# Drjay806/PRO-B-GAN

Measured on NVIDIA B200. Metric: generator+discriminator samples/sec (score_triplets pass, bf16 tensor-core mode), higher is better.
Workload: dtype bf16

## Files before the change

include/pbg.h:

```cpp
#ifndef PBG_H_
#define PBG_H_

#include <stddef.h>
#include <stdint.h>

#ifdef __cplusplus
extern "C" {
#endif

#define PBG_ABI_VERSION 1

typedef struct pbg_ctx pbg_ctx;

typedef enum pbg_status {
  PBG_OK = 0,
  PBG_ERR_INVALID = 1,
  PBG_ERR_CUDA = 2,
  PBG_ERR_NOT_LOADED = 3,
  PBG_ERR_INDEX = 4,
  PBG_ERR_UNSUPPORTED = 5,
  PBG_ERR_NOMEM = 6
} pbg_status;

typedef enum pbg_precision {
  PBG_PREC_F32 = 0,
  PBG_PREC_BF16 = 1
} pbg_precision;

typedef enum pbg_dtype { PBG_DT_F32 = 0, PBG_DT_BF16 = 1 } pbg_dtype;

typedef struct pbg_dims {
  int32_t embed_dim;
  int32_t noise_dim;
  int32_t g_hidden;
  int32_t d_hidden;
  int32_t device;
  float leaky_slope;
} pbg_dims;

int pbg_abi_version(void);

int pbg_create(pbg_ctx** out, const pbg_dims* dims);
void pbg_destroy(pbg_ctx* ctx);

const char* pbg_last_error(const pbg_ctx* ctx);

int pbg_load_generator(pbg_ctx* ctx, const float* packed_host, size_t n_floats);

int pbg_load_discriminator(pbg_ctx* ctx, const float* packed_host, size_t n_floats);

int pbg_generator_forward(pbg_ctx* ctx, const float* h, const float* r, const float* z, void* out,
                          int64_t B, int precision, int out_dtype, void* stream);

int pbg_generator_forward_gather(pbg_ctx* ctx, const float* node_emb, int64_t N, const float* rel_emb,
                                 int64_t R, const int64_t* heads, int64_t head_stride,
                                 const int64_t* rels, int64_t rel_stride, const float* z, void* out,
                                 int64_t B, int precision, int out_dtype, void* stream);

int pbg_discriminator_forward(pbg_ctx* ctx, const float* h, const float* r, const float* t,
                              float* logits, float* probs, int64_t B, int precision, void* stream);

int pbg_discriminator_score_triplets(pbg_ctx* ctx, const float* node_emb, int64_t N,
                                     const float* rel_emb, int64_t R, const int64_t* triplets,
                                     float* logits, float* probs, int64_t B, int precision,
                                     void* stream);

int pbg_score_triplets(pbg_ctx* ctx, const float* node_emb, int64_t N, const float* rel_emb, int64_t R,
                       const int64_t* triplets, const float* z, void* gen_out, int out_dtype,
                       float* gen_scores, float* logits, float* probs, int64_t B, int precision,
                       void* stream);

int pbg_score_triplets_host(pbg_ctx* ctx, const float* node_emb, int64_t N, const float* rel_emb,
                            int64_t R, const int64_t* triplets_host, const float* z_host,
                            float* gen_out_host, float* gen_scores_host, float* logits_host,
                            float* probs_host, int64_t B, int precision);

int pbg_score_triplets_host_packed(pbg_ctx* ctx, const float* node_emb, int64_t N, const float* rel_emb,
                                   int64_t R, const void* in_block_host, float* out_block_host, int64_t B,
                                   int precision);

int pbg_draw_latents(pbg_ctx* ctx, uint64_t seed, uint64_t offset, int64_t total_rows, int64_t row_begin,
                     int64_t rows, float* z_out, uint64_t* offset_after, void* stream);

int pbg_set_latent_stream(pbg_ctx* ctx, int enable, uint64_t seed, uint64_t offset);
int pbg_get_latent_stream(pbg_ctx* ctx, uint64_t* seed, uint64_t* offset, void* stream);

int pbg_score_triplets_host_ids(pbg_ctx* ctx, const float* node_emb, int64_t N, const float* rel_emb, int64_t R,
                                const int64_t* triplets_host, float* out_block_host, int64_t B, int precision);

int pbg_reserve(pbg_ctx* ctx, int64_t rows, int precision, int stage_slots);
int pbg_stage_triplets(pbg_ctx* ctx, int slot, const float* node_emb, int64_t N, const float* rel_emb, int64_t R,
                       const int64_t* triplets, const float* z, int64_t B, int want_gen, int want_disc, void* stream);
int pbg_score_staged(pbg_ctx* ctx, int slot, void* gen_out, int out_dtype, float* gen_scores, float* logits,
                     float* probs, void* stream);
int pbg_score_staged_stage_next(pbg_ctx* ctx, int slot, void* gen_out, int out_dtype, float* gen_scores, float* logits,
                                float* probs, const float* node_emb, int64_t N, const float* rel_emb, int64_t R,
                                const int64_t* next_triplets, const float* next_z, int64_t next_B, void* stream);

int pbg_check_indices(pbg_ctx* ctx, void* stream);

int pbg_linear_bf16(pbg_ctx* ctx, int model, int layer, const void* a_bf16, void* out, int64_t M,
                    void* stream);

enum {
  PBG_K_GATHER = 0,
  PBG_K_G_L0 = 1,
  PBG_K_G_L1 = 2,
  PBG_K_G_L2 = 3,
  PBG_K_D_L0 = 4,
  PBG_K_D_L1 = 5,
  PBG_K_OTHER = 6,
  PBG_K_PASS = 7,
  PBG_K_TOPK = 8,
  PBG_NUM_KERNEL_KINDS = 9
};
int pbg_profile_enable(pbg_ctx* ctx, int enable);
int pbg_profile_read(pbg_ctx* ctx, double* ms, int64_t* count);

int pbg_debug_trace(pbg_ctx* ctx, int enable, int64_t* host_out, int64_t n_slots);

int pbg_set_launch_width(pbg_ctx* ctx, int n_ctas);

int pbg_last_pass_sm_clock(pbg_ctx* ctx, void* stream, double* mhz_out);

int pbg_set_workspace_discard(pbg_ctx* ctx, int on);

int pbg_set_result_mirrors(pbg_ctx* ctx, int n, void* const* gen_out, float* const* gen_scores,
                           float* const* logits, float* const* probs);

int pbg_set_result_multicast(pbg_ctx* ctx, void* gen_out_mc, float* gen_scores_mc, float* logits_mc, float* probs_mc);

int pbg_topk_prepare(pbg_ctx* ctx, const float* table, int64_t N, void* stream);
int pbg_topk(pbg_ctx* ctx, const float* queries, int64_t B, int k, int64_t* out_idx, float* out_scores, void* stream);
int64_t pbg_topk_last_flagged(pbg_ctx* ctx, void* stream);

int64_t pbg_parse_index_rows(const char* text, size_t len, int cols, int64_t* out, size_t cap_rows);

int64_t pbg_format_f32_json(const float* v, size_t rows, int cols, int indent, int depth, char* out, size_t cap);
int64_t pbg_format_i64_json(const int64_t* v, size_t rows, int cols, int indent, int depth, char* out, size_t cap);

int64_t pbg_launch_count(const pbg_ctx* ctx);

#ifdef __cplusplus
}
#endif
#endif
```

pro-b-gan_b200/csrc/gather.cuh:

```cuda
#pragma once
#include <cuda_bf16.h>
#include <stdint.h>

namespace pbg {

struct GatherParams {
  const float* node_emb;
  const float* rel_emb;
  long long N, R;
  int E, Z;
  const long long* heads; long long head_stride;
  const long long* rels;  long long rel_stride;
  const long long* tails; long long tail_stride;
  const float* h; const float* r; const float* t;
  const float* z;
  void* xg; int ldg;
  void* xd; int ldd;
  long long B;
  int* err_flag;
};

template <typename T>
__device__ __forceinline__ void store4(T* dst, float4 v);
template <>
__device__ __forceinline__ void store4<float>(float* dst, float4 v) {
  *reinterpret_cast<float4*>(dst) = v;
}
template <>
__device__ __forceinline__ void store4<__nv_bfloat16>(__nv_bfloat16* dst, float4 v) {
  __nv_bfloat162 lo = __floats2bfloat162_rn(v.x, v.y), hi = __floats2bfloat162_rn(v.z, v.w);
  uint2 w;
  w.x = *reinterpret_cast<uint32_t*>(&lo);
  w.y = *reinterpret_cast<uint32_t*>(&hi);
  *reinterpret_cast<uint2*>(dst) = w;
}

__device__ __forceinline__ float4 ld_stream4(const float* p) {
  float4 v;
  asm volatile("ld.global.nc.L1::no_allocate.v4.f32 {%0, %1, %2, %3}, [%4];"
               : "=f"(v.x), "=f"(v.y), "=f"(v.z), "=f"(v.w) : "l"(p));
  return v;
}

template <typename T>
__global__ void __launch_bounds__(256) gather_concat_kernel(const GatherParams p) {
  const int lane = threadIdx.x & 31;
  const long long warp_global = (static_cast<long long>(blockIdx.x) * blockDim.x + threadIdx.x) >> 5;
  const long long num_warps = (static_cast<long long>(gridDim.x) * blockDim.x) >> 5;
  const int E4 = p.E >> 2, Z4 = p.Z >> 2;
  T* xg = static_cast<T*>(p.xg);
  T* xd = static_cast<T*>(p.xd);

  for (long long b = warp_global; b < p.B; b += num_warps) {
    const float *hrow, *rrow, *trow = nullptr;
    bool bad = false;
    if (p.heads != nullptr) {
      long long i = p.heads[b * p.head_stride];
      if (i < 0) i += p.N;
      if (i < 0 || i >= p.N) { bad = true; i = 0; }
      hrow = p.node_emb + i * p.E;
    } else {
      hrow = p.h + b * p.E;
    }
    if (p.rels != nullptr) {
      long long i = p.rels[b * p.rel_stride];
      if (i < 0 || i >= p.R) { bad = true; i = 0; }
      rrow = p.rel_emb + i * p.E;
    } else {
      rrow = p.r + b * p.E;
    }
    if (p.tails != nullptr) {
      long long i = p.tails[b * p.tail_stride];
      if (i < 0) i += p.N;
      if (i < 0 || i >= p.N) { bad = true; i = 0; }
      trow = p.node_emb + i * p.E;
    } else if (xd != nullptr) {
      trow = p.t + b * p.E;
    }
    if (bad && lane == 0) atomicOr(p.err_flag, 1);

    T* g = xg ? xg + b * p.ldg : nullptr;
    T* d = xd ? xd + b * p.ldd : nullptr;
    for (int v = lane; v < E4; v += 32) {
      const float4 hv = ld_stream4(hrow + 4 * v);
      const float4 rv = ld_stream4(rrow + 4 * v);
      if (g) { store4<T>(g + 4 * v, hv); store4<T>(g + p.E + 4 * v, rv); }
      if (d) {
        store4<T>(d + 4 * v, hv);
        store4<T>(d + p.E + 4 * v, rv);
        store4<T>(d + 2 * p.E + 4 * v, ld_stream4(trow + 4 * v));
      }
    }
    if (g) {
      const float* zrow = p.z + b * p.Z;
      for (int v = lane; v < Z4; v += 32) store4<T>(g + 2 * p.E + 4 * v, ld_stream4(zrow + 4 * v));
      for (int v = (2 * p.E + p.Z) / 4 + lane; v < p.ldg / 4; v += 32)
        store4<T>(g + 4 * v, make_float4(0.f, 0.f, 0.f, 0.f));
    }
    if (d) {
      for (int v = (3 * p.E) / 4 + lane; v < p.ldd / 4; v += 32)
        store4<T>(d + 4 * v, make_float4(0.f, 0.f, 0.f, 0.f));
    }
  }
}

struct StageParams {
  GatherParams g;
  float* xt;
};
__global__ void __launch_bounds__(128, 12) stage_rows_kernel(const __grid_constant__ StageParams sp) {
  const int lane = threadIdx.x & 31;
  const long long warp_global = (static_cast<long long>(blockIdx.x) * blockDim.x + threadIdx.x) >> 5;
  const long long num_warps = (static_cast<long long>(gridDim.x) * blockDim.x) >> 5;
  const int E = sp.g.E, Z = sp.g.Z, E4 = E >> 2, Z4 = Z >> 2;
  const long long N = sp.g.N;
  __nv_bfloat16* const xg = static_cast<__nv_bfloat16*>(sp.g.xg);
  __nv_bfloat16* const xd = static_cast<__nv_bfloat16*>(sp.g.xd);
  for (long long b = warp_global; b < sp.g.B; b += num_warps) {
    bool bad = false;
    long long hi = sp.g.heads[b * 3], ri = sp.g.rels[b * 3], ti = sp.g.tails[b * 3];
    if (hi < 0) hi += N;
    if (ti < 0) ti += N;
    if (hi < 0 || hi >= N) { bad = true; hi = 0; }
    if (ri < 0 || ri >= sp.g.R) { bad = true; ri = 0; }
    if (ti < 0 || ti >= N) { bad = true; ti = 0; }
    if (bad && lane == 0) atomicOr(sp.g.err_flag, 1);
    const float* hrow = sp.g.node_emb + hi * E;
    const float* rrow = sp.g.rel_emb + ri * E;
    const float* trow = sp.g.node_emb + ti * E;
    __nv_bfloat16* g = xg ? xg + b * sp.g.ldg : nullptr;
    __nv_bfloat16* d = xd ? xd + b * sp.g.ldd : nullptr;
    for (int v = lane; v < E4; v += 32) {
      const float4 hv = ld_stream4(hrow + 4 * v);
      const float4 rv = ld_stream4(rrow + 4 * v);
      const float4 tv = ld_stream4(trow + 4 * v);
      if (g) {
        store4<__nv_bfloat16>(g + 4 * v, hv);
        store4<__nv_bfloat16>(g + E + 4 * v, rv);
      }
      if (d) {
        store4<__nv_bfloat16>(d + 4 * v, hv);
        store4<__nv_bfloat16>(d + E + 4 * v, rv);
        store4<__nv_bfloat16>(d + 2 * E + 4 * v, tv);
      }
      if (sp.xt) store4<float>(sp.xt + b * E + 4 * v, tv);
    }
    if (g) {
      for (int v = lane; v < Z4; v += 32) store4<__nv_bfloat16>(g + 2 * E + 4 * v, ld_stream4(sp.g.z + b * Z + 4 * v));
      for (int v = (2 * E + Z) / 4 + lane; v < sp.g.ldg / 4; v += 32)
        store4<__nv_bfloat16>(g + 4 * v, make_float4(0.f, 0.f, 0.f, 0.f));
    }
    if (d)
      for (int v = (3 * E) / 4 + lane; v < sp.g.ldd / 4; v += 32)
        store4<__nv_bfloat16>(d + 4 * v, make_float4(0.f, 0.f, 0.f, 0.f));
  }
}

__global__ void pack_bf16_kernel(const float* __restrict__ src, __nv_bfloat16* __restrict__ dst, int rows, int cols,
                                 int rows_p, int cols_p) {
  const long long total = static_cast<long long>(rows_p) * cols_p;
  for (long long i = static_cast<long long>(blockIdx.x) * blockDim.x + threadIdx.x; i < total;
       i += static_cast<long long>(gridDim.x) * blockDim.x) {
    const int r = static_cast<int>(i / cols_p), c = static_cast<int>(i % cols_p);
    dst[i] = __float2bfloat16_rn((r < rows && c < cols) ? src[static_cast<long long>(r) * cols + c] : 0.f);
  }
}

__global__ void pad_f32_kernel(const float* __restrict__ src, float* __restrict__ dst, int n, int n_p) {
  for (int i = blockIdx.x * blockDim.x + threadIdx.x; i < n_p; i += gridDim.x * blockDim.x)
    dst[i] = i < n ? src[i] : 0.f;
}

}
```

pro-b-gan_b200/csrc/pass2_kernel.cuh:

```cuda
#pragma once
#include <cuda.h>
#include "ptx.cuh"
#include "gather.cuh"
#include "tc_common.cuh"
#include "pass_common.cuh"

namespace pbg {

#ifndef PBG_STAGES
#define PBG_STAGES 5
#endif
#ifndef PBG_EPI_WARPS
#define PBG_EPI_WARPS 8
#endif
constexpr int kP2Stages = PBG_STAGES;
constexpr int kP2Epi = PBG_EPI_WARPS;
constexpr int kP2Slots = kP2Epi / 4;
constexpr int kP2Threads = 64 + 32 * kP2Epi;
static_assert(kP2Epi == 8 || kP2Epi == 16, "epilogue warps");
#ifndef PBG_ROLES_FIRST
#define PBG_ROLES_FIRST 0
#endif
constexpr int kProdWarp = PBG_ROLES_FIRST ? 0 : kP2Epi;
constexpr int kMmaWarp = PBG_ROLES_FIRST ? 1 : kP2Epi + 1;
// ... 50 lines not shown
  int phase0_groups;
  int n_total;
  int n_seg;
  P2Segment seg[16];
  int nrb;
  int rb_cap;
  int M;
  float slope;
  PassSched* sched;
  int* ready;
  int* fin;
  void* gen_out; int out_f32; int n_valid; int ld_gen;
  float* cosine; const float* tail_tab; const long long* tail_idx; long long tail_stride; long long n_ent;
  float* part_g;
  int slots_g;
  const float* w3; float b3; float* logits; float* probs;
  int w3_off;
  float* part_d;
  int slots_d;
  int n_mirror;
  void* mir_gen[kMaxMirrors]; float* mir_cos[kMaxMirrors]; float* mir_logits[kMaxMirrors]; float* mir_probs[kMaxMirrors];
  void* mc_gen; float* mc_cos; float* mc_logits; float* mc_probs;
  long long* trace;
};
static_assert(sizeof(Pass2Params) <= 4096, "kernel parameter space");

struct P2Smem {
  static constexpr int kA = 128 * kBlockK * 2;
  static constexpr int kW = 128 * kBlockK * 2;
  static constexpr int kStage = kA + kW;
  static constexpr int kStagingOff = kP2Stages * kStage;
  static constexpr int kStagingPerWarp = 4096;
  static constexpr int kBiasOff = kStagingOff + kP2Epi * kStagingPerWarp;
  static constexpr int kBiasFloats = 6144;
  static constexpr int kBarOff = kBiasOff + kBiasFloats * 4;
  static constexpr int kXchgOff = kBarOff + 256;
  static constexpr int kXchgBytes = 4 * 32 * 3 * 4;
  static constexpr int kTotal = kXchgOff + kXchgBytes + 256 + 1024 ;
};
static_assert(P2Smem::kTotal <= 232448, "pass2: shared memory budget");

__device__ __forceinline__ void st_cluster_u32x2(uint32_t cluster_addr, uint2 v) {
  asm volatile("st.shared::cluster.v2.u32 [%0], {%1, %2};" ::"r"(cluster_addr), "r"(v.x), "r"(v.y) : "memory");
}
__device__ __forceinline__ void multimem_st_v4(void* mc_addr, uint4 v) {
  asm volatile("multimem.st.relaxed.sys.global.v4.f32 [%0], {%1, %2, %3, %4};" ::"l"(mc_addr), "f"(__uint_as_float(v.x)),
               "f"(__uint_as_float(v.y)), "f"(__uint_as_float(v.z)), "f"(__uint_as_float(v.w)) : "memory");
}
__device__ __forceinline__ void multimem_st_f32(float* mc_addr, float v) {
  asm volatile("multimem.st.relaxed.sys.global.f32 [%0], %1;" ::"l"(mc_addr), "f"(v) : "memory");
}
__device__ __forceinline__ float2 add2(float2 a, float2 b) {
  float2 d;
  asm("{\n\t.reg .b64 ra, rb, rd;\n\tmov.b64 ra, {%2, %3};\n\tmov.b64 rb, {%4, %5};\n\tadd.rn.f32x2 rd, ra, rb;\n\t"
      "mov.b64 {%0, %1}, rd;\n\t}\n"
      : "=f"(d.x), "=f"(d.y) : "f"(a.x), "f"(a.y), "f"(b.x), "f"(b.y));
  return d;
}
__device__ __forceinline__ float2 mul2(float2 a, float2 b) {
  float2 d;
  asm("{\n\t.reg .b64 ra, rb, rd;\n\tmov.b64 ra, {%2, %3};\n\tmov.b64 rb, {%4, %5};\n\tmul.rn.f32x2 rd, ra, rb;\n\t"
      "mov.b64 {%0, %1}, rd;\n\t}\n"
      : "=f"(d.x), "=f"(d.y) : "f"(a.x), "f"(a.y), "f"(b.x), "f"(b.y));
  return d;
}
__device__ __forceinline__ uint32_t bias_leaky_pack(uint32_t a0, uint32_t a1, float b0, float b1, float slope) {
  const float2 y = add2(make_float2(__uint_as_float(a0), __uint_as_float(a1)), make_float2(b0, b1));
  const float2 s = mul2(y, make_float2(slope, slope));
  return pack_bf16x2(fmaxf(y.x, s.x), fmaxf(y.y, s.y));
}

__device__ __forceinline__ int p2_dep_target(const Pass2Params& p, int dep_kind) {
  if (p.no_deps) return 0;
  if (dep_kind == DEP_X) return p.gather_external ? 0 : kP2GroupsPerBlock;
  const int producer = dep_kind == DEP_G0 ? IT_G_L0 : (dep_kind == DEP_D0 ? IT_D_L0 : IT_G_L1);
  return p.layer[producer].n_tiles * kP2WarpsPerPair;
}
__device__ __forceinline__ void p2_arrive(const Pass2Params& p, int dep_kind, int rb, int lane, bool async_stores,
                                          long long* t_wait = nullptr) {
  __syncwarp();
  if (lane == 0) {
    int* ctr = p.ready + dep_kind * p.rb_cap + rb;
    if (async_stores) {
      const long long t0 = t_wait ? clock64() : 0;
      tma_store_wait<0>();
      if (t_wait) *t_wait += clock64() - t0;
      red_relaxed_gpu_add(ctr, 1);
    } else {
      red_release_gpu_add(ctr, 1);
    }
  }
}
__device__ __forceinline__ void p2_arrive_done(const Pass2Params& p, int dep_kind, int rb, int lane) {
  if (lane == 0) red_relaxed_gpu_add(p.ready + dep_kind * p.rb_cap + rb, 1);
}
__device__ __forceinline__ void p2_poll_dep(const Pass2Params& p, int dep_kind, int rb) {
  const int target = p2_dep_target(p, dep_kind);
  const int* ctr = p.ready + dep_kind * p.rb_cap + rb;
  uint32_t spins = 0;
  while (ld_relaxed_gpu(ctr) < target) {
    __nanosleep(p.poll_ns);
#if PBG_HANG_GUARD
    if (++spins > 4000000u) pbg_wait_timed_out("dependency (kind, row block)", dep_kind, rb);
#endif
  }
  fence_proxy_async_all();
}

__device__ __forceinline__ void p2_discard(const void* base, size_t bytes, int part, int nparts, int lane) {
  const char* b = static_cast<const char*>(base);
  for (size_t off = static_cast<size_t>(part) * 4096 + static_cast<size_t>(lane) * 128; off < bytes; off += static_cast<size_t>(nparts) * 4096)
    asm volatile("discard.global.L2 [%0], 128;" ::"l"(b + off) : "memory");
}

__device__ __forceinline__ void p2_tail_load(float4 (&tv)[8], unsigned long long trow_bits, int col0, int n_valid, int lane) {
#pragma unroll
  for (int i = 0; i < 8; ++i) {
    const int r = i * 4 + (lane >> 3), t = lane & 7;
    const float* tp2 = reinterpret_cast<const float*>(__shfl_sync(0xffffffffu, trow_bits, r));
    tv[i] = make_float4(0.f, 0.f, 0.f, 0.f);
    if (tp2 != nullptr && col0 + t * 4 < n_valid) tv[i] = ld_stream4(tp2 + col0 + t * 4);
  }
}
__device__ __forceinline__ void p2_tail_stage(uint8_t* st, const float4 (&tv)[8], int lane) {
#pragma unroll
  for (int i = 0; i < 8; ++i) {
    const int r = i * 4 + (lane >> 3), t = lane & 7;
    *reinterpret_cast<float4*>(st + r * 128 + ((t ^ (r & 7)) << 4)) = tv[i];
  }
  __syncwarp();
}
__device__ __forceinline__ void p2_tail_dot(const uint8_t* st, const float* f, int col0, int n_valid, int lane, float& d, float& pp,
                                            float& tt) {
#pragma unroll
  for (int t = 0; t < 8; ++t) {
    const float4 x = *reinterpret_cast<const float4*>(st + lane * 128 + ((t ^ (lane & 7)) << 4));
    if (col0 + t * 4 < n_valid) {
      d += f[4 * t] * x.x + f[4 * t + 1] * x.y + f[4 * t + 2] * x.z + f[4 * t + 3] * x.w;
      pp += f[4 * t] * f[4 * t] + f[4 * t + 1] * f[4 * t + 1] + f[4 * t + 2] * f[4 * t + 2] + f[4 * t + 3] * f[4 * t + 3];
      tt += x.x * x.x + x.y * x.y + x.z * x.z + x.w * x.w;
    }
  }
  __syncwarp();
}

template <class F>
__device__ __forceinline__ void p2_gather_group_bulk(const GatherParams& g, long long group, int lane, uint8_t* st,
                                                     F&& before_staging, bool keep) {
  const long long r0 = group * 4;
  __nv_bfloat16* xg = static_cast<__nv_bfloat16*>(g.xg);
  __nv_bfloat16* xd = static_cast<__nv_bfloat16*>(g.xd);
  const float* src = nullptr;
  bool bad = false;
  if (lane < 12) {
    const long long row = r0 + lane / 3;
    const int which = lane % 3;
    if (row < g.B) {
      if (which == 0) {
        if (g.heads) { long long i = g.heads[row * g.head_stride]; if (i < 0) i += g.N; if (i < 0 || i >= g.N) { bad = true; i = 0; } src = g.node_emb + i * g.E; }
        else src = g.h + row * g.E;
      } else if (which == 1) {
        if (g.rels) { long long i = g.rels[row * g.rel_stride]; if (i < 0 || i >= g.R) { bad = true; i = 0; } src = g.rel_emb + i * g.E; }
        else src = g.r + row * g.E;
      } else if (g.tails) {
        long long i = g.tails[row * g.tail_stride]; if (i < 0) i += g.N; if (i < 0 || i >= g.N) { bad = true; i = 0; } src = g.node_emb + i * g.E;
      } else if (xd != nullptr) {
        src = g.t + row * g.E;
      }
    }
  }
  if (bad) atomicOr(g.err_flag, 1);
  const unsigned long long sp = reinterpret_cast<unsigned long long>(src);
  const int Z4 = g.Z >> 2;
  const int wg = 2 * g.E + g.Z, wd = 3 * g.E;
  float4 hv[4], rv[4], tv[4], zv[4];
#pragma unroll
  for (int j = 0; j < 4; ++j) {
    const float* ph = reinterpret_cast<const float*>(__shfl_sync(0xffffffffu, sp, j * 3 + 0));
    const float* pr = reinterpret_cast<const float*>(__shfl_sync(0xffffffffu, sp, j * 3 + 1));
    const float* pt = reinterpret_cast<const float*>(__shfl_sync(0xffffffffu, sp, j * 3 + 2));
    const long long row = r0 + j;
    hv[j] = rv[j] = tv[j] = zv[j] = make_float4(0.f, 0.f, 0.f, 0.f);
    if (row < g.B) {
      hv[j] = ld_stream4(ph + 4 * lane);
      rv[j] = ld_stream4(pr + 4 * lane);
      if (xd != nullptr) tv[j] = ld_stream4(pt + 4 * lane);
      if (xg != nullptr && lane < Z4) zv[j] = ld_stream4(g.z + row * g.Z + 4 * lane);
    }
  }
  before_staging();
  const long long nrow = min(4ll, g.B - r0);
  if (xg != nullptr) {
#pragma unroll
    for (int j = 0; j < 4; ++j) {
      __nv_bfloat16* o = reinterpret_cast<__nv_bfloat16*>(st) + j * wg;
      store4<__nv_bfloat16>(o + 4 * lane, hv[j]);
      store4<__nv_bfloat16>(o + g.E + 4 * lane, rv[j]);
      if (lane < Z4) store4<__nv_bfloat16>(o + 2 * g.E + 4 * lane, zv[j]);
    }
    fence_proxy_async_smem();
    __syncwarp();
    if (lane == 0 && nrow > 0) {
      if (keep) bulk_store_1d_hint(xg + r0 * wg, st, static_cast<uint32_t>(nrow * wg * 2), kEvictLast);
      else bulk_store_1d(xg + r0 * wg, st, static_cast<uint32_t>(nrow * wg * 2));
      tma_store_commit();
      if (xd != nullptr) tma_store_wait_read<0>();
    }
    __syncwarp();
  }
  if (xd != nullptr) {
#pragma unroll
    for (int j = 0; j < 4; ++j) {
      __nv_bfloat16* o = reinterpret_cast<__nv_bfloat16*>(st) + j * wd;
      store4<__nv_bfloat16>(o + 4 * lane, hv[j]);
      store4<__nv_bfloat16>(o + g.E + 4 * lane, rv[j]);
      store4<__nv_bfloat16>(o + 2 * g.E + 4 * lane, tv[j]);
    }
    fence_proxy_async_smem();
    __syncwarp();
    if (lane == 0 && nrow > 0) {
      if (keep) bulk_store_1d_hint(xd + r0 * wd, st, static_cast<uint32_t>(nrow * wd * 2), kEvictLast);
      else bulk_store_1d(xd + r0 * wd, st, static_cast<uint32_t>(nrow * wd * 2));
      tma_store_commit();
    }
  }
}

__device__ __forceinline__ uint32_t ring_dep(uint2 it) { return (it.x >> 24) << 3; }

template <bool TR, bool FASTG, bool BIASS>
__global__ void __cluster_dims__(2, 1, 1) __launch_bounds__(kP2Threads, 1)
pbg_pass2_kernel(const __grid_constant__ Pass2Params p) {
  using L = P2Smem;
  extern __shared__ uint8_t smem_raw[];
  uint8_t* smem = smem_raw + ((1024u - (smem_u32(smem_raw) & 1023u)) & 1023u);
  uint64_t* full_bar = reinterpret_cast<uint64_t*>(smem + L::kBarOff);
  uint64_t* empty_bar = full_bar + kP2Stages;
  uint64_t* tmem_full = empty_bar + kP2Stages;
  uint64_t* tmem_empty = tmem_full + 2;
  uint64_t* sched_full = tmem_empty + 2;
  uint64_t* sched_empty = sched_full + kP2Ring;
  uint64_t* bias_bar = sched_empty + kP2Ring;
  uint2* ring = reinterpret_cast<uint2*>(bias_bar + 1);
  uint32_t* tmem_slot = reinterpret_cast<uint32_t*>(ring + kP2Ring);
  int* last_flag = reinterpret_cast<int*>(tmem_slot + 1);
  volatile long long* t_issue = reinterpret_cast<volatile long long*>(smem + L::kXchgOff + L::kXchgBytes);
  float* xchg = reinterpret_cast<float*>(smem + L::kXchgOff);
  float* sbias = reinterpret_cast<float*>(smem + L::kBiasOff);

  const int warp = threadIdx.x >> 5;
  const int lane = threadIdx.x & 31;
  const uint32_t rank = cluster_ctarank();
  const bool leader = rank == 0;
  const long long t_entry = (TR && p.trace && threadIdx.x == 0) ? static_cast<long long>(globaltimer_ns()) : 0;
  asm volatile("griddepcontrol.launch_dependents;" ::: "memory");
  constexpr int kRingConsumers = 2 * (1 + kP2Epi) + 1;

  if (threadIdx.x == 0) {
    for (int i = 0; i < 5; ++i) {
      if (p.layer_mask & (1u << i)) {
        prefetch_tmap(&p.tm_a[i]);
        prefetch_tmap(&p.tm_w[i]);
        if (p.layer[i].epi == PEPI_STORE) prefetch_tmap(&p.tm_o[i]);
      }
    }
    for (int s = 0; s < kP2Stages; ++s) {
      mbar_init(&full_bar[s], 1);
      mbar_init(&empty_bar[s], 1);
    }
    for (int s = 0; s < 2; ++s) {
      mbar_init(&tmem_full[s], 1);
      mbar_init(&tmem_empty[s], kP2WarpsPerPair);
    }
    for (int s = 0; s < kP2Ring; ++s) {
      mbar_init(&sched_full[s], 1);
      mbar_init(&sched_empty[s], kRingConsumers);
    }
    mbar_init(bias_bar, 1);
    fence_mbar_init();
    if (BIASS) {
    uint32_t bytes = 0;
    for (int k = 0; k < 5; ++k)
      if (p.layer_mask & (1u << k)) bytes += static_cast<uint32_t>(p.layer[k].n_tiles * p.layer[k].block_n) * 4u;
    if (p.layer_mask & (1u << IT_D_L1)) bytes += static_cast<uint32_t>(p.layer[IT_D_L1].n_tiles * p.layer[IT_D_L1].block_n) * 4u;
    mbar_arrive_expect_tx(bias_bar, bytes);
    for (int k = 0; k < 5; ++k)
      if (p.layer_mask & (1u << k))
        bulk_load_1d(sbias + p.layer[k].bias_off, p.layer[k].bias, static_cast<uint32_t>(p.layer[k].n_tiles * p.layer[k].block_n) * 4u, bias_bar);
    if (p.layer_mask & (1u << IT_D_L1))
      bulk_load_1d(sbias + p.w3_off, p.w3, static_cast<uint32_t>(p.layer[IT_D_L1].n_tiles * p.layer[IT_D_L1].block_n) * 4u, bias_bar);
    }
  }
  if (warp == kMmaWarp) tmem_alloc_pair<512>(tmem_slot);
  tc_fence_before();
  __syncthreads();
  cluster_sync_all();
  tc_fence_after();
  asm volatile("griddepcontrol.wait;" ::: "memory");
  const uint32_t tmem_base = *tmem_slot;
  long long* const clk0 = reinterpret_cast<long long*>(smem + L::kXchgOff + L::kXchgBytes) + 8;
  if (blockIdx.x == 0 && threadIdx.x == 0) { clk0[0] = clock64(); clk0[1] = static_cast<long long>(globaltimer_ns()); }
  long long* const tr = (TR && p.trace) ? p.trace + kTraceSlots * blockIdx.x : nullptr;
  if (tr && threadIdx.x == 0) { tr[0] = clock64(); tr[14] = static_cast<long long>(globaltimer_ns()); tr[254] = t_entry; }

  const uint32_t lead_tmem_empty = mapa_u32(smem_u32(tmem_empty), 0);
  const uint32_t sched_empty_addr = mapa_u32(smem_u32(sched_empty), 1);
  const uint32_t ring_addr = mapa_u32(smem_u32(ring), 1);
  if (warp == kMmaWarp && !leader) {
    if (lane == 0) {
      uint32_t slot = 0, sphase = 0;
      const uint32_t lead_sched_full = mapa_u32(smem_u32(sched_full), 0);
      for (;;) {
        const int ticket = atomicAdd(&p.sched->q_head, 1);
        uint2 it = make_uint2(IT_END, 0u);
        if (ticket < p.n_total) {
          int sg = 0;
          while (sg + 1 < p.n_seg && ticket >= p.seg[sg + 1].start) ++sg;
          const int i = ticket - p.seg[sg].start;
          const int nt1 = p.seg[sg].n_tiles, nt = nt1 + p.seg[sg].n_tiles2;
          const int j = i % nt;
          it = make_uint2(static_cast<uint32_t>(j < nt1 ? p.seg[sg].kind : p.seg[sg].kind2) | (static_cast<uint32_t>(j < nt1 ? j : j - nt1) << 8),
                          static_cast<uint32_t>(p.seg[sg].rb0 + i / nt));
        }
        if ((it.x & 0xff) != IT_END) p2_poll_dep(p, p.layer[it.x & 0xff].dep_kind, static_cast<int>(it.y));
        mbar_wait_role(&sched_empty[slot], sphase ^ 1);
        ring[slot] = it;
        mbar_arrive(&sched_full[slot]);
        mbar_arrive_cluster(lead_sched_full + slot * 8);
        if (++slot == kP2Ring) { slot = 0; sphase ^= 1; }
        if ((it.x & 0xff) == IT_END) break;
      }
    }
    __syncwarp();
  } else if (warp == kProdWarp) {
    if (lane == 0) {
      uint32_t stage = 0, phase = 0, slot = 0, sphase = 0;
      long long w_dep = 0, w_empty = 0, n_items = 0;
      const uint32_t lead_full = mapa_u32(smem_u32(full_bar), 0);
      for (;;) {
        mbar_wait_role(&sched_full[slot], sphase);
        const uint2 it = ld_cluster_u32x2(ring_addr + slot * 8);
        mbar_arrive_remote(sched_empty_addr + slot * 8 + ring_dep(it));
        if (++slot == kP2Ring) { slot = 0; sphase ^= 1; }
        const int kind = it.x & 0xff;
        if (kind == IT_END) break;
        long long* ti = (tr && n_items < kTraceItems) ? tr + 16 + 4 * n_items : nullptr;
        if (ti) { ti[0] = (clock64() << 20) | (static_cast<long long>(it.y & 0xfff) << 8) | kind; }
        ++n_items;
        const int n_blk = (it.x >> 8) & 0xff;
        const int rb = static_cast<int>(it.y);
        const P2Layer& ly = p.layer[kind];
        const int w_rows = ly.block_n >> 1;
        const uint32_t bytes_pair = 2u * (L::kA + static_cast<uint32_t>(w_rows) * kBlockK * 2);
        const int a_row = rb * kP2Rows + static_cast<int>(rank) * 128;
        const int w_row = n_blk * ly.block_n + static_cast<int>(rank) * w_rows;
        for (int kb = 0; kb < ly.num_kb; ++kb) {
          if (tr) { const long long t = clock64(); mbar_wait_role(&empty_bar[stage], phase ^ 1); w_empty += clock64() - t; }
          else mbar_wait_role(&empty_bar[stage], phase ^ 1);
          uint8_t* sa = smem + stage * L::kStage;
          if (leader) mbar_arrive_expect_tx(&full_bar[stage], bytes_pair);
          if (tr) t_issue[stage] = clock64();
          tma_load_2d_pair(sa + L::kA, &p.tm_w[kind], lead_full + stage * 8, kb * kBlockK, w_row);
          tma_load_2d_pair(sa, &p.tm_a[kind], lead_full + stage * 8, kb * kBlockK, a_row);
          if (++stage == kP2Stages) { stage = 0; phase ^= 1; }
        }
      }
      if (tr) { tr[1] = w_empty; tr[2] = clock64(); tr[12] = n_items; if (leader) tr[11] = w_dep; }
    }
    __syncwarp();
// ... 589 lines not shown
```

pro-b-gan_b200/csrc/pass_common.cuh:

```cuda
#pragma once
#include <cuda.h>
#include "ptx.cuh"
#include "gather.cuh"
#include "tc_common.cuh"

namespace pbg {

enum : int { IT_G_L0 = 0, IT_D_L0 = 1, IT_G_L1 = 2, IT_D_L1 = 3, IT_G_L2 = 4, IT_GATHER = 5, IT_END = 255 };
enum : int { DEP_X = 0, DEP_G0 = 1, DEP_D0 = 2, DEP_G1 = 3, DEP_KINDS = 4 };
enum : int { FIN_G = 0, FIN_D = 1, FIN_KINDS = 2 };
enum : int { PEPI_STORE = 0, PEPI_TANH = 1, PEPI_ROWDOT = 2 };

constexpr int kEpiWarps = 8;
constexpr int kPassThreads = 64 + 32 * kEpiWarps;
constexpr int kTraceSlots = 256;
constexpr int kTraceItems = 54;


struct PassSched {
  int q_head;
  int q_tail;
  int p0_next;
  int init;
  int done;
  int pad_;
  long long clk_ticks, clk_ns;
};



__device__ __forceinline__ int ld_relaxed_gpu(const int* p) {
  int v;
  asm volatile("ld.relaxed.gpu.global.s32 %0, [%1];" : "=r"(v) : "l"(p) : "memory");
  return v;
}
__device__ __forceinline__ void fence_acq_rel_gpu() { asm volatile("fence.acq_rel.gpu;" ::: "memory"); }
__device__ __forceinline__ void red_release_gpu_add(int* p, int v) {
  asm volatile("red.release.gpu.global.add.s32 [%0], %1;" ::"l"(p), "r"(v) : "memory");
}
__device__ __forceinline__ void red_relaxed_gpu_add(int* p, int v) {
  asm volatile("red.relaxed.gpu.global.add.s32 [%0], %1;" ::"l"(p), "r"(v) : "memory");
}
__device__ __forceinline__ int atom_relaxed_gpu_add(int* p, int v) {
  int old;
  asm volatile("atom.relaxed.gpu.global.add.s32 %0, [%1], %2;" : "=r"(old) : "l"(p), "r"(v) : "memory");
  return old;
}
__device__ __forceinline__ int atom_release_gpu_add(int* p, int v) {
  int old;
  asm volatile("atom.release.gpu.global.add.s32 %0, [%1], %2;" : "=r"(old) : "l"(p), "r"(v) : "memory");
  return old;
}
__device__ __forceinline__ unsigned long long globaltimer_ns() {
  unsigned long long t;
  asm volatile("mov.u64 %0, %%globaltimer;" : "=l"(t));
  return t;
}
__device__ __forceinline__ void fence_proxy_async_all() { asm volatile("fence.proxy.async;" ::: "memory"); }

__device__ __forceinline__ void tmem_ld_32x32_ptr(uint32_t taddr, uint32_t* v) {
  asm volatile(
      "tcgen05.ld.sync.aligned.32x32b.x32.b32 "
      "{%0, %1, %2, %3, %4, %5, %6, %7, %8, %9, %10, %11, %12, %13, %14, %15, "
      "%16, %17, %18, %19, %20, %21, %22, %23, %24, %25, %26, %27, %28, %29, %30, %31}, [%32];"
      : "=r"(v[0]), "=r"(v[1]), "=r"(v[2]), "=r"(v[3]), "=r"(v[4]), "=r"(v[5]), "=r"(v[6]), "=r"(v[7]),
        "=r"(v[8]), "=r"(v[9]), "=r"(v[10]), "=r"(v[11]), "=r"(v[12]), "=r"(v[13]), "=r"(v[14]), "=r"(v[15]),
        "=r"(v[16]), "=r"(v[17]), "=r"(v[18]), "=r"(v[19]), "=r"(v[20]), "=r"(v[21]), "=r"(v[22]), "=r"(v[23]),
        "=r"(v[24]), "=r"(v[25]), "=r"(v[26]), "=r"(v[27]), "=r"(v[28]), "=r"(v[29]), "=r"(v[30]), "=r"(v[31])
      : "r"(taddr)
      : "memory");
}

__device__ __forceinline__ float leaky_max(float x, float slope) { return fmaxf(x, x * slope); }

template <int MODE = 0>
__device__ __forceinline__ void pass_gather_group(const GatherParams& g, long long group, int lane) {
  const long long r0 = group * 4;
  __nv_bfloat16* xg = static_cast<__nv_bfloat16*>(g.xg);
  __nv_bfloat16* xd = static_cast<__nv_bfloat16*>(g.xd);
  const float* src = nullptr;
  bool bad = false;
  if (lane < 12) {
    const long long row = r0 + lane / 3;
    const int which = lane % 3;
    if (row < g.B) {
      if (which == 0) {
        if (g.heads) { long long i = g.heads[row * g.head_stride]; if (i < 0) i += g.N; if (i < 0 || i >= g.N) { bad = true; i = 0; } src = g.node_emb + i * g.E; }
        else src = g.h + row * g.E;
      } else if (which == 1) {
        if (g.rels) { long long i = g.rels[row * g.rel_stride]; if (i < 0 || i >= g.R) { bad = true; i = 0; } src = g.rel_emb + i * g.E; }
        else src = g.r + row * g.E;
      } else if (g.tails) {
        long long i = g.tails[row * g.tail_stride]; if (i < 0) i += g.N; if (i < 0 || i >= g.N) { bad = true; i = 0; } src = g.node_emb + i * g.E;
      } else if (xd != nullptr) {
        src = g.t + row * g.E;
      }
    }
  }
  if (bad) atomicOr(g.err_flag, 1);
  const unsigned long long sp = reinterpret_cast<unsigned long long>(src);
  const int E4 = g.E >> 2, Z4 = g.Z >> 2;
  if (MODE == 1 || (MODE == 0 && E4 == 32 && Z4 <= 32)) {
    float4 hv[4], rv[4], tv[4], zv[4];
#pragma unroll
    for (int j = 0; j < 4; ++j) {
      const float* ph = reinterpret_cast<const float*>(__shfl_sync(0xffffffffu, sp, j * 3 + 0));
      const float* pr = reinterpret_cast<const float*>(__shfl_sync(0xffffffffu, sp, j * 3 + 1));
      const float* pt = reinterpret_cast<const float*>(__shfl_sync(0xffffffffu, sp, j * 3 + 2));
      const long long row = r0 + j;
      hv[j] = rv[j] = tv[j] = zv[j] = make_float4(0.f, 0.f, 0.f, 0.f);
      if (row < g.B) {
        hv[j] = ld_stream4(ph + 4 * lane);
        rv[j] = ld_stream4(pr + 4 * lane);
        if (xd != nullptr) tv[j] = ld_stream4(pt + 4 * lane);
        if (xg != nullptr && lane < Z4) zv[j] = ld_stream4(g.z + row * g.Z + 4 * lane);
      }
    }
#pragma unroll
    for (int j = 0; j < 4; ++j) {
      const long long row = r0 + j;
      if (row >= g.B) continue;
      if (xg != nullptr) {
        __nv_bfloat16* o = xg + row * g.ldg;
        store4<__nv_bfloat16>(o + 4 * lane, hv[j]);
        store4<__nv_bfloat16>(o + g.E + 4 * lane, rv[j]);
        if (lane < Z4) store4<__nv_bfloat16>(o + 2 * g.E + 4 * lane, zv[j]);
        for (int v = (2 * g.E + g.Z) / 4 + lane; v < g.ldg / 4; v += 32)
          store4<__nv_bfloat16>(o + 4 * v, make_float4(0.f, 0.f, 0.f, 0.f));
      }
      if (xd != nullptr) {
        __nv_bfloat16* o = xd + row * g.ldd;
        store4<__nv_bfloat16>(o + 4 * lane, hv[j]);
        store4<__nv_bfloat16>(o + g.E + 4 * lane, rv[j]);
        store4<__nv_bfloat16>(o + 2 * g.E + 4 * lane, tv[j]);
        for (int v = (3 * g.E) / 4 + lane; v < g.ldd / 4; v += 32)
          store4<__nv_bfloat16>(o + 4 * v, make_float4(0.f, 0.f, 0.f, 0.f));
      }
    }
  } else {
    for (int j = 0; j < 4; ++j) {
      const float* ph = reinterpret_cast<const float*>(__shfl_sync(0xffffffffu, sp, j * 3 + 0));
      const float* pr = reinterpret_cast<const float*>(__shfl_sync(0xffffffffu, sp, j * 3 + 1));
      const float* pt = reinterpret_cast<const float*>(__shfl_sync(0xffffffffu, sp, j * 3 + 2));
      const long long row = r0 + j;
      if (row >= g.B) continue;
      __nv_bfloat16* og = xg ? xg + row * g.ldg : nullptr;
      __nv_bfloat16* od = xd ? xd + row * g.ldd : nullptr;
      for (int v = lane; v < E4; v += 32) {
        const float4 h4 = ld_stream4(ph + 4 * v), r4 = ld_stream4(pr + 4 * v);
        if (og) { store4<__nv_bfloat16>(og + 4 * v, h4); store4<__nv_bfloat16>(og + g.E + 4 * v, r4); }
        if (od) {
          store4<__nv_bfloat16>(od + 4 * v, h4);
          store4<__nv_bfloat16>(od + g.E + 4 * v, r4);
          store4<__nv_bfloat16>(od + 2 * g.E + 4 * v, ld_stream4(pt + 4 * v));
        }
      }
      if (og) {
        for (int v = lane; v < Z4; v += 32) store4<__nv_bfloat16>(og + 2 * g.E + 4 * v, ld_stream4(g.z + row * g.Z + 4 * v));
        for (int v = (2 * g.E + g.Z) / 4 + lane; v < g.ldg / 4; v += 32)
          store4<__nv_bfloat16>(og + 4 * v, make_float4(0.f, 0.f, 0.f, 0.f));
      }
      if (od)
        for (int v = (3 * g.E) / 4 + lane; v < g.ldd / 4; v += 32)
          store4<__nv_bfloat16>(od + 4 * v, make_float4(0.f, 0.f, 0.f, 0.f));
    }
  }
}

__device__ __forceinline__ void warp_publish(int* counter, int lane) {
  __syncwarp();
  if (lane == 0) red_release_gpu_add(counter, 1);
}
__device__ __forceinline__ int warp_publish_fetch(int* counter, int lane) {
  __syncwarp();
  int old = 0;
  if (lane == 0) old = atom_release_gpu_add(counter, 1);
  return __shfl_sync(0xffffffffu, old, 0);
}


}
```

pro-b-gan_b200/csrc/pbg.cu:

```cuda
#include <cuda.h>
#include <cuda_runtime.h>
#include <cuda_bf16.h>

#include <algorithm>
#include <cstdarg>
#include <cstdio>
#include <cstring>
#include <cstdlib>
#include <map>
#include <tuple>
#include <new>
#include <string>
#include <vector>

#include "../../include/pbg.h"
#include "gather.cuh"
#include "gemm_f32.cuh"
#include "tc_common.cuh"
#include "pass_common.cuh"
#include "pass2_kernel.cuh"
#include "topk_kernel.cuh"
#include "index_rows.cuh"
#include "json_out.cuh"
#include "latent.cuh"

using namespace pbg;

namespace {

constexpr long long kMaxChunk = 65536;
constexpr int kPartSlotsG = 16;
constexpr int kPartSlotsD = 64;

inline int round_up(int v, int m) { return (v + m - 1) / m * m; }

struct Linear {
  int n = 0, k = 0;
  int np = 0, kp = 0;
  float* w_f32 = nullptr;
  float* b_f32 = nullptr;
  __nv_bfloat16* w_bf16 = nullptr;
  float* b_pad = nullptr;
  CUtensorMap tmap_w128;
  CUtensorMap tmap_w64;
};

struct Workspace {
  long long rows = 0;
  void *xg0 = nullptr, *xd0 = nullptr, *bufA = nullptr, *bufB = nullptr, *bufD = nullptr;
  CUtensorMap tm_xg0, tm_xd0, tm_bufA_g, tm_bufA_d, tm_bufB_g, tm_bufD_d;
  CUtensorMap tmo_bufA, tmo_bufB, tmo_bufD;
  int mb_cap = 0;
  int* ready = nullptr;
  int* fin = nullptr;
  PassSched* sched = nullptr;
  float* part_g = nullptr;
  float* part_d = nullptr;
};

struct TopkState {
  const float* table = nullptr; long long N = 0, n_pad = 0;
  __nv_bfloat16* tn = nullptr; float* inv_t = nullptr; CUtensorMap tm_t;
  long long q_cap = 0; __nv_bfloat16* qn = nullptr; float* inv_q = nullptr; CUtensorMap tm_q;
  size_t cand_cap = 0; unsigned* cand_grp = nullptr; unsigned* cand_mask = nullptr; int* cand_cnt = nullptr;
  size_t samp_cap = 0; int* samp_keys = nullptr;
  float* tau = nullptr; int* flag = nullptr;
  long long last_rows = 0; bool last_filtered = false;
  size_t score_cap = 0; float* score_buf = nullptr;
};

struct StageSlot {
  long long cap = 0;
  void *xg0 = nullptr, *xd0 = nullptr;
  float* xt = nullptr;
  float* z = nullptr;
  CUtensorMap tm_xg0, tm_xd0;
  long long B = -1;
  bool has_g = false, has_d = false;
  bool has_xt = false;
  const float* node_emb = nullptr; long long N = 0; const long long* tails = nullptr;
};

thread_local std::string g_create_error;

typedef CUresult (*EncodeTiledFn)(CUtensorMap*, CUtensorMapDataType, cuuint32_t, void*, const cuuint64_t*,
                                  const cuuint64_t*, const cuuint32_t*, const cuuint32_t*, CUtensorMapInterleave,
                                  CUtensorMapSwizzle, CUtensorMapL2promotion, CUtensorMapFloatOOBfill);

}

struct pbg_ctx {
  pbg_dims dims{};
  int num_sms = 0;
  int max_threads_sm = 0;
  bool g_loaded = false, d_loaded = false;
  int kg0 = 0, kg0p = 0, kd0 = 0, kd0p = 0, hgp = 0, hdp = 0, hd2 = 0, hmax = 0;
  Linear g[3], d[2];
  float* d_w3 = nullptr;
  float* d_w3_pad = nullptr;
  float d_b3 = 0.f;
  Workspace ws_bf16, ws_f32;
  StageSlot stage[2];
  int* err_flag = nullptr;
  int* err_flag_host = nullptr;
  cudaStream_t own_stream = nullptr;
  long long host_cap = 0;
  char* st_block = nullptr;
  EncodeTiledFn encode = nullptr;
  TopkState tk;
  bool lat_on = false;
  unsigned long long lat_seed = 0;
  LatentStream* lat_st = nullptr;
  long long lat_cap = 0;
  float* lat_z = nullptr;
  long long launches = 0;
  int launch_ctas = 0;
  int discard = 1;
  bool host_block = false;
  cudaEvent_t host_evt = nullptr;
  int n_mirror = 0;
  void* mir_gen[kMaxMirrors] = {}; float* mir_cos[kMaxMirrors] = {}; float* mir_logits[kMaxMirrors] = {}; float* mir_probs[kMaxMirrors] = {};
  void* mc_gen = nullptr; float *mc_cos = nullptr, *mc_logits = nullptr, *mc_probs = nullptr;
  bool profiling = false;
  long long* trace = nullptr;
  struct ProfRec { cudaEvent_t a, b; int kind; };
  std::vector<ProfRec> prof;
  std::string err;
};

namespace {

int fail(pbg_ctx* c, int code, const char* fmt, ...) {
  char buf[512];
  va_list ap;
  va_start(ap, fmt);
  vsnprintf(buf, sizeof buf, fmt, ap);
  va_end(ap);
  if (c) c->err = buf; else g_create_error = buf;
  return code;
}

struct LaunchScope {
  pbg_ctx* c; cudaStream_t s; cudaEvent_t b = nullptr;
  LaunchScope(pbg_ctx* c_, int kind, cudaStream_t s_) : c(c_), s(s_) {
    c->launches += 1;
    if (c->profiling) {
      cudaEvent_t a;
      cudaEventCreate(&a); cudaEventCreate(&b);
      cudaEventRecord(a, s);
      c->prof.push_back({a, b, kind});
    }
  }
  ~LaunchScope() { if (b) cudaEventRecord(b, s); }
};

#define PBG_CUDA(c, expr)                                                                               \
  do {                                                                                                  \
    cudaError_t e_ = (expr);                                                                            \
    if (e_ != cudaSuccess) return fail((c), PBG_ERR_CUDA, "%s failed: %s", #expr, cudaGetErrorString(e_)); \
  } while (0)

#define PBG_TRY(expr)            \
  do {                           \
    int s_ = (expr);             \
    if (s_ != PBG_OK) return s_; \
  } while (0)

int make_tmap(pbg_ctx* c, CUtensorMap* tm, const void* base, long long rows, int cols, int box_rows) {
  cuuint64_t dims[2] = {static_cast<cuuint64_t>(cols), static_cast<cuuint64_t>(rows)};
  cuuint64_t strides[1] = {static_cast<cuuint64_t>(cols) * 2};
  cuuint32_t box[2] = {static_cast<cuuint32_t>(kBlockK), static_cast<cuuint32_t>(box_rows)};
  cuuint32_t estr[2] = {1, 1};
  CUresult r = c->encode(tm, CU_TENSOR_MAP_DATA_TYPE_BFLOAT16, 2, const_cast<void*>(base), dims, strides, box, estr,
                         CU_TENSOR_MAP_INTERLEAVE_NONE, CU_TENSOR_MAP_SWIZZLE_128B, CU_TENSOR_MAP_L2_PROMOTION_L2_256B,
                         CU_TENSOR_MAP_FLOAT_OOB_FILL_NONE);
  if (r != CUDA_SUCCESS) return fail(c, PBG_ERR_CUDA, "cuTensorMapEncodeTiled failed (%d) rows=%lld cols=%d", (int)r, rows, cols);
  return PBG_OK;
}

void free_linear(Linear& l) {
  cudaFree(l.w_f32); cudaFree(l.b_f32); cudaFree(l.w_bf16); cudaFree(l.b_pad);
  l = Linear{};
}

void free_ws(Workspace& w) {
  cudaFree(w.xg0); cudaFree(w.xd0); cudaFree(w.bufA); cudaFree(w.bufB); cudaFree(w.bufD);
  cudaFree(w.ready); cudaFree(w.fin); cudaFree(w.sched); cudaFree(w.part_g); cudaFree(w.part_d);
  w = Workspace{};
}

int upload_linear(pbg_ctx* c, Linear& l, int n, int k, int kp, const float* w_host, const float* b_host) {
  free_linear(l);
  l.n = n; l.k = k; l.kp = kp;
  l.np = round_up(n, 128);
  PBG_CUDA(c, cudaMalloc(&l.w_f32, sizeof(float) * n * k));
  PBG_CUDA(c, cudaMalloc(&l.b_f32, sizeof(float) * n));
  PBG_CUDA(c, cudaMalloc(&l.w_bf16, sizeof(__nv_bfloat16) * (size_t)l.np * l.kp));
  PBG_CUDA(c, cudaMalloc(&l.b_pad, sizeof(float) * l.np));
  PBG_CUDA(c, cudaMemcpyAsync(l.w_f32, w_host, sizeof(float) * n * k, cudaMemcpyHostToDevice, c->own_stream));
  PBG_CUDA(c, cudaMemcpyAsync(l.b_f32, b_host, sizeof(float) * n, cudaMemcpyHostToDevice, c->own_stream));
  { LaunchScope ls(c, PBG_K_OTHER, c->own_stream);
    pack_bf16_kernel<<<c->num_sms * 4, 256, 0, c->own_stream>>>(l.w_f32, l.w_bf16, n, k, l.np, l.kp); }
  { LaunchScope ls(c, PBG_K_OTHER, c->own_stream);
    pad_f32_kernel<<<8, 256, 0, c->own_stream>>>(l.b_f32, l.b_pad, n, l.np); }
  PBG_CUDA(c, cudaGetLastError());
  PBG_CUDA(c, cudaStreamSynchronize(c->own_stream));
  PBG_TRY(make_tmap(c, &l.tmap_w128, l.w_bf16, l.np, l.kp, 128));
  return make_tmap(c, &l.tmap_w64, l.w_bf16, l.np, l.kp, 64);
}

int begin_growth(pbg_ctx* c, cudaStream_t s, const char* what) {
  cudaStreamCaptureStatus st = cudaStreamCaptureStatusNone;
  if (cudaStreamIsCapturing(s, &st) == cudaSuccess && st != cudaStreamCaptureStatusNone)
    return fail(c, PBG_ERR_INVALID, "%s must grow while the stream is being captured: call pbg_reserve() first", what);
  PBG_CUDA(c, cudaDeviceSynchronize());
  return PBG_OK;
}

long long pow2_cap(long long rows) {
  long long cap = 1024;
  while (cap < rows) cap *= 2;
  return std::min(cap, kMaxChunk);
}

template <class T>
int realloc_dev(pbg_ctx* c, T*& p, size_t bytes) {
  cudaFree(p); p = nullptr;
  PBG_CUDA(c, cudaMalloc(&p, bytes));
  return PBG_OK;
}

void free_stage(StageSlot& st) {
  cudaFree(st.xg0); cudaFree(st.xd0); cudaFree(st.xt); cudaFree(st.z);
  st = StageSlot{};
}

int ensure_ws(pbg_ctx* c, int prec, long long rows, cudaStream_t stream) {
  Workspace& w = prec == PBG_PREC_BF16 ? c->ws_bf16 : c->ws_f32;
  if (w.rows >= rows) return PBG_OK;
  PBG_TRY(begin_growth(c, stream, "the workspace"));
  const long long cap = pow2_cap(rows);
  free_ws(w);
  if (prec == PBG_PREC_BF16) {
    const size_t es = sizeof(__nv_bfloat16);
    PBG_CUDA(c, cudaMalloc(&w.xg0, es * cap * c->kg0p));
    PBG_CUDA(c, cudaMalloc(&w.xd0, es * cap * c->kd0p));
    PBG_CUDA(c, cudaMalloc(&w.bufA, es * cap * c->hmax));
    PBG_CUDA(c, cudaMalloc(&w.bufB, es * cap * c->hmax));
    PBG_CUDA(c, cudaMalloc(&w.bufD, es * cap * c->hdp));
    PBG_TRY(make_tmap(c, &w.tm_bufD_d, w.bufD, cap, c->hdp, kBlockM));
    PBG_TRY(make_tmap(c, &w.tmo_bufA, w.bufA, cap, c->hgp, 32));
    PBG_TRY(make_tmap(c, &w.tmo_bufB, w.bufB, cap, c->hgp, 32));
    PBG_TRY(make_tmap(c, &w.tmo_bufD, w.bufD, cap, c->hdp, 32));
    w.mb_cap = static_cast<int>(cap / kBlockM);
    PBG_CUDA(c, cudaMalloc(&w.ready, sizeof(int) * DEP_KINDS * w.mb_cap));
    PBG_CUDA(c, cudaMalloc(&w.fin, sizeof(int) * FIN_KINDS * w.mb_cap));
    PBG_CUDA(c, cudaMalloc(&w.sched, sizeof(PassSched)));
    PBG_CUDA(c, cudaMalloc(&w.part_g, sizeof(float) * w.mb_cap * kPartSlotsG * 3 * kBlockM));
    PBG_CUDA(c, cudaMalloc(&w.part_d, sizeof(float) * w.mb_cap * kPartSlotsD * kBlockM));
    PBG_CUDA(c, cudaMemset(w.ready, 0, sizeof(int) * DEP_KINDS * w.mb_cap));
    PBG_CUDA(c, cudaMemset(w.fin, 0, sizeof(int) * FIN_KINDS * w.mb_cap));
    PBG_CUDA(c, cudaMemset(w.sched, 0, sizeof(PassSched)));
    PBG_TRY(make_tmap(c, &w.tm_xg0, w.xg0, cap, c->kg0p, kBlockM));
    PBG_TRY(make_tmap(c, &w.tm_xd0, w.xd0, cap, c->kd0p, kBlockM));
    PBG_TRY(make_tmap(c, &w.tm_bufA_g, w.bufA, cap, c->hgp, kBlockM));
    PBG_TRY(make_tmap(c, &w.tm_bufA_d, w.bufA, cap, c->hdp, kBlockM));
    PBG_TRY(make_tmap(c, &w.tm_bufB_g, w.bufB, cap, c->hgp, kBlockM));
  } else {
    const size_t es = sizeof(float);
    const int hm = std::max(std::max(c->dims.g_hidden, c->dims.d_hidden), c->dims.embed_dim);
    PBG_CUDA(c, cudaMalloc(&w.xg0, es * cap * c->kg0));
    PBG_CUDA(c, cudaMalloc(&w.xd0, es * cap * c->kd0));
    PBG_CUDA(c, cudaMalloc(&w.bufA, es * cap * hm));
    PBG_CUDA(c, cudaMalloc(&w.bufB, es * cap * hm));
  }
  w.rows = cap;
  return PBG_OK;
}

int ensure_stage(pbg_ctx* c, StageSlot& st, long long rows, cudaStream_t stream) {
  if (st.cap >= rows) return PBG_OK;
  PBG_TRY(begin_growth(c, stream, "a staging slot"));
  const long long cap = pow2_cap(rows);
  free_stage(st);
  const size_t es = sizeof(__nv_bfloat16);
  PBG_CUDA(c, cudaMalloc(&st.xg0, es * cap * c->kg0p));
  PBG_CUDA(c, cudaMalloc(&st.xd0, es * cap * c->kd0p));
  PBG_CUDA(c, cudaMalloc(&st.xt, sizeof(float) * cap * c->dims.embed_dim));
  PBG_CUDA(c, cudaMalloc(&st.z, sizeof(float) * cap * c->dims.noise_dim));
  PBG_TRY(make_tmap(c, &st.tm_xg0, st.xg0, cap, c->kg0p, kBlockM));
  PBG_TRY(make_tmap(c, &st.tm_xd0, st.xd0, cap, c->kd0p, kBlockM));
  st.cap = cap;
  return PBG_OK;
}

int ensure_latents(pbg_ctx* c, long long rows, cudaStream_t stream) {
  if (c->lat_cap >= rows) return PBG_OK;
  PBG_TRY(begin_growth(c, stream, "the latent workspace"));
  const long long cap = pow2_cap(rows);
  c->lat_cap = 0;
  PBG_TRY(realloc_dev(c, c->lat_z, sizeof(float) * cap * c->dims.noise_dim));
  c->lat_cap = cap;
  return PBG_OK;
}

int check_draw_size(pbg_ctx* c, long long total_rows) {
  if (total_rows < 1) return fail(c, PBG_ERR_INVALID, "latent draw: total_rows must be positive");
  if (total_rows > 0x7fffffffll / c->dims.noise_dim)
    return fail(c, PBG_ERR_UNSUPPORTED, "latent draw: %lld x %d elements is above the 2^31 - 1 of one torch launch",
                total_rows, c->dims.noise_dim);
  return PBG_OK;
}

int launch_draw(pbg_ctx* c, unsigned long long seed, unsigned long long offset, LatentStream* st, bool advance,
                long long total_rows, long long row_begin, long long rows, float* out, cudaStream_t s) {
  if (rows <= 0) return PBG_OK;
  const long long Z = c->dims.noise_dim;
  const LatentGeometry g = latent_geometry(total_rows * Z, c->num_sms, c->max_threads_sm);
  LatentParams p{};
  p.seed = seed; p.offset = offset; p.st = st; p.advance = advance ? 1 : 0; p.inc = g.inc; p.T = g.T;
  p.e_begin = row_begin * Z; p.e_end = (row_begin + rows) * Z; p.out = out;
  const long long r_lo = p.e_begin / (4 * g.T), r_hi = (p.e_end - 1) / (4 * g.T);
  p.slot_begin = r_lo * g.T;
  const long long blocks = (r_hi - r_lo + 1) * g.T / kLatentThreads;
  { LaunchScope ls(c, PBG_K_OTHER, s);
    latent_draw_kernel<<<static_cast<unsigned>(blocks), kLatentThreads, 0, s>>>(p); }
  PBG_CUDA(c, cudaGetLastError());
  return PBG_OK;
}

int draw_stream(pbg_ctx* c, long long B, float* out, cudaStream_t s) {
  PBG_TRY(check_draw_size(c, B));
  return launch_draw(c, c->lat_seed, 0, c->lat_st, true, B, 0, B, out, s);
}

template <int ACT>
int launch_f32(pbg_ctx* c, int kind, const Linear& l, const float* A, long long lda, float* out, long long ldo, long long M,
               cudaStream_t s) {
  F32GemmParams p{A, lda, l.w_f32, l.k, l.b_f32, out, ldo, (int)M, l.n, l.k, c->dims.leaky_slope};
  dim3 grid((l.n + 63) / 64, (unsigned)((M + 63) / 64));
  { LaunchScope ls(c, kind, s);
    gemm_f32_kernel<ACT><<<grid, 256, 0, s>>>(p); }
  PBG_CUDA(c, cudaGetLastError());
  return PBG_OK;
}


int pass_grid(const pbg_ctx* c) {
  static const int env = [] { const char* e = getenv("PBG_GRID"); return e ? atoi(e) : 0; }();
  const int want = c->launch_ctas > 0 ? c->launch_ctas : env;
  return (want > 0 && want < c->num_sms) ? std::max(2, want) : c->num_sms;
}

struct Pass;
int launch_pass2(pbg_ctx* c, Workspace& w, const Pass& a, const GatherParams& gp, long long off, long long rows,
                 void* gen_out, float* scores, bool external_gather, const StageSlot* slot = nullptr, bool gather_ahead = false);

struct Pass {
  const float* node_emb = nullptr; long long N = 0;
  const float* rel_emb = nullptr;  long long R = 0;
  const long long *heads = nullptr, *rels = nullptr, *tails = nullptr;
  long long hs = 1, rs = 1, ts = 1;
  const float *h = nullptr, *r = nullptr, *t = nullptr, *z = nullptr;
  bool draw_z = false;
  void* gen_out = nullptr; int out_dtype = PBG_DT_F32;
  float *gen_scores = nullptr, *logits = nullptr, *probs = nullptr;
  bool run_g = false, run_d = false;
  long long B = 0; int prec = PBG_PREC_BF16; cudaStream_t stream = nullptr;
};

int run_chunk(pbg_ctx* c, const Pass& a, long long off, long long rows) {
  const int E = c->dims.embed_dim, Z = c->dims.noise_dim;
  const bool bf = a.prec == PBG_PREC_BF16;
  Workspace& w = bf ? c->ws_bf16 : c->ws_f32;
  cudaStream_t s = a.stream;

  GatherParams gp{};
  gp.node_emb = a.node_emb; gp.rel_emb = a.rel_emb; gp.N = a.N; gp.R = a.R; gp.E = E; gp.Z = Z;
  gp.heads = a.heads ? a.heads + off * a.hs : nullptr; gp.head_stride = a.hs;
  gp.rels = a.rels ? a.rels + off * a.rs : nullptr;    gp.rel_stride = a.rs;
  gp.tails = a.tails ? a.tails + off * a.ts : nullptr; gp.tail_stride = a.ts;
  gp.h = a.h ? a.h + off * E : nullptr; gp.r = a.r ? a.r + off * E : nullptr; gp.t = a.t ? a.t + off * E : nullptr;
  gp.z = a.z ? a.z + off * Z : nullptr;
  if (a.draw_z) {
    PBG_TRY(launch_draw(c, c->lat_seed, 0, c->lat_st, off + rows == a.B, a.B, off, rows, c->lat_z, s));
    gp.z = c->lat_z;
  }
  gp.xg = a.run_g ? w.xg0 : nullptr; gp.ldg = bf ? c->kg0p : c->kg0;
  gp.xd = a.run_d ? w.xd0 : nullptr; gp.ldd = bf ? c->kd0p : c->kd0;
  gp.B = rows; gp.err_flag = c->err_flag;
  const int gather_blocks = (int)std::min<long long>((rows + 7) / 8, (long long)c->num_sms * 8);
  if (!bf && (c->n_mirror > 0 || c->mc_gen || c->mc_cos || c->mc_logits || c->mc_probs))
    return fail(c, PBG_ERR_UNSUPPORTED, "result mirrors / multicast are a bf16-mode feature");
  static const bool split_env = [] { const char* e = getenv("PBG_SPLIT_GATHER"); return e && atoi(e) != 0; }();
  const bool split = bf && split_env && rows > 0;
  if (!bf) {
    LaunchScope ls(c, PBG_K_GATHER, s);
    gather_concat_kernel<float><<<gather_blocks, 256, 0, s>>>(gp);
  } else if (split) {
    LaunchScope ls(c, PBG_K_GATHER, s);
    gather_concat_kernel<__nv_bfloat16><<<gather_blocks, 256, 0, s>>>(gp);
  }
  PBG_CUDA(c, cudaGetLastError());

  const size_t out_es = a.out_dtype == PBG_DT_BF16 ? 2 : 4;
  void* gen_out = a.gen_out ? static_cast<char*>(a.gen_out) + (size_t)off * E * out_es : nullptr;
  float* scores = a.gen_scores ? a.gen_scores + off : nullptr;

  if (bf) {
    return launch_pass2(c, w, a, gp, off, rows, gen_out, scores, split);
  } else {
    float *xg0 = (float*)w.xg0, *xd0 = (float*)w.xd0, *bufA = (float*)w.bufA, *bufB = (float*)w.bufB;
    const int row_blocks = (int)std::min<long long>((rows + 7) / 8, (long long)c->num_sms * 8);
    if (a.run_g) {
      const int H = c->dims.g_hidden;
      PBG_TRY(launch_f32<ACT_LEAKY>(c, PBG_K_G_L0, c->g[0], xg0, c->kg0, bufA, H, rows, s));
      PBG_TRY(launch_f32<ACT_LEAKY>(c, PBG_K_G_L1, c->g[1], bufA, H, bufB, H, rows, s));
      float* pred = gen_out ? (float*)gen_out : bufA;
      PBG_TRY(launch_f32<ACT_TANH>(c, PBG_K_G_L2, c->g[2], bufB, H, pred, E, rows, s));
      if (scores) {
        { LaunchScope ls(c, PBG_K_OTHER, s);
          cosine_f32_kernel<<<row_blocks, 256, 0, s>>>(pred, E, a.node_emb, a.N, a.tails + off * a.ts, a.ts, E, rows,
                                                       scores); }
        PBG_CUDA(c, cudaGetLastError());
      }
    }
    if (a.run_d) {
      const int H = c->dims.d_hidden, H2 = c->hd2;
      PBG_TRY(launch_f32<ACT_LEAKY>(c, PBG_K_D_L0, c->d[0], xd0, c->kd0, bufA, H, rows, s));
      PBG_TRY(launch_f32<ACT_LEAKY>(c, PBG_K_D_L1, c->d[1], bufA, H, bufB, H2, rows, s));
      { LaunchScope ls(c, PBG_K_OTHER, s);
        rowdot_f32_kernel<<<row_blocks, 256, 0, s>>>(bufB, H2, c->d_w3, c->d_b3, H2, rows, a.logits + off,
                                                     a.probs ? a.probs + off : nullptr); }
      PBG_CUDA(c, cudaGetLastError());
    }
  }
  return PBG_OK;
}


template <class... KArgs, class... Args>
cudaError_t launch_pdl(bool pdl, void (*kern)(KArgs...), unsigned grid, unsigned block, size_t smem, cudaStream_t s, Args&&... args) {
  cudaLaunchConfig_t cfg = {};
  cfg.gridDim = dim3(grid); cfg.blockDim = dim3(block); cfg.dynamicSmemBytes = smem; cfg.stream = s;
  cudaLaunchAttribute at[1];
  at[0].id = cudaLaunchAttributeProgrammaticStreamSerialization;
  at[0].val.programmaticStreamSerializationAllowed = 1;
  cfg.attrs = at; cfg.numAttrs = pdl ? 1 : 0;
  return cudaLaunchKernelEx(&cfg, kern, static_cast<KArgs>(args)...);
}

using Pass2Kernel = void (*)(Pass2Params);
const Pass2Kernel kPass2[8] = {
    pbg_pass2_kernel<false, false, false>, pbg_pass2_kernel<false, false, true>, pbg_pass2_kernel<false, true, false>,
    pbg_pass2_kernel<false, true, true>,   pbg_pass2_kernel<true, false, false>, pbg_pass2_kernel<true, false, true>,
    pbg_pass2_kernel<true, true, false>,   pbg_pass2_kernel<true, true, true>};

const int kEpiOf[5] = {PEPI_STORE, PEPI_STORE, PEPI_STORE, PEPI_ROWDOT, PEPI_TANH};
const int kPredOf[5] = {DEP_X, DEP_X, DEP_G0, DEP_D0, DEP_G1};
const int kOutOf[5] = {DEP_G0, DEP_D0, DEP_G1, -1, -1};

void set_layer(Pass2Params& p, int k, const Linear& l, const CUtensorMap& amap, const CUtensorMap* omap,
               __nv_bfloat16* out, int ldo) {
  const int bn = (l.np % 256 == 0) ? 256 : 128;
  p.tm_a[k] = amap;
  p.tm_w[k] = bn == 256 ? l.tmap_w128 : l.tmap_w64;
  if (omap) p.tm_o[k] = *omap;
  p.layer[k] = P2Layer{l.kp / kBlockK, bn, l.np / bn, kEpiOf[k], kPredOf[k], kOutOf[k], ldo, -1, l.b_pad, out};
  p.layer_mask |= 1u << k;
}

int launch_pass2(pbg_ctx* c, Workspace& w, const Pass& a, const GatherParams& gp, long long off, long long rows,
                 void* gen_out, float* scores, bool external_gather, const StageSlot* slot, bool gather_ahead) {
  const int grid = pass_grid(c) & ~1;
  Pass2Params p;
  memset(&p, 0, sizeof p);
  const Linear* lin[5] = {&c->g[0], &c->d[0], &c->g[1], &c->d[1], &c->g[2]};
  const CUtensorMap* amap[5] = {slot ? &slot->tm_xg0 : &w.tm_xg0, slot ? &slot->tm_xd0 : &w.tm_xd0, &w.tm_bufA_g, &w.tm_bufD_d,
                                &w.tm_bufB_g};
  const CUtensorMap* omap[5] = {&w.tmo_bufA, &w.tmo_bufD, &w.tmo_bufB, nullptr, nullptr};
  const bool on[5] = {a.run_g, a.run_d, a.run_g, a.run_d, a.run_g};
  const int nrb = static_cast<int>((rows + kP2Rows - 1) / kP2Rows);
  __nv_bfloat16* outs[5] = {(__nv_bfloat16*)w.bufA, (__nv_bfloat16*)w.bufD, (__nv_bfloat16*)w.bufB, nullptr, nullptr};
  const int ldos[5] = {c->hgp, c->hdp, c->hgp, 0, 0};
  long long total = 0;
  for (int k = 0; k < 5; ++k) {
    if (!on[k]) continue;
    set_layer(p, k, *lin[k], *amap[k], omap[k], outs[k], ldos[k]);
    if (p.layer[k].n_tiles > 255) return fail(c, PBG_ERR_UNSUPPORTED, "layer too wide for the tile index");
    total += static_cast<long long>(nrb) * p.layer[k].n_tiles;
  }
  bool biass = false;
  {
    int off = 0;
    for (int k = 0; k < 5; ++k) if (on[k]) { p.layer[k].bias_off = off; off += lin[k]->np; }
    p.w3_off = off;
    if (on[IT_D_L1]) off += lin[IT_D_L1]->np;
    biass = off <= P2Smem::kBiasFloats;
  }
  if (on[IT_D_L1] && lin[IT_D_L1]->np / 64 > kPartSlotsD) return fail(c, PBG_ERR_UNSUPPORTED, "d_hidden too wide for the partial buffer");
  if (on[IT_G_L2] && lin[IT_G_L2]->np / 64 > kPartSlotsG / 2) return fail(c, PBG_ERR_UNSUPPORTED, "embed_dim too wide for the partial buffer");
  p.phase0_groups = external_gather ? 0 : nrb * kP2GroupsPerBlock;
  p.gather_external = external_gather ? 1 : 0;
  if (gather_ahead) {
    p.phase0_groups = static_cast<int>((gp.B + 3) / 4);
    p.gather_ahead = 1;
  }
  {
    static const int waves_env = [] { const char* e = getenv("PBG_WAVES"); return e ? atoi(e) : 1; }();
    const int waves = std::max(1, std::min(waves_env, std::min(nrb, 3)));
    static const int mix_env = [] { const char* e = getenv("PBG_MIX"); return e ? atoi(e) : 0; }();
    const bool mix = on[IT_D_L1] && on[IT_G_L2] && mix_env != 0;
    int start = 0;
    auto add_seg = [&](int k, int rb_lo, int rb_hi, int k2 = -1) {
      if (k < 0 || !on[k] || rb_hi == rb_lo) return;
      const int nt2 = (k2 >= 0 && on[k2]) ? p.layer[k2].n_tiles : 0;
      p.seg[p.n_seg++] = P2Segment{k, p.layer[k].n_tiles, start, rb_lo, nt2 ? k2 : k, nt2};
      start += (rb_hi - rb_lo) * (p.layer[k].n_tiles + nt2);
    };
    for (int wv = 0; wv < waves; ++wv) {
      const int rb_lo = static_cast<int>(static_cast<long long>(nrb) * wv / waves);
      const int rb_hi = static_cast<int>(static_cast<long long>(nrb) * (wv + 1) / waves);
      add_seg(IT_G_L0, rb_lo, rb_hi);
      add_seg(IT_D_L0, rb_lo, rb_hi);
    }
    add_seg(IT_G_L1, 0, nrb);
    if (mix) {
      add_seg(IT_D_L1, 0, nrb, IT_G_L2);
    } else {
      add_seg(IT_D_L1, 0, nrb);
      add_seg(IT_G_L2, 0, nrb);
    }
    if (start != total) return fail(c, PBG_ERR_INVALID, "internal: static item list does not cover the pass");
    p.n_total = start;
  }
  p.gather = gp;
  static const int poll_env = [] { const char* e = getenv("PBG_POLL_NS"); return e ? atoi(e) : 40; }();
  p.poll_ns = poll_env;
  static const int defer_env = [] { const char* e = getenv("PBG_GATHER_DEFER"); return e ? atoi(e) : 1; }();
  p.gather_defer = defer_env;
  p.discard = c->discard;
  if (!external_gather) {
    p.dead_xg = gp.xg; p.dead_xd = gp.xd;
  } else if (gather_ahead && slot) {
    p.dead_xg = a.run_g ? slot->xg0 : nullptr; p.dead_xd = a.run_d ? slot->xd0 : nullptr;
  }
  p.dead_ldg = c->kg0p; p.dead_ldd = c->kd0p;
  p.nrb = nrb; p.rb_cap = w.mb_cap; p.M = static_cast<int>(rows); p.slope = c->dims.leaky_slope;
  p.sched = w.sched; p.ready = w.ready; p.fin = w.fin;
  p.gen_out = gen_out; p.out_f32 = a.out_dtype == PBG_DT_F32; p.n_valid = c->dims.embed_dim; p.ld_gen = c->dims.embed_dim;
  if (scores && slot && slot->has_xt) {
    p.cosine = scores; p.tail_tab = slot->xt; p.n_ent = slot->cap; p.tail_idx = nullptr; p.tail_stride = 0;
  } else if (scores && slot) {
    p.cosine = scores; p.tail_tab = slot->node_emb; p.n_ent = slot->N; p.tail_idx = slot->tails; p.tail_stride = 3;
  } else if (scores) {
    p.cosine = scores; p.tail_tab = a.node_emb; p.n_ent = a.N;
    p.tail_idx = a.tails + off * a.ts; p.tail_stride = a.ts;
  }
  p.part_g = w.part_g; p.slots_g = on[IT_G_L2] ? (c->dims.embed_dim + 63) / 64 : 0;
  p.w3 = c->d_w3_pad; p.b3 = c->d_b3;
  p.logits = a.logits ? a.logits + off : nullptr;
  p.probs = a.probs ? a.probs + off : nullptr;
  p.part_d = w.part_d; p.slots_d = on[IT_D_L1] ? lin[IT_D_L1]->np / 64 : 0;
  p.trace = c->trace;
  p.n_mirror = c->n_mirror;
  for (int i = 0; i < c->n_mirror; ++i) {
    if (gen_out && !c->mir_gen[i]) return fail(c, PBG_ERR_INVALID, "result mirror %d has no gen_out buffer", i);
    if (scores && !c->mir_cos[i]) return fail(c, PBG_ERR_INVALID, "result mirror %d has no gen_scores buffer", i);
    if (a.logits && !c->mir_logits[i]) return fail(c, PBG_ERR_INVALID, "result mirror %d has no logits buffer", i);
    const size_t es = a.out_dtype == PBG_DT_BF16 ? 2 : 4;
    p.mir_gen[i] = c->mir_gen[i] ? static_cast<char*>(c->mir_gen[i]) + static_cast<size_t>(off) * c->dims.embed_dim * es : nullptr;
    p.mir_cos[i] = c->mir_cos[i] ? c->mir_cos[i] + off : nullptr;
    p.mir_logits[i] = c->mir_logits[i] ? c->mir_logits[i] + off : nullptr;
    p.mir_probs[i] = (c->mir_probs[i] && a.probs) ? c->mir_probs[i] + off : nullptr;
  }
  {
    const size_t es = a.out_dtype == PBG_DT_BF16 ? 2 : 4;
    p.mc_gen = (c->mc_gen && gen_out) ? static_cast<char*>(c->mc_gen) + static_cast<size_t>(off) * c->dims.embed_dim * es : nullptr;
    p.mc_cos = (c->mc_cos && scores) ? c->mc_cos + off : nullptr;
    p.mc_logits = (c->mc_logits && a.logits) ? c->mc_logits + off : nullptr;
    p.mc_probs = (c->mc_probs && a.probs) ? c->mc_probs + off : nullptr;
  }
  static const bool pdl = [] { const char* e = getenv("PBG_PDL"); return !e || atoi(e) != 0; }();
  const bool fastg = c->dims.embed_dim == 128 && c->dims.noise_dim % 4 == 0 && c->dims.noise_dim <= 128 &&
                     c->kg0p == c->kg0 && c->kd0p == c->kd0;
  const Pass2Kernel kern = kPass2[(p.trace ? 4 : 0) | (fastg ? 2 : 0) | (biass ? 1 : 0)];
  cudaError_t le;
  { LaunchScope ls(c, PBG_K_PASS, a.stream);
    le = launch_pdl(pdl, kern, grid, kP2Threads, P2Smem::kTotal, a.stream, p); }
  if (le == cudaSuccess) le = cudaGetLastError();
  if (le != cudaSuccess) {
    cudaFuncAttributes fa{};
    cudaFuncGetAttributes(&fa, kern);
    return fail(c, PBG_ERR_CUDA, "pass kernel launch failed: %s (grid %d x %d threads, %d regs/thread, %zu B static + %d B dynamic smem, "
                "max threads/block %d, max dynamic smem %d)", cudaGetErrorString(le), grid, kP2Threads, fa.numRegs,
                fa.sharedSizeBytes, P2Smem::kTotal, fa.maxThreadsPerBlock, fa.maxDynamicSharedSizeBytes);
  }
  return PBG_OK;
}

int run_pass(pbg_ctx* c, Pass a) {
  if (!c) return PBG_ERR_INVALID;
  if (a.B < 0) return fail(c, PBG_ERR_INVALID, "negative batch");
  if (a.prec != PBG_PREC_F32 && a.prec != PBG_PREC_BF16) return fail(c, PBG_ERR_INVALID, "unknown precision %d", a.prec);
  if (a.run_g && !c->g_loaded) return fail(c, PBG_ERR_NOT_LOADED, "generator weights not loaded");
  if (a.run_d && !c->d_loaded) return fail(c, PBG_ERR_NOT_LOADED, "discriminator weights not loaded");
  if (a.run_g && a.z == nullptr && !c->lat_on) return fail(c, PBG_ERR_INVALID, "generator needs latents z");
  a.draw_z = a.run_g && a.z == nullptr && a.B > 0;
  if (a.draw_z) PBG_TRY(check_draw_size(c, a.B));
  if (a.run_g && a.gen_out && a.prec == PBG_PREC_F32 && a.out_dtype != PBG_DT_F32)
    return fail(c, PBG_ERR_INVALID, "fp32 mode writes fp32 output");
  if (a.gen_scores && a.tails == nullptr) return fail(c, PBG_ERR_INVALID, "gen_scores needs tail ids");
  if (a.B == 0 || (!a.run_g && !a.run_d)) return PBG_OK;
  PBG_CUDA(c, cudaSetDevice(c->dims.device));
  const long long chunk = std::min(a.B, kMaxChunk);
  PBG_TRY(ensure_ws(c, a.prec, chunk, a.stream));
  if (a.draw_z) PBG_TRY(ensure_latents(c, chunk, a.stream));
  for (long long off = 0; off < a.B; off += chunk) PBG_TRY(run_chunk(c, a, off, std::min(chunk, a.B - off)));
  return PBG_OK;
}

}

extern "C" {

int pbg_abi_version(void) { return PBG_ABI_VERSION; }

const char* pbg_last_error(const pbg_ctx* ctx) { return ctx ? ctx->err.c_str() : g_create_error.c_str(); }

int64_t pbg_launch_count(const pbg_ctx* ctx) { return ctx ? ctx->launches : 0; }

int64_t pbg_format_f32_json(const float* v, size_t rows, int cols, int indent, int depth, char* out, size_t cap) {
  if ((!v && rows) || cols < 0 || depth < 0) return -(int64_t)fail(nullptr, PBG_ERR_INVALID, "format_f32_json: bad arguments");
  return (int64_t)pbg_host::format_rows<float>(v, rows, cols, indent, depth, out, cap, pbg_host::put_py_float);
}

int64_t pbg_format_i64_json(const int64_t* v, size_t rows, int cols, int indent, int depth, char* out, size_t cap) {
  if ((!v && rows) || cols < 0 || depth < 0) return -(int64_t)fail(nullptr, PBG_ERR_INVALID, "format_i64_json: bad arguments");
  return (int64_t)pbg_host::format_rows<int64_t>(v, rows, cols, indent, depth, out, cap, pbg_host::put_i64);
}

int64_t pbg_parse_index_rows(const char* text, size_t len, int cols, int64_t* out, size_t cap_rows) {
  if (!text || cols < 1 || cols > 8) return -(int64_t)fail(nullptr, PBG_ERR_INVALID, "parse_index_rows: null text or cols outside 1..8");
  const char* msg = nullptr;
  size_t off = 0;
  const long long rows = pbg_host::parse_index_rows(text, len, cols, out, cap_rows, &msg, &off);
  if (rows < 0) return -(int64_t)fail(nullptr, PBG_ERR_INVALID, "parse_index_rows: %s at byte %zu", msg, off);
  return rows;
}

int pbg_topk_prepare(pbg_ctx* c, const float* table, int64_t N, void* stream) {
  if (!c) return PBG_ERR_INVALID;
  if (!table || N <= 0) return fail(c, PBG_ERR_INVALID, "topk: null or empty table");
  const int E = c->dims.embed_dim;
  if (E % 4) return fail(c, PBG_ERR_UNSUPPORTED, "topk: embed_dim must be a multiple of 4");
  PBG_CUDA(c, cudaSetDevice(c->dims.device));
  cudaStream_t s = (cudaStream_t)stream;
  TopkState& t = c->tk;
  const long long n_pad = (N + 255) / 256 * 256;
  if (n_pad != t.n_pad) {
    PBG_TRY(begin_growth(c, s, "the top-k table"));
    t.n_pad = 0;
    PBG_TRY(realloc_dev(c, t.tn, sizeof(__nv_bfloat16) * n_pad * E));
    PBG_TRY(realloc_dev(c, t.inv_t, sizeof(float) * n_pad));
    t.n_pad = n_pad;
    if (E == 128) PBG_TRY(make_tmap(c, &t.tm_t, t.tn, n_pad, E, 128));
  }
  t.table = table; t.N = N;
  { LaunchScope ls(c, PBG_K_OTHER, s);
    if (E <= 128) topk_prepare_kernel<8, 1><<<c->num_sms * 8, 256, 0, s>>>(table, N, n_pad, E, t.tn, t.inv_t);
    else topk_prepare_kernel<2, 4><<<c->num_sms * 8, 256, 0, s>>>(table, N, n_pad, E, t.tn, t.inv_t); }
  PBG_CUDA(c, cudaGetLastError());
  return PBG_OK;
}

constexpr int kTkGeneralMaxK = 512;

namespace {
int topk_general(pbg_ctx* c, TopkState& t, const float* q, long long rows, int k, long long* oi, float* os, cudaStream_t s) {
  const int E = c->dims.embed_dim;
  const long long chunk = std::max<long long>(64, std::min<long long>(rows, (512ll << 20) / (4 * t.N)));
  const size_t need = static_cast<size_t>(chunk) * t.N;
  if (t.score_cap < need) {
    PBG_TRY(begin_growth(c, s, "the top-k score buffer"));
    t.score_cap = 0;
    PBG_TRY(realloc_dev(c, t.score_buf, sizeof(float) * need));
    t.score_cap = need;
  }
  const int threads = std::max(32, std::min(256, (200 * 1024 / (k * 8)) / 32 * 32));
  const size_t smem = static_cast<size_t>(E) * 4 + static_cast<size_t>(threads) * k * 8;
  for (long long off = 0; off < rows; off += chunk) {
    const long long r = std::min(chunk, rows - off);
    F32GemmParams gp{q + off * E, E, t.table, E, nullptr, t.score_buf, t.N, (int)r, (int)t.N, E, 0.f};
    dim3 grid((unsigned)((t.N + 63) / 64), (unsigned)((r + 63) / 64));
    { LaunchScope ls(c, PBG_K_OTHER, s);
      gemm_f32_kernel<ACT_NONE><<<grid, 256, 0, s>>>(gp); }
    PBG_CUDA(c, cudaGetLastError());
    { LaunchScope ls(c, PBG_K_OTHER, s);
      topk_select_kernel<<<static_cast<unsigned>(std::min<long long>(r, 6ll * c->num_sms)), kSelThreads, 0, s>>>(
          t.score_buf, t.inv_q + off, t.inv_t, t.N, k, r, oi + off * k, os + off * k, t.flag + off); }
    PBG_CUDA(c, cudaGetLastError());
    { LaunchScope ls(c, PBG_K_OTHER, s);
      topk_exact_kernel<<<static_cast<unsigned>(std::min<long long>(r, 2ll * c->num_sms)), threads, smem, s>>>(
          q + off * E, t.inv_q + off, t.table, t.inv_t, t.N, E, k, t.flag + off, 0, t.score_buf, oi + off * k, os + off * k, r); }
    PBG_CUDA(c, cudaGetLastError());
  }
  return PBG_OK;
}
}

int pbg_topk(pbg_ctx* c, const float* queries, int64_t B, int k, int64_t* out_idx, float* out_scores, void* stream) {
  if (!c) return PBG_ERR_INVALID;
  TopkState& t = c->tk;
  if (B < 0) return fail(c, PBG_ERR_INVALID, "negative batch");
  if (B == 0) return PBG_OK;
  if (!t.table) return fail(c, PBG_ERR_NOT_LOADED, "topk: no table prepared (pbg_topk_prepare)");
  if (!queries || !out_idx || !out_scores) return fail(c, PBG_ERR_INVALID, "null tensor");
  if (k < 1) return fail(c, PBG_ERR_INVALID, "topk: k must be positive");
  if (k > t.N) return fail(c, PBG_ERR_INVALID, "topk: k = %d exceeds the %lld rows of the table", k, t.N);
  if (k > kTkGeneralMaxK) return fail(c, PBG_ERR_UNSUPPORTED, "topk: k = %d is above the %d this library selects on the device", k, kTkGeneralMaxK);
  PBG_CUDA(c, cudaSetDevice(c->dims.device));
  cudaStream_t s = (cudaStream_t)stream;
  const int E = c->dims.embed_dim;
  const long long kChunk = k > 16 ? 4096 : 16384;
  const int stride = tk_sample_stride(k);
  const bool filter = E == 128 && k <= kTkMaxK && t.N >= std::max<long long>(16 * 256, 64ll * stride * k);
  for (long long off = 0; off < B; off += kChunk) {
    const long long rows = std::min(kChunk, B - off);
    const long long rows_pad = (rows + 255) / 256 * 256;
    const float* q = queries + off * E;
    if (t.q_cap < rows_pad) {
      PBG_TRY(begin_growth(c, s, "the top-k query buffers"));
      t.q_cap = 0;
      PBG_TRY(realloc_dev(c, t.qn, sizeof(__nv_bfloat16) * rows_pad * E));
      PBG_TRY(realloc_dev(c, t.inv_q, sizeof(float) * rows_pad));
      PBG_TRY(realloc_dev(c, t.flag, sizeof(int) * rows_pad));
      PBG_TRY(realloc_dev(c, t.tau, sizeof(float) * rows_pad));
      t.q_cap = rows_pad;
      if (E == 128) PBG_TRY(make_tmap(c, &t.tm_q, t.qn, rows_pad, E, 128));
    }
    { LaunchScope ls(c, PBG_K_OTHER, s);
      const unsigned pg = static_cast<unsigned>(std::min<long long>(c->num_sms * 8, (rows_pad + 7) / 8));
      if (E <= 128) topk_prepare_kernel<8, 1><<<pg, 256, 0, s>>>(q, rows, rows_pad, E, t.qn, t.inv_q);
      else topk_prepare_kernel<2, 4><<<pg, 256, 0, s>>>(q, rows, rows_pad, E, t.qn, t.inv_q); }
    PBG_CUDA(c, cudaGetLastError());
    long long* oi = reinterpret_cast<long long*>(out_idx) + off * k;
    float* os = out_scores + off * k;
    t.last_rows = rows; t.last_filtered = filter;
    if (!filter) {
      PBG_TRY(topk_general(c, t, q, rows, k, oi, os, s));
      continue;
    }
    const int grid = pass_grid(c) & ~1;
    const int npairs = grid / 2;
    const int n_rb = static_cast<int>(rows_pad / 256);
    const int n_tiles = static_cast<int>(t.n_pad / 256);
    auto split = [&](int tiles, TopkParams& p, bool align) {
      p.n_rb = n_rb;
      p.n_tiles = tiles;
      p.total = n_rb * tiles;
      p.span = std::max({1, (p.total + npairs - 1) / npairs, (tiles + kTkMaxRanges - 2) / (kTkMaxRanges - 1)});
      if (align && p.span < tiles) { const int pieces = std::max(1, tiles / p.span); p.span = (tiles + pieces - 1) / pieces; }
      p.n_ranges = 1;
      for (int rb = 0; rb < n_rb; ++rb)
        p.n_ranges = std::max(p.n_ranges, ((rb + 1) * tiles - 1) / p.span - (rb * tiles) / p.span + 1);
    };
    TopkParams ps, pm;
    memset(&ps, 0, sizeof ps); memset(&pm, 0, sizeof pm);
    ps.tm_q = pm.tm_q = t.tm_q; ps.tm_t = pm.tm_t = t.tm_t; ps.N = pm.N = t.N;
    ps.tile_stride = stride; pm.tile_stride = 1;
    split((n_tiles + stride - 1) / stride, ps, true);
    split(n_tiles, pm, false);
    const int n_slists = ps.n_ranges * 2, n_lists = pm.n_ranges * 2;
    const size_t need = static_cast<size_t>(rows_pad) * n_lists * kTkCand;
    const size_t sneed = static_cast<size_t>(rows_pad) * n_slists * kTkKeys;
    if (t.cand_cap < need || t.samp_cap < sneed) {
      PBG_TRY(begin_growth(c, s, "the top-k candidate buffers"));
      t.cand_cap = t.samp_cap = 0;
      PBG_TRY(realloc_dev(c, t.cand_grp, sizeof(unsigned) * need));
      PBG_TRY(realloc_dev(c, t.cand_mask, sizeof(unsigned) * need));
      PBG_TRY(realloc_dev(c, t.cand_cnt, sizeof(int) * need / kTkCand));
      PBG_TRY(realloc_dev(c, t.samp_keys, sizeof(int) * sneed));
      t.cand_cap = need; t.samp_cap = sneed;
    }
    ps.samp_keys = t.samp_keys;
    pm.tau = t.tau; pm.cand_grp = t.cand_grp; pm.cand_mask = t.cand_mask; pm.cand_cnt = t.cand_cnt;
    { LaunchScope ls(c, PBG_K_TOPK, s);
      PBG_CUDA(c, launch_pdl(true, pbg_topk_scan_kernel<TK_SAMPLE>, std::min(grid, 2 * ((ps.total + ps.span - 1) / ps.span)), kPassThreads, TkSmem::kTotal, s, ps)); }
    { LaunchScope ls(c, PBG_K_OTHER, s);
      PBG_CUDA(c, launch_pdl(false, topk_tau_kernel, static_cast<unsigned>((rows_pad + 7) / 8), 256, 0, s, t.samp_keys, n_slists, rows, rows_pad, k, t.tau)); }
    { LaunchScope ls(c, PBG_K_TOPK, s);
      PBG_CUDA(c, launch_pdl(true, pbg_topk_scan_kernel<TK_SCAN>, std::min(grid, 2 * ((pm.total + pm.span - 1) / pm.span)), kPassThreads, TkSmem::kTotal, s, pm)); }
    { LaunchScope ls(c, PBG_K_OTHER, s);
      PBG_CUDA(c, launch_pdl(false, topk_rescore_kernel, static_cast<unsigned>((rows + kTkRescoreWarps - 1) / kTkRescoreWarps), 32 * kTkRescoreWarps, 0, s,
                             q, t.inv_q, t.table, t.inv_t, t.cand_grp, t.cand_mask, t.cand_cnt, t.tau, n_lists, rows, t.N, k, oi, os, t.flag)); }
    {
      LaunchScope ls(c, PBG_K_OTHER, s);
      PBG_CUDA(c, launch_pdl(true, topk_exact_kernel, static_cast<unsigned>(std::min<long long>(rows, 2ll * c->num_sms)), 256,
                             static_cast<size_t>(E * 4 + 256 * k * 8), s, q, t.inv_q, t.table, t.inv_t, t.N, E, k, t.flag, 0, nullptr, oi, os, rows)); }
  }
  return PBG_OK;
}

int64_t pbg_topk_last_flagged(pbg_ctx* c, void* stream) {
  if (!c) return -1;
  TopkState& t = c->tk;
  if (!t.last_filtered || t.last_rows <= 0) return 0;
  if (cudaSetDevice(c->dims.device) != cudaSuccess) return -1;
  std::vector<int> h(static_cast<size_t>(t.last_rows));
  if (cudaMemcpyAsync(h.data(), t.flag, sizeof(int) * h.size(), cudaMemcpyDeviceToHost, (cudaStream_t)stream) != cudaSuccess) return -1;
  if (cudaStreamSynchronize((cudaStream_t)stream) != cudaSuccess) return -1;
  int64_t n = 0, why[5] = {0, 0, 0, 0, 0};
  for (int v : h) { n += v != 0; why[(v >= 0 && v <= 4) ? v : 0] += 1; }
  char buf[160];
  snprintf(buf, sizeof buf, "topk: %lld of %lld rows to the exact scan (list overflow %lld, too many candidates %lld, too few %lld, proof failed %lld)",
           (long long)n, t.last_rows, (long long)why[1], (long long)why[2], (long long)why[3], (long long)why[4]);
  c->err = buf;
  return n;
}

int pbg_set_result_mirrors(pbg_ctx* c, int n, void* const* gen_out, float* const* gen_scores, float* const* logits,
                           float* const* probs) {
  if (!c) return PBG_ERR_INVALID;
  if (n < 0 || n > kMaxMirrors) return fail(c, PBG_ERR_INVALID, "at most %d result mirrors", kMaxMirrors);
  c->n_mirror = n;
  for (int i = 0; i < kMaxMirrors; ++i) {
    c->mir_gen[i] = (i < n && gen_out) ? gen_out[i] : nullptr;
    c->mir_cos[i] = (i < n && gen_scores) ? gen_scores[i] : nullptr;
    c->mir_logits[i] = (i < n && logits) ? logits[i] : nullptr;
    c->mir_probs[i] = (i < n && probs) ? probs[i] : nullptr;
  }
  return PBG_OK;
}

int pbg_set_result_multicast(pbg_ctx* c, void* gen_out_mc, float* gen_scores_mc, float* logits_mc, float* probs_mc) {
  if (!c) return PBG_ERR_INVALID;
  c->mc_gen = gen_out_mc; c->mc_cos = gen_scores_mc; c->mc_logits = logits_mc; c->mc_probs = probs_mc;
  return PBG_OK;
}

int pbg_set_launch_width(pbg_ctx* c, int n_ctas) {
  if (!c) return PBG_ERR_INVALID;
  if (n_ctas < 0) return fail(c, PBG_ERR_INVALID, "launch width must be >= 0");
  c->launch_ctas = n_ctas;
  return PBG_OK;
}

int pbg_last_pass_sm_clock(pbg_ctx* c, void* stream, double* mhz_out) {
  if (!c || !mhz_out) return PBG_ERR_INVALID;
  *mhz_out = 0.0;
  Workspace& w = c->ws_bf16;
  if (!w.sched) return fail(c, PBG_ERR_INVALID, "no bf16-mode pass has run on this ctx");
  PBG_CUDA(c, cudaSetDevice(c->dims.device));
  cudaStream_t s = (cudaStream_t)stream;
  PassSched h;
  PBG_CUDA(c, cudaMemcpyAsync(&h, w.sched, sizeof h, cudaMemcpyDeviceToHost, s));
  PBG_CUDA(c, cudaStreamSynchronize(s));
  if (h.clk_ns > 0) *mhz_out = static_cast<double>(h.clk_ticks) / static_cast<double>(h.clk_ns) * 1e3;
  return PBG_OK;
}

int pbg_set_workspace_discard(pbg_ctx* c, int on) {
  if (!c) return PBG_ERR_INVALID;
  c->discard = on ? 1 : 0;
  return PBG_OK;
}

int pbg_create(pbg_ctx** out, const pbg_dims* dims) {
  if (!out || !dims) return fail(nullptr, PBG_ERR_INVALID, "null argument");
  *out = nullptr;
  const int E = dims->embed_dim, Z = dims->noise_dim, HG = dims->g_hidden, HD = dims->d_hidden;
  if (E <= 0 || Z <= 0 || HG <= 0 || HD <= 0) return fail(nullptr, PBG_ERR_INVALID, "dims must be positive");
  if (!(dims->leaky_slope >= 0.f && dims->leaky_slope <= 1.f))
    return fail(nullptr, PBG_ERR_UNSUPPORTED, "leaky_slope must be in [0, 1]");
  if (E % 8 || Z % 8 || HG % 8 || HD % 16)
    return fail(nullptr, PBG_ERR_UNSUPPORTED, "embed_dim, noise_dim, g_hidden must be multiples of 8 and d_hidden of 16");
  int ndev = 0;
  cudaError_t e = cudaGetDeviceCount(&ndev);
  if (e != cudaSuccess || ndev == 0)
    return fail(nullptr, PBG_ERR_UNSUPPORTED, "no CUDA device (%s); this library has no CPU fallback",
                e == cudaSuccess ? "device count 0" : cudaGetErrorString(e));
  if (dims->device < 0 || dims->device >= ndev) return fail(nullptr, PBG_ERR_INVALID, "device %d out of range", dims->device);
  cudaDeviceProp prop;
  if ((e = cudaGetDeviceProperties(&prop, dims->device)) != cudaSuccess)
    return fail(nullptr, PBG_ERR_CUDA, "cudaGetDeviceProperties: %s", cudaGetErrorString(e));
  if (prop.major != 10)
    return fail(nullptr, PBG_ERR_UNSUPPORTED, "device %d is sm_%d%d; the kernels are sm_100a only (no fallback)",
                dims->device, prop.major, prop.minor);
  pbg_ctx* c = new (std::nothrow) pbg_ctx();
  if (!c) return fail(nullptr, PBG_ERR_NOMEM, "out of host memory");
  c->dims = *dims;
  c->num_sms = prop.multiProcessorCount;
  c->max_threads_sm = prop.maxThreadsPerMultiProcessor;
  if (const char* e = getenv("PBG_DISCARD")) c->discard = atoi(e) != 0;
  if (const char* e = getenv("PBG_HOST_SYNC")) c->host_block = strcmp(e, "block") == 0;
  c->kg0 = 2 * E + Z; c->kg0p = round_up(c->kg0, kBlockK);
  c->kd0 = 3 * E;     c->kd0p = round_up(c->kd0, kBlockK);
  c->hgp = round_up(HG, 128); c->hdp = round_up(HD, 128);
  c->hd2 = HD / 2;
  c->hmax = std::max(c->hgp, c->hdp);
  auto bail = [&](int code) { g_create_error = c->err; pbg_destroy(c); return code; };
  if (cudaSetDevice(dims->device) != cudaSuccess) { c->err = "cudaSetDevice failed"; return bail(PBG_ERR_CUDA); }
  e = cudaSuccess;
  for (Pass2Kernel k : kPass2)
    if (e == cudaSuccess) e = cudaFuncSetAttribute(k, cudaFuncAttributeMaxDynamicSharedMemorySize, P2Smem::kTotal);
  if (e == cudaSuccess) e = cudaFuncSetAttribute(pbg_topk_scan_kernel<TK_SAMPLE>, cudaFuncAttributeMaxDynamicSharedMemorySize, TkSmem::kTotal);
  if (e == cudaSuccess) e = cudaFuncSetAttribute(pbg_topk_scan_kernel<TK_SCAN>, cudaFuncAttributeMaxDynamicSharedMemorySize, TkSmem::kTotal);
  if (e == cudaSuccess) e = cudaFuncSetAttribute(topk_exact_kernel, cudaFuncAttributeMaxDynamicSharedMemorySize, 220 * 1024);
  if (e != cudaSuccess) { c->err = std::string("cudaFuncSetAttribute failed: ") + cudaGetErrorString(e); return bail(PBG_ERR_CUDA); }
  void* fn = nullptr;
  cudaDriverEntryPointQueryResult qres;
  if (cudaGetDriverEntryPoint("cuTensorMapEncodeTiled", &fn, cudaEnableDefault, &qres) != cudaSuccess || !fn) {
    c->err = "cuTensorMapEncodeTiled not available from the driver";
    return bail(PBG_ERR_CUDA);
  }
  c->encode = reinterpret_cast<EncodeTiledFn>(fn);
  if (cudaStreamCreateWithFlags(&c->own_stream, cudaStreamNonBlocking) != cudaSuccess ||
      cudaMalloc(&c->err_flag, sizeof(int)) != cudaSuccess ||
      cudaMemset(c->err_flag, 0, sizeof(int)) != cudaSuccess ||
      cudaMallocHost(&c->err_flag_host, sizeof(int)) != cudaSuccess ||
      cudaMalloc(&c->lat_st, sizeof(LatentStream)) != cudaSuccess ||
      cudaMemset(c->lat_st, 0, sizeof(LatentStream)) != cudaSuccess) {
    c->err = std::string("ctx allocation failed: ") + cudaGetErrorString(cudaGetLastError());
    return bail(PBG_ERR_CUDA);
  }
  *c->err_flag_host = 0;
  *out = c;
  return PBG_OK;
}

void pbg_destroy(pbg_ctx* c) {
  if (!c) return;
  cudaSetDevice(c->dims.device);
  cudaDeviceSynchronize();
  for (auto& l : c->g) free_linear(l);
  for (auto& l : c->d) free_linear(l);
  cudaFree(c->d_w3); cudaFree(c->d_w3_pad);
  free_ws(c->ws_bf16); free_ws(c->ws_f32);
  free_stage(c->stage[0]); free_stage(c->stage[1]);
  cudaFree(c->err_flag); cudaFree(c->trace);
  cudaFree(c->lat_st); cudaFree(c->lat_z);
  cudaFree(c->tk.tn); cudaFree(c->tk.inv_t); cudaFree(c->tk.qn); cudaFree(c->tk.inv_q);
  cudaFree(c->tk.cand_grp); cudaFree(c->tk.cand_mask); cudaFree(c->tk.cand_cnt); cudaFree(c->tk.flag);
  cudaFree(c->tk.samp_keys); cudaFree(c->tk.tau); cudaFree(c->tk.score_buf);

  if (c->err_flag_host) cudaFreeHost(c->err_flag_host);
  if (c->host_evt) cudaEventDestroy(c->host_evt);
  cudaFree(c->st_block);
  if (c->own_stream) cudaStreamDestroy(c->own_stream);
  delete c;
}

int pbg_load_generator(pbg_ctx* c, const float* p, size_t n_floats) {
  if (!c || !p) return PBG_ERR_INVALID;
  const size_t E = c->dims.embed_dim, H = c->dims.g_hidden, K0 = c->kg0;
  const size_t want = H * K0 + H + H * H + H + E * H + E;
  if (n_floats != want) return fail(c, PBG_ERR_INVALID, "generator blob has %zu floats, expected %zu", n_floats, want);
  PBG_CUDA(c, cudaSetDevice(c->dims.device));
  c->g_loaded = false;
  const float* w1 = p;            const float* b1 = w1 + H * K0;
  const float* w2 = b1 + H;       const float* b2 = w2 + H * H;
  const float* w3 = b2 + H;       const float* b3 = w3 + E * H;
  PBG_TRY(upload_linear(c, c->g[0], (int)H, (int)K0, c->kg0p, w1, b1));
  PBG_TRY(upload_linear(c, c->g[1], (int)H, (int)H, c->hgp, w2, b2));
  PBG_TRY(upload_linear(c, c->g[2], (int)E, (int)H, c->hgp, w3, b3));
  c->g_loaded = true;
  return PBG_OK;
}

int pbg_load_discriminator(pbg_ctx* c, const float* p, size_t n_floats) {
  if (!c || !p) return PBG_ERR_INVALID;
  const size_t H = c->dims.d_hidden, H2 = c->hd2, K0 = c->kd0;
  const size_t want = H * K0 + H + H2 * H + H2 + H2 + 1;
  if (n_floats != want) return fail(c, PBG_ERR_INVALID, "discriminator blob has %zu floats, expected %zu", n_floats, want);
  PBG_CUDA(c, cudaSetDevice(c->dims.device));
  c->d_loaded = false;
  const float* w1 = p;            const float* b1 = w1 + H * K0;
  const float* w2 = b1 + H;       const float* b2 = w2 + H2 * H;
  const float* w3 = b2 + H2;      const float* b3 = w3 + H2;
  PBG_TRY(upload_linear(c, c->d[0], (int)H, (int)K0, c->kd0p, w1, b1));
  PBG_TRY(upload_linear(c, c->d[1], (int)H2, (int)H, c->hdp, w2, b2));
  cudaFree(c->d_w3); cudaFree(c->d_w3_pad); c->d_w3 = c->d_w3_pad = nullptr;
  const int np = c->d[1].np;
  PBG_CUDA(c, cudaMalloc(&c->d_w3, sizeof(float) * H2));
  PBG_CUDA(c, cudaMalloc(&c->d_w3_pad, sizeof(float) * np));
  PBG_CUDA(c, cudaMemcpyAsync(c->d_w3, w3, sizeof(float) * H2, cudaMemcpyHostToDevice, c->own_stream));
  { LaunchScope ls(c, PBG_K_OTHER, c->own_stream);
    pad_f32_kernel<<<8, 256, 0, c->own_stream>>>(c->d_w3, c->d_w3_pad, (int)H2, np); }
  PBG_CUDA(c, cudaGetLastError());
  PBG_CUDA(c, cudaStreamSynchronize(c->own_stream));
  c->d_b3 = *b3;
  c->d_loaded = true;
  return PBG_OK;
}

int pbg_generator_forward(pbg_ctx* c, const float* h, const float* r, const float* z, void* out, int64_t B,
                          int precision, int out_dtype, void* stream) {
  if (!c) return PBG_ERR_INVALID;
  if (B > 0 && (!h || !r || !out)) return fail(c, PBG_ERR_INVALID, "null tensor");
  Pass a; a.h = h; a.r = r; a.z = z; a.gen_out = out; a.out_dtype = out_dtype; a.run_g = true;
  a.B = B; a.prec = precision; a.stream = (cudaStream_t)stream;
  return run_pass(c, a);
}

int pbg_generator_forward_gather(pbg_ctx* c, const float* node_emb, int64_t N, const float* rel_emb, int64_t R,
                                 const int64_t* heads, int64_t head_stride, const int64_t* rels, int64_t rel_stride,
                                 const float* z, void* out, int64_t B, int precision, int out_dtype, void* stream) {
  if (!c) return PBG_ERR_INVALID;
  if (B > 0 && (!node_emb || !rel_emb || !heads || !rels || !out)) return fail(c, PBG_ERR_INVALID, "null tensor");
  Pass a; a.node_emb = node_emb; a.N = N; a.rel_emb = rel_emb; a.R = R;
  a.heads = (const long long*)heads; a.hs = head_stride; a.rels = (const long long*)rels; a.rs = rel_stride;
  a.z = z; a.gen_out = out; a.out_dtype = out_dtype; a.run_g = true;
  a.B = B; a.prec = precision; a.stream = (cudaStream_t)stream;
  return run_pass(c, a);
}

int pbg_discriminator_forward(pbg_ctx* c, const float* h, const float* r, const float* t, float* logits, float* probs,
                              int64_t B, int precision, void* stream) {
  if (!c) return PBG_ERR_INVALID;
  if (B > 0 && (!h || !r || !t || !logits)) return fail(c, PBG_ERR_INVALID, "null tensor");
  Pass a; a.h = h; a.r = r; a.t = t; a.logits = logits; a.probs = probs; a.run_d = true;
  a.B = B; a.prec = precision; a.stream = (cudaStream_t)stream;
  return run_pass(c, a);
}

int pbg_discriminator_score_triplets(pbg_ctx* c, const float* node_emb, int64_t N, const float* rel_emb, int64_t R,
                                     const int64_t* triplets, float* logits, float* probs, int64_t B, int precision,
                                     void* stream) {
  return pbg_score_triplets(c, node_emb, N, rel_emb, R, triplets, nullptr, nullptr, PBG_DT_F32, nullptr, logits, probs,
                            B, precision, stream);
}

int pbg_score_triplets(pbg_ctx* c, const float* node_emb, int64_t N, const float* rel_emb, int64_t R,
                       const int64_t* triplets, const float* z, void* gen_out, int out_dtype, float* gen_scores,
                       float* logits, float* probs, int64_t B, int precision, void* stream) {
  if (!c) return PBG_ERR_INVALID;
  if (B > 0 && (!node_emb || !rel_emb || !triplets)) return fail(c, PBG_ERR_INVALID, "null tensor");
  Pass a; a.node_emb = node_emb; a.N = N; a.rel_emb = rel_emb; a.R = R;
  const long long* t = (const long long*)triplets;
  a.heads = t; a.rels = t + 1; a.tails = t + 2; a.hs = a.rs = a.ts = 3;
  a.z = z; a.gen_out = gen_out; a.out_dtype = out_dtype; a.gen_scores = gen_scores;
  a.logits = logits; a.probs = probs;
  a.run_g = (gen_out != nullptr || gen_scores != nullptr); a.run_d = (logits != nullptr);
  a.B = B; a.prec = precision; a.stream = (cudaStream_t)stream;
  return run_pass(c, a);
}

int pbg_reserve(pbg_ctx* c, int64_t rows, int precision, int stage_slots) {
  if (!c) return PBG_ERR_INVALID;
  if (rows <= 0) return fail(c, PBG_ERR_INVALID, "reserve: rows must be positive");
  if (precision != PBG_PREC_F32 && precision != PBG_PREC_BF16) return fail(c, PBG_ERR_INVALID, "unknown precision %d", precision);
  if (stage_slots < 0 || stage_slots > 2) return fail(c, PBG_ERR_INVALID, "reserve: stage_slots must be 0, 1 or 2");
  PBG_CUDA(c, cudaSetDevice(c->dims.device));
  const long long chunk = std::min<long long>(rows, kMaxChunk);
  PBG_TRY(ensure_ws(c, precision, chunk, nullptr));
  PBG_TRY(ensure_latents(c, chunk, nullptr));
  for (int i = 0; i < stage_slots; ++i) PBG_TRY(ensure_stage(c, c->stage[i], chunk, nullptr));
  return PBG_OK;
}

int pbg_draw_latents(pbg_ctx* c, uint64_t seed, uint64_t offset, int64_t total_rows, int64_t row_begin, int64_t rows,
                     float* z_out, uint64_t* offset_after, void* stream) {
  if (!c) return PBG_ERR_INVALID;
  PBG_TRY(check_draw_size(c, total_rows));
  if (row_begin < 0 || rows < 0 || row_begin + rows > total_rows)
    return fail(c, PBG_ERR_INVALID, "latent draw: rows [%lld, %lld) outside the %lld of the draw", (long long)row_begin,
                (long long)(row_begin + rows), (long long)total_rows);
  if (rows > 0 && !z_out) return fail(c, PBG_ERR_INVALID, "null tensor");
  if (offset % 4) return fail(c, PBG_ERR_INVALID, "latent draw: the Philox offset must be a multiple of 4, as torch's");
  PBG_CUDA(c, cudaSetDevice(c->dims.device));
  PBG_TRY(launch_draw(c, seed, offset, nullptr, false, total_rows, row_begin, rows, z_out, (cudaStream_t)stream));
  if (offset_after)
    *offset_after = offset + latent_geometry(total_rows * c->dims.noise_dim, c->num_sms, c->max_threads_sm).inc;
  return PBG_OK;
}

int pbg_set_latent_stream(pbg_ctx* c, int enable, uint64_t seed, uint64_t offset) {
  if (!c) return PBG_ERR_INVALID;
  if (offset % 4) return fail(c, PBG_ERR_INVALID, "latent stream: the Philox offset must be a multiple of 4, as torch's");
  PBG_CUDA(c, cudaSetDevice(c->dims.device));
  PBG_CUDA(c, cudaDeviceSynchronize());
  const LatentStream st{offset, 0u};
  PBG_CUDA(c, cudaMemcpy(c->lat_st, &st, sizeof st, cudaMemcpyHostToDevice));
  c->lat_on = enable != 0;
  c->lat_seed = seed;
  return PBG_OK;
}

int pbg_get_latent_stream(pbg_ctx* c, uint64_t* seed, uint64_t* offset, void* stream) {
  if (!c || !seed || !offset) return PBG_ERR_INVALID;
  PBG_CUDA(c, cudaSetDevice(c->dims.device));
  LatentStream st{};
  PBG_CUDA(c, cudaMemcpyAsync(&st, c->lat_st, sizeof st, cudaMemcpyDeviceToHost, (cudaStream_t)stream));
  PBG_CUDA(c, cudaStreamSynchronize((cudaStream_t)stream));
  *seed = c->lat_seed;
  *offset = st.offset;
  return PBG_OK;
}

namespace {
GatherParams slot_gather(const pbg_ctx* c, const StageSlot& st, const float* node_emb, long long N, const float* rel_emb,
                         long long R, const long long* t, const float* z, long long B, bool gen, bool disc) {
  GatherParams gp{};
  gp.node_emb = node_emb; gp.rel_emb = rel_emb; gp.N = N; gp.R = R; gp.E = c->dims.embed_dim; gp.Z = c->dims.noise_dim;
  gp.heads = t; gp.rels = t + 1; gp.tails = t + 2; gp.head_stride = gp.rel_stride = gp.tail_stride = 3;
  gp.z = z;
  gp.xg = gen ? st.xg0 : nullptr; gp.ldg = c->kg0p;
  gp.xd = disc ? st.xd0 : nullptr; gp.ldd = c->kd0p;
  gp.B = B; gp.err_flag = c->err_flag;
  return gp;
}

int staged_pass(pbg_ctx* c, int slot, void* gen_out, int out_dtype, float* gen_scores, float* logits, float* probs,
                void* stream, Pass& a) {
  if (slot < 0 || slot > 1) return fail(c, PBG_ERR_INVALID, "score_staged: slot must be 0 or 1");
  const StageSlot& st = c->stage[slot];
  if (st.B <= 0) return fail(c, PBG_ERR_INVALID, "score_staged: nothing staged in slot %d", slot);
  a.gen_out = gen_out; a.out_dtype = out_dtype; a.gen_scores = gen_scores; a.logits = logits; a.probs = probs;
  a.run_g = (gen_out != nullptr || gen_scores != nullptr); a.run_d = (logits != nullptr);
  if (a.run_g && !st.has_g) return fail(c, PBG_ERR_INVALID, "score_staged: slot %d holds no generator operands", slot);
  if (a.run_d && !st.has_d) return fail(c, PBG_ERR_INVALID, "score_staged: slot %d holds no discriminator operands", slot);
  a.B = st.B; a.prec = PBG_PREC_BF16; a.stream = (cudaStream_t)stream;
  return PBG_OK;
}
}

int pbg_stage_triplets(pbg_ctx* c, int slot, const float* node_emb, int64_t N, const float* rel_emb, int64_t R,
                       const int64_t* triplets, const float* z, int64_t B, int want_gen, int want_disc, void* stream) {
  if (!c) return PBG_ERR_INVALID;
  if (slot < 0 || slot > 1) return fail(c, PBG_ERR_INVALID, "stage: slot must be 0 or 1");
  if (B <= 0 || B > kMaxChunk) return fail(c, PBG_ERR_INVALID, "stage: B must be in [1, %lld]", kMaxChunk);
  if (!node_emb || !rel_emb || !triplets) return fail(c, PBG_ERR_INVALID, "null tensor");
  if (!want_gen && !want_disc) return fail(c, PBG_ERR_INVALID, "stage: nothing to stage");
  if (want_gen && !c->g_loaded) return fail(c, PBG_ERR_NOT_LOADED, "generator weights not loaded");
  if (want_disc && !c->d_loaded) return fail(c, PBG_ERR_NOT_LOADED, "discriminator weights not loaded");
  if (want_gen && !z && !c->lat_on) return fail(c, PBG_ERR_INVALID, "generator needs latents z");
  PBG_CUDA(c, cudaSetDevice(c->dims.device));
  cudaStream_t s = (cudaStream_t)stream;
  StageSlot& st = c->stage[slot];
  PBG_TRY(ensure_stage(c, st, B, s));
  if (want_gen && !z) {
    PBG_TRY(draw_stream(c, B, st.z, s));
    z = st.z;
  }
  const long long* t = (const long long*)triplets;
  StageParams sp{};
  sp.g = slot_gather(c, st, node_emb, N, rel_emb, R, t, z, B, want_gen != 0, want_disc != 0);
  sp.xt = want_gen ? st.xt : nullptr;
  const int blocks = (int)std::min<long long>((B + 3) / 4, (long long)c->num_sms * 16);
  { LaunchScope ls(c, PBG_K_GATHER, s);
    stage_rows_kernel<<<blocks, 128, 0, s>>>(sp); }
  PBG_CUDA(c, cudaGetLastError());
  st.B = B; st.has_g = want_gen != 0; st.has_d = want_disc != 0; st.has_xt = want_gen != 0;
  st.node_emb = node_emb; st.N = N; st.tails = t + 2;
  return PBG_OK;
}

int pbg_score_staged(pbg_ctx* c, int slot, void* gen_out, int out_dtype, float* gen_scores, float* logits, float* probs,
                     void* stream) {
  if (!c) return PBG_ERR_INVALID;
  Pass a;
  PBG_TRY(staged_pass(c, slot, gen_out, out_dtype, gen_scores, logits, probs, stream, a));
  if (!a.run_g && !a.run_d) return PBG_OK;
  PBG_CUDA(c, cudaSetDevice(c->dims.device));
  PBG_TRY(ensure_ws(c, PBG_PREC_BF16, a.B, a.stream));
  GatherParams gp{};
  return launch_pass2(c, c->ws_bf16, a, gp, 0, a.B, gen_out, gen_scores, true, &c->stage[slot]);
}

int pbg_score_staged_stage_next(pbg_ctx* c, int slot, void* gen_out, int out_dtype, float* gen_scores, float* logits, float* probs,
                                const float* node_emb, int64_t N, const float* rel_emb, int64_t R, const int64_t* next_triplets,
                                const float* next_z, int64_t next_B, void* stream) {
  if (!c) return PBG_ERR_INVALID;
  Pass a;
  PBG_TRY(staged_pass(c, slot, gen_out, out_dtype, gen_scores, logits, probs, stream, a));
  StageSlot& st = c->stage[slot];
  StageSlot& nx = c->stage[1 - slot];
  if (next_B <= 0 || next_B > kMaxChunk) return fail(c, PBG_ERR_INVALID, "stage next: B must be in [1, %lld]", kMaxChunk);
  if (!node_emb || !rel_emb || !next_triplets) return fail(c, PBG_ERR_INVALID, "null tensor");
  if (!a.run_g && !a.run_d) return fail(c, PBG_ERR_INVALID, "score_staged_stage_next: no result requested");
  if (a.run_g && !next_z && !c->lat_on) return fail(c, PBG_ERR_INVALID, "generator needs latents z");
  PBG_CUDA(c, cudaSetDevice(c->dims.device));
  PBG_TRY(ensure_ws(c, PBG_PREC_BF16, a.B, a.stream));
  PBG_TRY(ensure_stage(c, nx, next_B, a.stream));
  if (a.run_g && !next_z) {
    PBG_TRY(draw_stream(c, next_B, nx.z, a.stream));
    next_z = nx.z;
  }
  const long long* t = reinterpret_cast<const long long*>(next_triplets);
  const GatherParams gp = slot_gather(c, nx, node_emb, N, rel_emb, R, t, next_z, next_B, a.run_g, a.run_d);
  PBG_TRY(launch_pass2(c, c->ws_bf16, a, gp, 0, a.B, gen_out, gen_scores, true, &st, true));
  st.B = -1;
  nx.B = next_B; nx.has_g = a.run_g; nx.has_d = a.run_d; nx.has_xt = false;
  nx.node_emb = node_emb; nx.N = N; nx.tails = t + 2;
  return PBG_OK;
}

int pbg_linear_bf16(pbg_ctx* c, int model, int layer, const void* a, void* out, int64_t M, void* stream) {
  if (!c || !a || !out || M <= 0) return c ? fail(c, PBG_ERR_INVALID, "bad argument") : PBG_ERR_INVALID;
  if (model == 0 && !c->g_loaded) return fail(c, PBG_ERR_NOT_LOADED, "generator weights not loaded");
  if (model == 1 && !c->d_loaded) return fail(c, PBG_ERR_NOT_LOADED, "discriminator weights not loaded");
  if (model < 0 || model > 1 || layer < 0 || layer > (model == 0 ? 2 : 1)) return fail(c, PBG_ERR_INVALID, "no such layer");
  if (M > kMaxChunk) return fail(c, PBG_ERR_INVALID, "linear_bf16: at most %lld rows", kMaxChunk);
  PBG_CUDA(c, cudaSetDevice(c->dims.device));
  cudaStream_t s = (cudaStream_t)stream;
  PBG_TRY(ensure_ws(c, PBG_PREC_BF16, M, s));
  Workspace& w = c->ws_bf16;
  static const int kind_of[2][3] = {{IT_G_L0, IT_G_L1, IT_G_L2}, {IT_D_L0, IT_D_L1, -1}};
  const int k = kind_of[model][layer];
  const Linear& l = model == 0 ? c->g[layer] : c->d[layer];
  const bool store = kEpiOf[k] == PEPI_STORE;
  CUtensorMap amap, omap;
  PBG_TRY(make_tmap(c, &amap, a, M, l.kp, kBlockM));
  if (store) PBG_TRY(make_tmap(c, &omap, out, M, l.np, 32));
  Pass2Params p;
  memset(&p, 0, sizeof p);
  set_layer(p, k, l, amap, store ? &omap : nullptr, store ? static_cast<__nv_bfloat16*>(out) : nullptr, l.np);
  const int nrb = static_cast<int>((M + kP2Rows - 1) / kP2Rows);
  p.seg[0] = P2Segment{k, p.layer[k].n_tiles, 0, 0, k, 0};
  p.n_seg = 1; p.n_total = nrb * p.layer[k].n_tiles;
  p.no_deps = 1; p.gather_external = 1; p.phase0_groups = 0;
  p.poll_ns = 40; p.gather_defer = 1;
  p.nrb = nrb; p.rb_cap = w.mb_cap; p.M = static_cast<int>(M); p.slope = c->dims.leaky_slope;
  p.sched = w.sched; p.ready = w.ready; p.fin = w.fin;
  p.part_g = w.part_g; p.part_d = w.part_d;
  if (k == IT_G_L2) {
    p.gen_out = out; p.out_f32 = 1; p.n_valid = c->dims.embed_dim; p.ld_gen = c->dims.embed_dim;
    p.slots_g = (c->dims.embed_dim + 63) / 64;
  }
  if (k == IT_D_L1) {
    if (l.np / 64 > kPartSlotsD) return fail(c, PBG_ERR_UNSUPPORTED, "d_hidden too wide for the partial buffer");
    p.w3 = c->d_w3_pad; p.b3 = c->d_b3; p.logits = static_cast<float*>(out); p.slots_d = l.np / 64;
  }
  p.w3_off = -1;
  const int grid = pass_grid(c) & ~1;
  cudaError_t le;
  { LaunchScope ls(c, model == 0 ? PBG_K_G_L0 + layer : PBG_K_D_L0 + layer, s);
    le = launch_pdl(false, kPass2[0], grid, kP2Threads, P2Smem::kTotal, s, p); }
  if (le == cudaSuccess) le = cudaGetLastError();
  if (le != cudaSuccess) return fail(c, PBG_ERR_CUDA, "single-layer pass launch failed: %s", cudaGetErrorString(le));
  return PBG_OK;
}

int pbg_profile_enable(pbg_ctx* c, int enable) {
  if (!c) return PBG_ERR_INVALID;
  c->profiling = enable != 0;
  return PBG_OK;
}

int pbg_profile_read(pbg_ctx* c, double* ms, int64_t* count) {
  if (!c || !ms || !count) return PBG_ERR_INVALID;
  PBG_CUDA(c, cudaSetDevice(c->dims.device));
  PBG_CUDA(c, cudaDeviceSynchronize());
  for (auto& r : c->prof) {
    float t = 0.f;
    if (cudaEventElapsedTime(&t, r.a, r.b) == cudaSuccess && r.kind >= 0 && r.kind < PBG_NUM_KERNEL_KINDS) {
      ms[r.kind] += t; count[r.kind] += 1;
    }
    cudaEventDestroy(r.a); cudaEventDestroy(r.b);
  }
  c->prof.clear();
  return PBG_OK;
}

int pbg_debug_trace(pbg_ctx* c, int enable, int64_t* host_out, int64_t n_slots) {
  if (!c) return PBG_ERR_INVALID;
  PBG_CUDA(c, cudaSetDevice(c->dims.device));
  PBG_CUDA(c, cudaDeviceSynchronize());
  const size_t n = static_cast<size_t>(c->num_sms) * kTraceSlots;
  if (host_out && c->trace) {
    std::vector<long long> tmp(n);
    PBG_CUDA(c, cudaMemcpy(tmp.data(), c->trace, n * sizeof(long long), cudaMemcpyDeviceToHost));
    for (size_t i = 0; i < n && i < static_cast<size_t>(n_slots); ++i) host_out[i] = tmp[i];
  }
  if (enable && !c->trace) {
    PBG_CUDA(c, cudaMalloc(&c->trace, n * sizeof(long long)));
  } else if (!enable && c->trace) {
    cudaFree(c->trace); c->trace = nullptr;
  }
  if (c->trace) PBG_CUDA(c, cudaMemset(c->trace, 0, n * sizeof(long long)));
  return PBG_OK;
}

int pbg_check_indices(pbg_ctx* c, void* stream) {
  if (!c) return PBG_ERR_INVALID;
  cudaStream_t s = (cudaStream_t)stream;
  PBG_CUDA(c, cudaSetDevice(c->dims.device));
  PBG_CUDA(c, cudaMemcpyAsync(c->err_flag_host, c->err_flag, sizeof(int), cudaMemcpyDeviceToHost, s));
  if (c->host_block) {
    if (!c->host_evt) PBG_CUDA(c, cudaEventCreateWithFlags(&c->host_evt, cudaEventBlockingSync | cudaEventDisableTiming));
    PBG_CUDA(c, cudaEventRecord(c->host_evt, s));
    PBG_CUDA(c, cudaEventSynchronize(c->host_evt));
  } else {
    PBG_CUDA(c, cudaStreamSynchronize(s));
  }
  if (*c->err_flag_host != 0) {
    PBG_CUDA(c, cudaMemsetAsync(c->err_flag, 0, sizeof(int), s));
    PBG_CUDA(c, cudaStreamSynchronize(s));
    return fail(c, PBG_ERR_INDEX, "index out of range in embedding gather");
  }
  return PBG_OK;
}

namespace {
int score_host(pbg_ctx* c, const float* node_emb, int64_t N, const float* rel_emb, int64_t R, const int64_t* triplets_host,
               const float* z_host, float* gen_out_host, float* gen_scores_host, float* logits_host, float* probs_host,
               int64_t B, int precision, bool packed) {
  if (!c) return PBG_ERR_INVALID;
  if (B < 0) return fail(c, PBG_ERR_INVALID, "negative batch");
  if (B == 0) return PBG_OK;
  if (!triplets_host) return fail(c, PBG_ERR_INVALID, "null triplets");
  const bool run_g = gen_out_host || gen_scores_host;
  if (run_g && !z_host && !c->lat_on) return fail(c, PBG_ERR_INVALID, "generator needs latents z");
  PBG_CUDA(c, cudaSetDevice(c->dims.device));
  const int E = c->dims.embed_dim, Z = c->dims.noise_dim;
  cudaStream_t s = c->own_stream;
  if (c->host_cap < B) {
    PBG_TRY(begin_growth(c, s, "the host staging block"));
    c->host_cap = 0;
    const size_t per_row = sizeof(long long) * 3 + sizeof(float) * (Z + 3 + E);
    PBG_TRY(realloc_dev(c, c->st_block, per_row * B + 64));
    c->host_cap = B;
  }
  auto up16 = [](size_t v) { return (v + 15) & ~static_cast<size_t>(15); };
  char* b0 = c->st_block;
  size_t off = 0;
  long long* trip = reinterpret_cast<long long*>(b0 + off);  off = up16(off + sizeof(long long) * 3 * B);
  float* z = reinterpret_cast<float*>(b0 + off);             off += sizeof(float) * Z * B;
  float* scores = reinterpret_cast<float*>(b0 + off);        off += sizeof(float) * B;
  float* logits = reinterpret_cast<float*>(b0 + off);        off += sizeof(float) * B;
  float* probs = reinterpret_cast<float*>(b0 + off);         off = up16(off + sizeof(float) * B);
  float* gen = reinterpret_cast<float*>(b0 + off);
  const bool one_h2d = packed && z_host && reinterpret_cast<char*>(z) == reinterpret_cast<char*>(trip) + sizeof(long long) * 3 * B;
  if (one_h2d) {
    PBG_CUDA(c, cudaMemcpyAsync(trip, triplets_host, sizeof(long long) * 3 * B + sizeof(float) * Z * B, cudaMemcpyHostToDevice, s));
  } else {
    PBG_CUDA(c, cudaMemcpyAsync(trip, triplets_host, sizeof(long long) * 3 * B, cudaMemcpyHostToDevice, s));
    if (run_g && z_host) PBG_CUDA(c, cudaMemcpyAsync(z, z_host, sizeof(float) * Z * B, cudaMemcpyHostToDevice, s));
  }
  PBG_TRY(pbg_score_triplets(c, node_emb, N, rel_emb, R, (const int64_t*)trip, run_g && z_host ? z : nullptr,
                             gen_out_host ? gen : nullptr, PBG_DT_F32, gen_scores_host ? scores : nullptr,
                             logits_host ? logits : nullptr, probs_host ? probs : nullptr, B, precision, s));
  if (packed) {
    PBG_CUDA(c, cudaMemcpyAsync(gen_scores_host, scores, sizeof(float) * 3 * B, cudaMemcpyDeviceToHost, s));
  } else {
    if (gen_scores_host) PBG_CUDA(c, cudaMemcpyAsync(gen_scores_host, scores, sizeof(float) * B, cudaMemcpyDeviceToHost, s));
// ... 36 lines not shown
```

pro-b-gan_b200/pbg/cabi.py:

```python
from __future__ import annotations

import ctypes as C
from pathlib import Path

from . import build as _build

PBG_OK, PBG_ERR_INVALID, PBG_ERR_CUDA, PBG_ERR_NOT_LOADED, PBG_ERR_INDEX, PBG_ERR_UNSUPPORTED, PBG_ERR_NOMEM = range(7)
PREC_F32, PREC_BF16 = 0, 1
DT_F32, DT_BF16 = 0, 1
KERNEL_KINDS = ("gather", "g_l0", "g_l1", "g_l2", "d_l0", "d_l1", "other", "pass", "topk")

SYMBOLS = (
    "pbg_abi_version", "pbg_create", "pbg_destroy", "pbg_last_error", "pbg_load_generator",
    "pbg_load_discriminator", "pbg_generator_forward", "pbg_generator_forward_gather",
    "pbg_discriminator_forward", "pbg_discriminator_score_triplets", "pbg_score_triplets",
    "pbg_score_triplets_host", "pbg_linear_bf16", "pbg_profile_enable", "pbg_profile_read", "pbg_debug_trace", "pbg_check_indices", "pbg_launch_count",
    "pbg_set_launch_width", "pbg_set_result_mirrors", "pbg_topk_prepare", "pbg_topk", "pbg_parse_index_rows", "pbg_format_f32_json", "pbg_format_i64_json",
    "pbg_reserve", "pbg_stage_triplets", "pbg_score_staged", "pbg_set_result_multicast", "pbg_topk_last_flagged", "pbg_score_triplets_host_packed", "pbg_score_staged_stage_next", "pbg_set_workspace_discard", "pbg_last_pass_sm_clock",
    "pbg_draw_latents", "pbg_set_latent_stream", "pbg_get_latent_stream", "pbg_score_triplets_host_ids",
)


class PbgDims(C.Structure):
    _fields_ = [("embed_dim", C.c_int32), ("noise_dim", C.c_int32), ("g_hidden", C.c_int32),
                ("d_hidden", C.c_int32), ("device", C.c_int32), ("leaky_slope", C.c_float)]


class PbgError(RuntimeError):
    def __init__(self, status: int, message: str):
        super().__init__(f"libpbg_b200 status {status}: {message}")
        self.status = status


_lib = None


def lib_path() -> Path:
    return _build.LIB_PATH


def load() -> C.CDLL:
    global _lib
    if _lib is not None:
        return _lib
    import os
    override = os.environ.get("PBG_LIB_PATH")
    path = Path(override) if override else _build.build()
    lib = C.CDLL(str(path))
    vp, i64, i32, sz, u64 = C.c_void_p, C.c_int64, C.c_int, C.c_size_t, C.c_uint64
    sig = {
        "pbg_abi_version": (C.c_int, []),
        "pbg_create": (C.c_int, [C.POINTER(vp), C.POINTER(PbgDims)]),
        "pbg_destroy": (None, [vp]),
        "pbg_last_error": (C.c_char_p, [vp]),
        "pbg_load_generator": (C.c_int, [vp, vp, sz]),
        "pbg_load_discriminator": (C.c_int, [vp, vp, sz]),
        "pbg_generator_forward": (C.c_int, [vp, vp, vp, vp, vp, i64, i32, i32, vp]),
        "pbg_generator_forward_gather": (C.c_int, [vp, vp, i64, vp, i64, vp, i64, vp, i64, vp, vp, i64, i32, i32, vp]),
        "pbg_discriminator_forward": (C.c_int, [vp, vp, vp, vp, vp, vp, i64, i32, vp]),
        "pbg_discriminator_score_triplets": (C.c_int, [vp, vp, i64, vp, i64, vp, vp, vp, i64, i32, vp]),
        "pbg_score_triplets": (C.c_int, [vp, vp, i64, vp, i64, vp, vp, vp, i32, vp, vp, vp, i64, i32, vp]),
        "pbg_score_triplets_host": (C.c_int, [vp, vp, i64, vp, i64, vp, vp, vp, vp, vp, vp, i64, i32]),
        "pbg_linear_bf16": (C.c_int, [vp, i32, i32, vp, vp, i64, vp]),
        "pbg_profile_enable": (C.c_int, [vp, i32]),
        "pbg_profile_read": (C.c_int, [vp, vp, vp]),
        "pbg_debug_trace": (C.c_int, [vp, i32, vp, i64]),
        "pbg_check_indices": (C.c_int, [vp, vp]),
        "pbg_launch_count": (i64, [vp]),
        "pbg_set_launch_width": (C.c_int, [vp, i32]),
        "pbg_set_workspace_discard": (C.c_int, [vp, i32]),
        "pbg_last_pass_sm_clock": (C.c_int, [vp, vp, C.POINTER(C.c_double)]),
        "pbg_set_result_mirrors": (C.c_int, [vp, i32, vp, vp, vp, vp]),
        "pbg_topk_prepare": (C.c_int, [vp, vp, i64, vp]),
        "pbg_topk": (C.c_int, [vp, vp, i64, i32, vp, vp, vp]),
        "pbg_parse_index_rows": (i64, [C.c_char_p, sz, i32, vp, sz]),
        "pbg_format_f32_json": (i64, [vp, sz, i32, i32, i32, vp, sz]),
        "pbg_format_i64_json": (i64, [vp, sz, i32, i32, i32, vp, sz]),
        "pbg_reserve": (C.c_int, [vp, i64, i32, i32]),
        "pbg_stage_triplets": (C.c_int, [vp, i32, vp, i64, vp, i64, vp, vp, i64, i32, i32, vp]),
        "pbg_score_staged": (C.c_int, [vp, i32, vp, i32, vp, vp, vp, vp]),
        "pbg_set_result_multicast": (C.c_int, [vp, vp, vp, vp, vp]),
        "pbg_topk_last_flagged": (i64, [vp, vp]),
        "pbg_score_triplets_host_packed": (C.c_int, [vp, vp, i64, vp, i64, vp, vp, i64, i32]),
        "pbg_score_staged_stage_next": (C.c_int, [vp, i32, vp, i32, vp, vp, vp, vp, i64, vp, i64, vp, vp, i64, vp]),
        "pbg_draw_latents": (C.c_int, [vp, u64, u64, i64, i64, i64, vp, C.POINTER(u64), vp]),
        "pbg_set_latent_stream": (C.c_int, [vp, i32, u64, u64]),
        "pbg_get_latent_stream": (C.c_int, [vp, C.POINTER(u64), C.POINTER(u64), vp]),
        "pbg_score_triplets_host_ids": (C.c_int, [vp, vp, i64, vp, i64, vp, vp, i64, i32]),
    }
    for name, (res, args) in sig.items():
        fn = getattr(lib, name)
        fn.restype, fn.argtypes = res, args
    _lib = lib
    return lib


def last_error(handle) -> str:
    msg = load().pbg_last_error(handle)
    return msg.decode("utf-8", "replace") if msg else ""


def check(status: int, handle=None) -> None:
    if status == PBG_OK:
        return
    msg = last_error(handle)
    if status == PBG_ERR_INDEX:
        raise IndexError(msg or "index out of range in embedding gather")
    raise PbgError(status, msg)
```

pro-b-gan_b200/pbg/engine.py:

```python
from __future__ import annotations

import ctypes as C
import os

import torch
import torch.nn as nn

from . import cabi

_PRECISIONS = {"fp32": cabi.PREC_F32, "f32": cabi.PREC_F32, "float32": cabi.PREC_F32,
               "bf16": cabi.PREC_BF16, "bfloat16": cabi.PREC_BF16}


def default_precision() -> str:
    return os.environ.get("PBG_PRECISION", "bf16").lower()


def precision_code(precision: str | None) -> int:
    p = (precision or default_precision()).lower()
    if p not in _PRECISIONS:
        raise ValueError(f"unknown precision {p!r}; use 'fp32' or 'bf16'")
    return _PRECISIONS[p]


def fold_linear_bn(lin: nn.Linear, bn: nn.BatchNorm1d | None):
    W = lin.weight.detach().double().cpu()
    b = lin.bias.detach().double().cpu() if lin.bias is not None else torch.zeros(W.shape[0], dtype=torch.float64)
    if bn is not None:
        s = bn.weight.detach().double().cpu() / torch.sqrt(bn.running_var.detach().double().cpu() + bn.eps)
        W = W * s[:, None]
        b = (b - bn.running_mean.detach().double().cpu()) * s + bn.bias.detach().double().cpu()
    return W.float().contiguous(), b.float().contiguous()


def _ptr(t: torch.Tensor | None):
    return C.c_void_p(t.data_ptr()) if t is not None else C.c_void_p(0)


class Engine:

    def __init__(self, embed_dim: int, noise_dim: int, g_hidden: int, d_hidden: int,
                 device: torch.device | str | int, leaky_slope: float = 0.2, ctas: int = 0):
        device = torch.device(device)
        if device.type != "cuda":
            raise RuntimeError(f"pro-b-gan_b200 runs only on CUDA (sm_100a) devices, got {device}; there is no CPU fallback")
        if not torch.cuda.is_available():
            raise RuntimeError("pro-b-gan_b200: no CUDA device is available and there is no CPU fallback")
        self.device = torch.device("cuda", device.index if device.index is not None else torch.cuda.current_device())
        self.E, self.Z, self.HG, self.HD = int(embed_dim), int(noise_dim), int(g_hidden), int(d_hidden)
        self._lib = cabi.load()
        self._h = C.c_void_p(0)
        dims = cabi.PbgDims(self.E, self.Z, self.HG, self.HD, self.device.index, float(leaky_slope))
        st = self._lib.pbg_create(C.byref(self._h), C.byref(dims))
        if st != cabi.PBG_OK:
            self._h = C.c_void_p(0)
            cabi.check(st, None)
        self.g_loaded = self.d_loaded = False
        self._latent_on = False
        if ctas:
            self.set_launch_width(ctas)

    def set_launch_width(self, ctas: int) -> None:
        cabi.check(self._lib.pbg_set_launch_width(self._h, int(ctas)), self._h)

    def last_pass_sm_clock(self) -> float:
        import ctypes
        mhz = ctypes.c_double(0.0)
        with torch.cuda.device(self.device):
            cabi.check(self._lib.pbg_last_pass_sm_clock(self._h, self._stream(), ctypes.byref(mhz)), self._h)
        return float(mhz.value)

    def set_workspace_discard(self, on: bool) -> None:
        cabi.check(self._lib.pbg_set_workspace_discard(self._h, int(bool(on))), self._h)

    def cosine_topk(self, queries: torch.Tensor, table: torch.Tensor, k: int):
        table = self._f32(table, self.E, "table")
        queries = self._f32(queries, self.E, "queries")
        self.validate_top_k(k, table.shape[0])
        key = (table.data_ptr(), tuple(table.shape), table._version)
        with torch.cuda.device(self.device):
            if getattr(self, "_topk_key", None) != key:
                cabi.check(self._lib.pbg_topk_prepare(self._h, _ptr(table), table.shape[0], self._stream()), self._h)
                self._topk_key, self._topk_table = key, table
            B = queries.shape[0]
            scores = torch.empty(B, k, dtype=torch.float32, device=self.device)
            idx = torch.empty(B, k, dtype=torch.int64, device=self.device)
            cabi.check(self._lib.pbg_topk(self._h, _ptr(queries), B, int(k), _ptr(idx), _ptr(scores), self._stream()), self._h)
        return scores, idx

    def topk_last_flagged(self) -> int:
        n = int(self._lib.pbg_topk_last_flagged(self._h, self._stream()))
        self.topk_flag_report = cabi.last_error(self._h)
        return n

    MAX_TOP_K = 512

    @classmethod
    def validate_top_k(cls, k: int, num_rows: int) -> None:
        if k > num_rows:
            raise RuntimeError(f"selected index k out of range: k = {k} > {num_rows} rows")
        if k < 1:
            raise RuntimeError(f"top_k must be positive, got {k}")
        if k > cls.MAX_TOP_K:
            raise NotImplementedError(f"top_k = {k}: the CUDA path selects at most {cls.MAX_TOP_K} per row "
                                      "(k <= 64 on the tensor-core filter, above that exact fp32 scores + selection)")

    def set_result_mirrors(self, gen_out=(), gen_scores=(), logits=(), probs=()) -> None:
        n = max(len(gen_out), len(gen_scores), len(logits), len(probs))
        def arr(ptrs):
            if not ptrs:
                return None
            if len(ptrs) != n:
                raise ValueError("every given mirror list must have the same length")
            return (C.c_void_p * n)(*[C.c_void_p(int(x)) for x in ptrs])
        a = [arr(gen_out), arr(gen_scores), arr(logits), arr(probs)]
        cabi.check(self._lib.pbg_set_result_mirrors(self._h, n, *[C.cast(x, C.c_void_p) if x is not None else None for x in a]),
                   self._h)

    def set_result_multicast(self, gen_out: int = 0, gen_scores: int = 0, logits: int = 0, probs: int = 0) -> None:
        cabi.check(self._lib.pbg_set_result_multicast(self._h, *[C.c_void_p(int(x)) if x else None
                                                                 for x in (gen_out, gen_scores, logits, probs)]), self._h)

    def __del__(self):
        h = getattr(self, "_h", None)
        if h is not None and h.value:
            try:
                self._lib.pbg_destroy(h)
            except Exception:
                pass
            self._h = C.c_void_p(0)

    def load_generator(self, layers) -> None:
        blob = torch.cat([t.reshape(-1).float().cpu() for wb in layers for t in wb]).contiguous()
        cabi.check(self._lib.pbg_load_generator(self._h, C.c_void_p(blob.data_ptr()), blob.numel()), self._h)
        self.g_loaded = True

    def load_discriminator(self, layers) -> None:
        blob = torch.cat([t.reshape(-1).float().cpu() for wb in layers for t in wb]).contiguous()
        cabi.check(self._lib.pbg_load_discriminator(self._h, C.c_void_p(blob.data_ptr()), blob.numel()), self._h)
        self.d_loaded = True

    def _stream(self):
        return C.c_void_p(torch.cuda.current_stream(self.device).cuda_stream)

    def _f32(self, t: torch.Tensor, cols: int, name: str) -> torch.Tensor:
        if t.device != self.device:
            raise RuntimeError(f"{name} is on {t.device}, engine is on {self.device}")
        if t.dim() != 2 or t.shape[1] != cols:
            raise ValueError(f"{name} must be [B, {cols}], got {tuple(t.shape)}")
        return t.detach().to(torch.float32).contiguous()

    def _i64(self, t: torch.Tensor, name: str) -> torch.Tensor:
        if t.device != self.device:
            raise RuntimeError(f"{name} is on {t.device}, engine is on {self.device}")
        return t.detach().to(torch.int64)

    def check_indices(self) -> None:
        cabi.check(self._lib.pbg_check_indices(self._h, self._stream()), self._h)

    def profile_enable(self, on: bool = True) -> None:
        cabi.check(self._lib.pbg_profile_enable(self._h, 1 if on else 0), self._h)

    def profile_read(self) -> dict:
        n = len(cabi.KERNEL_KINDS)
        ms = (C.c_double * n)(*([0.0] * n))
        cnt = (C.c_int64 * n)(*([0] * n))
        cabi.check(self._lib.pbg_profile_read(self._h, ms, cnt), self._h)
        return {k: (ms[i], cnt[i]) for i, k in enumerate(cabi.KERNEL_KINDS)}

    def debug_trace(self, enable: bool = True):
        n = torch.cuda.get_device_properties(self.device).multi_processor_count * 256
        buf = (C.c_int64 * n)()
        cabi.check(self._lib.pbg_debug_trace(self._h, 1 if enable else 0, buf, n), self._h)
        return torch.tensor(list(buf), dtype=torch.int64).reshape(-1, 256)

    @property
    def launch_count(self) -> int:
        return int(self._lib.pbg_launch_count(self._h))

    def set_latent_stream(self, enable: bool = True, seed: int = 0, offset: int = 0) -> None:
        with torch.cuda.device(self.device):
            cabi.check(self._lib.pbg_set_latent_stream(self._h, int(bool(enable)), int(seed), int(offset)), self._h)
        self._latent_on = bool(enable)

    def latent_stream(self) -> tuple[int, int]:
        seed, off = C.c_uint64(0), C.c_uint64(0)
        with torch.cuda.device(self.device):
            cabi.check(self._lib.pbg_get_latent_stream(self._h, C.byref(seed), C.byref(off), self._stream()), self._h)
        return int(seed.value), int(off.value)

    def draw_latents(self, rows: int, seed: int, offset: int, row_begin: int = 0,
                     total_rows: int | None = None) -> tuple[torch.Tensor, int]:
        total = int(rows if total_rows is None else total_rows)
        z = torch.empty(int(rows), self.Z, dtype=torch.float32, device=self.device)
        after = C.c_uint64(0)
        with torch.cuda.device(self.device):
            cabi.check(self._lib.pbg_draw_latents(self._h, int(seed), int(offset), total, int(row_begin), int(rows), _ptr(z),
                                                  C.byref(after), self._stream()), self._h)
        return z, int(after.value)

    def _latents(self, z, name: str = "z"):
        if z is not None:
            return self._f32(z, self.Z, name)
        if not self._latent_on:
            raise ValueError("generator pass needs latents z (or the ctx's latent stream: set_latent_stream)")
        return None

    def generator_forward(self, h, r, z=None, precision=None, out_dtype=torch.float32) -> torch.Tensor:
        h, r, z = self._f32(h, self.E, "h_emb"), self._f32(r, self.E, "r_emb"), self._latents(z)
        B = h.shape[0]
        if r.shape[0] != B or (z is not None and z.shape[0] != B):
            raise ValueError("h_emb, r_emb and z must have the same batch size")
        out = torch.empty(B, self.E, dtype=out_dtype, device=self.device)
        with torch.cuda.device(self.device):
            cabi.check(self._lib.pbg_generator_forward(
                self._h, _ptr(h), _ptr(r), _ptr(z), _ptr(out), B, precision_code(precision),
                cabi.DT_BF16 if out_dtype == torch.bfloat16 else cabi.DT_F32, self._stream()), self._h)
        return out

    def generator_forward_gather(self, node_emb, rel_w, heads, rels, z=None, precision=None,
                                 out_dtype=torch.float32) -> torch.Tensor:
        node_emb = self._f32(node_emb, self.E, "node_emb")
        rel_w = self._f32(rel_w, self.E, "rel_emb.weight")
        heads, rels = self._i64(heads, "heads"), self._i64(rels, "relations")
        z = self._latents(z)
        B = heads.shape[0]
        out = torch.empty(B, self.E, dtype=out_dtype, device=self.device)
        with torch.cuda.device(self.device):
            cabi.check(self._lib.pbg_generator_forward_gather(
                self._h, _ptr(node_emb), node_emb.shape[0], _ptr(rel_w), rel_w.shape[0],
                _ptr(heads), heads.stride(0) if B else 1, _ptr(rels), rels.stride(0) if B else 1, _ptr(z), _ptr(out),
                B, precision_code(precision), cabi.DT_BF16 if out_dtype == torch.bfloat16 else cabi.DT_F32,
                self._stream()), self._h)
        return out

    def discriminator_forward(self, h, r, t, precision=None):
        h, r, t = self._f32(h, self.E, "h_emb"), self._f32(r, self.E, "r_emb"), self._f32(t, self.E, "t_emb")
        B = h.shape[0]
        logits = torch.empty(B, dtype=torch.float32, device=self.device)
        probs = torch.empty(B, dtype=torch.float32, device=self.device)
        with torch.cuda.device(self.device):
            cabi.check(self._lib.pbg_discriminator_forward(
                self._h, _ptr(h), _ptr(r), _ptr(t), _ptr(logits), _ptr(probs), B, precision_code(precision),
                self._stream()), self._h)
        return logits, probs

    def linear_bf16(self, model: int, layer: int, a_bf16: torch.Tensor) -> torch.Tensor:
        if a_bf16.dtype != torch.bfloat16 or a_bf16.device != self.device or not a_bf16.is_contiguous():
            raise ValueError("a_bf16 must be a contiguous bf16 tensor on the engine's device")
        M = a_bf16.shape[0]
        if model == 0 and layer == 2:
            out = torch.empty(M, self.E, dtype=torch.float32, device=self.device)
        elif model == 1 and layer == 1:
            out = torch.empty(M, dtype=torch.float32, device=self.device)
        else:
            width = (self.HG if model == 0 else self.HD)
            out = torch.empty(M, (width + 127) // 128 * 128, dtype=torch.bfloat16, device=self.device)
        with torch.cuda.device(self.device):
            cabi.check(self._lib.pbg_linear_bf16(self._h, model, layer, _ptr(a_bf16), _ptr(out), M, self._stream()),
                       self._h)
        return out

    def score_triplets(self, node_emb, rel_w, triplets, z=None, want_gen_out=False, want_gen_scores=False,
                       want_disc=True, precision=None, out_dtype=torch.float32, out: dict | None = None):
        node_emb = self._f32(node_emb, self.E, "node_emb")
        rel_w = self._f32(rel_w, self.E, "rel_emb.weight")
        trip = self._i64(triplets, "triplets")
        if trip.dim() != 2 or trip.shape[1] != 3:
            raise ValueError(f"triplets must be [B, 3], got {tuple(trip.shape)}")
        trip = trip.contiguous()
        B = trip.shape[0]
        run_g = want_gen_out or want_gen_scores
        if run_g:
            z = self._latents(z)
        res = {}
        out = out or {}

        def buf(key, want, shape, dtype):
            if not want:
                return None
            t = out.get(key)
            if t is None:
                return torch.empty(shape, dtype=dtype, device=self.device)
            if tuple(t.shape) != tuple(shape) or t.dtype != dtype or t.device != self.device or not t.is_contiguous():
                raise ValueError(f"out[{key!r}] must be a contiguous {dtype} tensor of shape {tuple(shape)} on {self.device}")
            return t

        gen_out = buf("gen_out", want_gen_out, (B, self.E), out_dtype)
        scores = buf("gen_scores", want_gen_scores, (B,), torch.float32)
        logits = buf("logits", want_disc, (B,), torch.float32)
        probs = buf("probs", want_disc, (B,), torch.float32)
        with torch.cuda.device(self.device):
            cabi.check(self._lib.pbg_score_triplets(
                self._h, _ptr(node_emb), node_emb.shape[0], _ptr(rel_w), rel_w.shape[0], _ptr(trip),
                _ptr(z if run_g else None), _ptr(gen_out),
                cabi.DT_BF16 if out_dtype == torch.bfloat16 else cabi.DT_F32,
                _ptr(scores), _ptr(logits), _ptr(probs), B, precision_code(precision), self._stream()), self._h)
        if want_gen_out:
            res["gen_out"] = gen_out
        if want_gen_scores:
            res["gen_scores"] = scores
        if want_disc:
            res["logits"], res["probs"] = logits, probs
        return res

    def reserve(self, rows: int, precision=None, stage_slots: int = 0) -> None:
        with torch.cuda.device(self.device):
            cabi.check(self._lib.pbg_reserve(self._h, int(rows), precision_code(precision), int(stage_slots)), self._h)

    def stage_triplets(self, slot: int, node_emb, rel_w, triplets, z=None, want_gen=True, want_disc=True) -> int:
        node_emb = self._f32(node_emb, self.E, "node_emb")
        rel_w = self._f32(rel_w, self.E, "rel_emb.weight")
        trip = self._i64(triplets, "triplets")
        if trip.dim() != 2 or trip.shape[1] != 3:
            raise ValueError(f"triplets must be [B, 3], got {tuple(trip.shape)}")
        trip = trip.contiguous()
        if want_gen:
            z = self._latents(z)
        B = trip.shape[0]
        with torch.cuda.device(self.device):
            cabi.check(self._lib.pbg_stage_triplets(
                self._h, int(slot), _ptr(node_emb), node_emb.shape[0], _ptr(rel_w), rel_w.shape[0], _ptr(trip),
                _ptr(z if want_gen else None), B, 1 if want_gen else 0, 1 if want_disc else 0, self._stream()), self._h)
        if not hasattr(self, "_staged_rows"):
            self._staged_rows = {}
        self._staged_rows[int(slot)] = B
        return B

    def score_staged(self, slot: int, want_gen_out=False, want_gen_scores=False, want_disc=True,
                     out_dtype=torch.float32, out: dict | None = None, stage_next: tuple | None = None):
        res, out = {}, (out or {})
        B = getattr(self, "_staged_rows", {}).get(int(slot))
        if B is None:
            raise ValueError(f"nothing staged in slot {slot}")

        def buf(key, want, shape, dtype):
            if not want:
                return None
            t = out.get(key)
            if t is None:
                return torch.empty(shape, dtype=dtype, device=self.device)
            if tuple(t.shape) != tuple(shape) or t.dtype != dtype or t.device != self.device or not t.is_contiguous():
                raise ValueError(f"out[{key!r}] must be a contiguous {dtype} tensor of shape {tuple(shape)} on {self.device}")
            return t

        gen_out = buf("gen_out", want_gen_out, (B, self.E), out_dtype)
        scores = buf("gen_scores", want_gen_scores, (B,), torch.float32)
        logits = buf("logits", want_disc, (B,), torch.float32)
        probs = buf("probs", want_disc, (B,), torch.float32)
        dt = cabi.DT_BF16 if out_dtype == torch.bfloat16 else cabi.DT_F32
        with torch.cuda.device(self.device):
            if stage_next is None:
                cabi.check(self._lib.pbg_score_staged(self._h, int(slot), _ptr(gen_out), dt, _ptr(scores), _ptr(logits),
                                                      _ptr(probs), self._stream()), self._h)
            else:
                n_emb, n_rel, n_trip, n_z = stage_next
                n_emb, n_rel = self._f32(n_emb, self.E, "node_emb"), self._f32(n_rel, self.E, "rel_emb.weight")
                n_trip = self._i64(n_trip, "triplets")
                if n_trip.dim() != 2 or n_trip.shape[1] != 3 or not n_trip.is_contiguous():
                    raise ValueError("the next request's triplets must be a contiguous [B, 3] tensor")
                run_g = want_gen_out or want_gen_scores
                if run_g:
                    n_z = self._latents(n_z)
                cabi.check(self._lib.pbg_score_staged_stage_next(
                    self._h, int(slot), _ptr(gen_out), dt, _ptr(scores), _ptr(logits), _ptr(probs), _ptr(n_emb), n_emb.shape[0],
                    _ptr(n_rel), n_rel.shape[0], _ptr(n_trip), _ptr(n_z if run_g else None), n_trip.shape[0], self._stream()),
                    self._h)
                self._staged_rows.pop(int(slot), None)
                self._staged_rows[1 - int(slot)] = n_trip.shape[0]
                if not hasattr(self, "_staged_keep"):
                    self._staged_keep = {}
                self._staged_keep[1 - int(slot)] = (n_emb, n_rel, n_trip, n_z)
        if want_gen_out:
            res["gen_out"] = gen_out
        if want_gen_scores:
            res["gen_scores"] = scores
        if want_disc:
            res["logits"], res["probs"] = logits, probs
        return res

    def score_triplets_host(self, node_emb, rel_w, triplets_host, z_host=None, gen_out_host=None,
                            gen_scores_host=None, logits_host=None, probs_host=None, precision=None) -> None:
        for name, t in (("triplets", triplets_host), ("z", z_host), ("gen_out", gen_out_host),
                        ("gen_scores", gen_scores_host), ("logits", logits_host), ("probs", probs_host)):
            if t is not None and (t.device.type != "cpu" or not t.is_contiguous()):
                raise ValueError(f"{name}_host must be a contiguous CPU tensor")
        if triplets_host.dtype != torch.int64 or triplets_host.dim() != 2 or triplets_host.shape[1] != 3:
            raise ValueError("triplets_host must be int64 [B, 3]")
        B = triplets_host.shape[0]
        with torch.cuda.device(self.device):
            cabi.check(self._lib.pbg_score_triplets_host(
                self._h, _ptr(node_emb), node_emb.shape[0], _ptr(rel_w), rel_w.shape[0], _ptr(triplets_host),
                _ptr(z_host), _ptr(gen_out_host), _ptr(gen_scores_host), _ptr(logits_host), _ptr(probs_host),
                B, precision_code(precision)), self._h)

    def score_triplets_host_packed(self, node_emb, rel_w, in_block_host: torch.Tensor, out_block_host: torch.Tensor,
                                   B: int, precision=None) -> None:
        if in_block_host.device.type != "cpu" or out_block_host.device.type != "cpu":
            raise ValueError("the blocks must be CPU (ideally pinned) tensors")
        if in_block_host.numel() * in_block_host.element_size() != B * (24 + 4 * self.Z) or not in_block_host.is_contiguous():
            raise ValueError(f"in_block_host must hold {B * (24 + 4 * self.Z)} contiguous bytes")
        if out_block_host.dtype != torch.float32 or out_block_host.numel() != 3 * B or not out_block_host.is_contiguous():
            raise ValueError(f"out_block_host must be a contiguous fp32 tensor of {3 * B} elements")
        with torch.cuda.device(self.device):
            cabi.check(self._lib.pbg_score_triplets_host_packed(
                self._h, _ptr(node_emb), node_emb.shape[0], _ptr(rel_w), rel_w.shape[0], _ptr(in_block_host),
                _ptr(out_block_host), B, precision_code(precision)), self._h)

    def score_triplets_host_ids(self, node_emb, rel_w, triplets_host: torch.Tensor, out_block_host: torch.Tensor,
                                precision=None) -> None:
        if triplets_host.device.type != "cpu" or out_block_host.device.type != "cpu":
            raise ValueError("the blocks must be CPU (ideally pinned) tensors")
        if triplets_host.dtype != torch.int64 or triplets_host.dim() != 2 or triplets_host.shape[1] != 3 \
                or not triplets_host.is_contiguous():
            raise ValueError("triplets_host must be a contiguous int64 [B, 3] tensor")
        B = triplets_host.shape[0]
        if out_block_host.dtype != torch.float32 or out_block_host.numel() != 3 * B or not out_block_host.is_contiguous():
            raise ValueError(f"out_block_host must be a contiguous fp32 tensor of {3 * B} elements")
        if not self._latent_on:
            raise ValueError("score_triplets_host_ids draws the latents on the device: call set_latent_stream first")
        with torch.cuda.device(self.device):
            cabi.check(self._lib.pbg_score_triplets_host_ids(
                self._h, _ptr(node_emb), node_emb.shape[0], _ptr(rel_w), rel_w.shape[0], _ptr(triplets_host),
                _ptr(out_block_host), B, precision_code(precision)), self._h)
```

pro-b-gan_b200/pbg/inference.py:

```python
from __future__ import annotations

import os
import time
from typing import Any, Dict

import numpy as np
import torch

from . import hostio
from .analyze import analyze_relations_batched


class FusedInference:
    def __init__(self, checkpoint_path: str, device: str = "auto", precision: str | None = None, verbose: bool = False,
                 latents: str | None = None):
        import modular_prot_b_gan as m
        if device in ("auto", "cuda"):
            if not torch.cuda.is_available():
                raise RuntimeError("pro-b-gan_b200 has no CPU path: a CUDA (sm_100a) device is required")
            self.device = torch.device("cuda", torch.cuda.current_device())
        else:
            self.device = torch.device(device)
            if self.device.type != "cuda":
                raise RuntimeError(f"device {device!r}: pro-b-gan_b200 has no CPU path")
        self.checkpoint_path = checkpoint_path
        self.precision = precision
        if not os.path.exists(checkpoint_path):
            raise FileNotFoundError(f"Checkpoint not found: {checkpoint_path}")
        t0 = time.perf_counter()
        ckpt = torch.load(checkpoint_path, map_location="cpu")
        t1 = time.perf_counter()
        args = ckpt.get("args", {})
        if not isinstance(args, dict):
            args = vars(args)
        self.embed_dim = args.get("embed_dim", 128)
        self.noise_dim = args.get("noise_dim", 64)
        self.hidden_dim = args.get("hidden_dim", 1024)
        self.node_emb = ckpt["node_emb"].detach().to(self.device, torch.float32).contiguous()
        self.rel_weight = ckpt["rel_emb"]["weight"].detach().to(self.device, torch.float32).contiguous()
        self.num_entities, self.num_relations = int(self.node_emb.shape[0]), int(self.rel_weight.shape[0])
        self.generator = m.ModularGenerator(self.embed_dim, self.noise_dim)
        self.discriminator = m.ModularDiscriminator(self.embed_dim, self.hidden_dim)
        self.generator.load_state_dict(ckpt["generator"])
        self.discriminator.load_state_dict(ckpt["discriminator"])
        self.generator.to(self.device).eval()
        self.discriminator.to(self.device).eval()
        self.generator.precision = self.discriminator.precision = precision
        t2 = time.perf_counter()
        self.engine = m.make_fused_engine(self.generator, self.discriminator)
        self.latents = m.latent_source(latents)
        if self.latents == "cuda":
            self.engine.set_latent_stream(True, m.LATENT_SEED, 0)
        torch.cuda.synchronize(self.device)
        t3 = time.perf_counter()
        self.best_val_hit10 = ckpt.get("best_val_hit10", 0.0)
        self.best_epoch = ckpt.get("best_epoch", 0)
        self.training_history = ckpt.get("training_history", {})
        self.ingest_ms = {"torch_load": (t1 - t0) * 1e3, "tables_and_modules": (t2 - t1) * 1e3,
                          "fold_pack_upload": (t3 - t2) * 1e3}
        self._pinned: Dict[str, torch.Tensor] = {}
        if verbose:
            print(f"FusedInference ready: {self.num_entities:,} entities, {self.num_relations:,} relations, "
                  f"E={self.embed_dim}; ingest {self.ingest_ms}")

    def reseed(self, seed: int | None = None) -> None:
        import modular_prot_b_gan as m
        seed = m.LATENT_SEED if seed is None else int(seed)
        self.generator.reseed(seed)
        if self.latents == "cuda":
            self.engine.set_latent_stream(True, seed, 0)

    def _pin(self, name: str, rows: int, shape_tail: tuple, dtype) -> torch.Tensor:
        buf = self._pinned.get(name)
        if buf is None or buf.shape[0] < rows or buf.dtype != dtype or tuple(buf.shape[1:]) != tuple(shape_tail):
            cap = max(256, 1 << max(rows - 1, 1).bit_length())
            buf = self._pinned[name] = torch.empty((cap, *shape_tail), dtype=dtype, pin_memory=True)
        return buf[:rows]

    def _stage_rows(self, name: str, x, cols: int) -> torch.Tensor:
        rows = hostio.index_rows(x, cols)
        buf = self._pin(name, rows.shape[0], (cols,), torch.int64)
        buf.copy_(rows)
        return buf

    def _latents(self, batch: int) -> torch.Tensor:
        buf = self._pin("z", batch, (self.noise_dim,), torch.float32)
        if batch:
            torch.randn(batch, self.noise_dim, generator=self.generator._latent_gen, dtype=torch.float32, out=buf)
        return buf

    @staticmethod
    def _echo(x, rows: torch.Tensor, flat: bool = False):
        if isinstance(x, (list, tuple)):
            return x
        return rows[:, 0].tolist() if flat else rows.tolist()

    def score_triplets(self, triplets, method: str = "both", as_arrays: bool = False) -> Dict[str, Any]:
        trip = self._stage_rows("trip", triplets, 3)
        B = trip.shape[0]
        out = (lambda t: t.numpy().copy()) if as_arrays else (lambda t: t.tolist())
        results: Dict[str, Any] = {
            "triplets": trip.numpy().copy() if as_arrays else self._echo(triplets, trip),
            "metadata": {"num_triplets": B, "method": method, "model_hit10": self.best_val_hit10},
        }
        if B == 0:
            raise IndexError("too many indices for tensor of dimension 1")
        run_g, run_d = method in ("generator", "both"), method in ("discriminator", "both")
        if not (run_g or run_d):
            return results
        if self.latents == "cuda" and run_g and run_d:
            block = self._pin("out_block", 3 * B, (), torch.float32)
            scores, logits, probs = block[:B], block[B:2 * B], block[2 * B:]
            with torch.cuda.device(self.device):
                self.engine.score_triplets_host_ids(self.node_emb, self.rel_weight, trip, block, precision=self.precision)
        else:
            z = self._latents(B) if run_g and self.latents == "cpu" else None
            scores = self._pin("gen_scores", B, (), torch.float32) if run_g else None
            logits = self._pin("logits", B, (), torch.float32) if run_d else None
            probs = self._pin("probs", B, (), torch.float32) if run_d else None
            with torch.cuda.device(self.device):
                self.engine.score_triplets_host(self.node_emb, self.rel_weight, trip, z, None, scores, logits, probs,
                                                precision=self.precision)
        if run_g:
            results["generator_scores"] = out(scores)
        if run_d:
            results["discriminator_logits"] = out(logits)
            results["discriminator_probabilities"] = out(probs)
        return results

    def predict_tails(self, head_relation_pairs, top_k: int = 10, return_scores: bool = False,
                      as_arrays: bool = False) -> Dict[str, Any]:
        pairs = self._stage_rows("pairs", head_relation_pairs, 2)
        out = (lambda t: t.cpu().numpy()) if as_arrays else (lambda t: t.tolist())
        B = pairs.shape[0]
        self.engine.validate_top_k(top_k, self.num_entities)
        with torch.no_grad(), torch.cuda.device(self.device):
            try:
                dev_pairs = pairs.to(self.device, non_blocking=True)
                z = self._latents(B).to(self.device, non_blocking=True) if self.latents == "cpu" else None
                pred = self.engine.generator_forward_gather(self.node_emb, self.rel_weight, dev_pairs[:, 0], dev_pairs[:, 1],
                                                            z, precision=self.precision)
                top_scores, top_idx = self.engine.cosine_topk(pred, self.node_emb, top_k)
                self.engine.check_indices()
            except BaseException:
                torch.cuda.current_stream(self.device).synchronize()
                raise
            results: Dict[str, Any] = {
                "predictions": out(top_idx),
                "metadata": {"num_queries": B, "top_k": top_k, "model_hit10": self.best_val_hit10},
            }
            if return_scores:
                results["scores"] = out(top_scores)
        return results

    def find_similar_entities(self, entity_ids, top_k: int = 10) -> Dict[str, Any]:
        ids = hostio.index_rows(entity_ids, 1)[:, 0]
        if ids.numel() and (int(ids.min()) < -self.num_entities or int(ids.max()) >= self.num_entities):
            raise IndexError(f"index out of range for node_emb with {self.num_entities} rows")
        echo = entity_ids if isinstance(entity_ids, (list, tuple)) else ids.tolist()
        results: Dict[str, Any] = {
            "similar_entities": [],
            "metadata": {"num_queries": int(ids.numel()), "top_k": top_k, "model_hit10": self.best_val_hit10},
        }
        self.engine.validate_top_k(top_k + 1, self.num_entities)
        with torch.no_grad(), torch.cuda.device(self.device):
            q = self.node_emb[ids.to(self.device)]
            top_scores, top_idx = self.engine.cosine_topk(q, self.node_emb, top_k + 1)
            top_scores, top_idx = top_scores.cpu().numpy(), top_idx.cpu().numpy()
        for i, query_id in enumerate(echo):
            keep = top_idx[i] != query_id
            results["similar_entities"].append({
                "query_entity": query_id,
                "similar_entities": top_idx[i][keep][:top_k].tolist(),
                "similarity_scores": top_scores[i][keep][:top_k].tolist(),
            })
        return results

    def analyze_relations(self, head_entities, tail_entities, top_k: int = 5) -> Dict[str, Any]:
        heads = hostio.index_rows(head_entities, 1)[:, 0]
        tails = hostio.index_rows(tail_entities, 1)[:, 0]
        res = analyze_relations_batched(self.discriminator, self.node_emb, self.rel_weight, heads.tolist(),
                                        tails.tolist(), top_k, self.best_val_hit10)
        if isinstance(head_entities, (list, tuple)) and isinstance(tail_entities, (list, tuple)):
            it = iter(res["relation_analysis"])
            for h in head_entities:
                for t in tail_entities:
                    e = next(it)
                    e["head_entity"], e["tail_entity"] = h, t
        return res

    def get_model_info(self) -> Dict[str, Any]:
        return {
            "model_architecture": {"embedding_dim": self.embed_dim, "noise_dim": self.noise_dim,
                                   "hidden_dim": self.hidden_dim, "num_entities": self.num_entities,
                                   "num_relations": self.num_relations},
            "training_performance": {"best_validation_hit10": self.best_val_hit10, "best_epoch": self.best_epoch},
            "checkpoint_path": self.checkpoint_path,
            "device": str(self.device),
        }
```

Baseline: 178.1 million.

## Fold relation embeddings into first-layer weights via one-hot relation inputs

Precomputes W_r·rel_emb for every relation and stores it as extra columns of the generator and discriminator first-layer weights, in bf16. The gather then writes a one-hot relation vector padded to Rp instead of loading and storing the E-wide relation embedding row. This removes one embedding gather per row and changes the first-layer K from E to Rp. It only pays off when the number of relations is small. It adds a weight re-fold whenever the relation table changes, a cache keyed on tensor version, and slightly different rounding because the product is pre-multiplied.

```diff
diff --git a/include/pbg.h b/include/pbg.h
--- a/include/pbg.h
+++ b/include/pbg.h
@@ -131,6 +131,8 @@
 int pbg_set_result_multicast(pbg_ctx* ctx, void* gen_out_mc, float* gen_scores_mc, float* logits_mc, float* probs_mc);
 
 int pbg_topk_prepare(pbg_ctx* ctx, const float* table, int64_t N, void* stream);
+
+int pbg_prepare_relations(pbg_ctx* ctx, const float* rel_emb, int64_t R, void* stream);
 int pbg_topk(pbg_ctx* ctx, const float* queries, int64_t B, int k, int64_t* out_idx, float* out_scores, void* stream);
 int64_t pbg_topk_last_flagged(pbg_ctx* ctx, void* stream);
 
diff --git a/pro-b-gan_b200/csrc/gather.cuh b/pro-b-gan_b200/csrc/gather.cuh
--- a/pro-b-gan_b200/csrc/gather.cuh
+++ b/pro-b-gan_b200/csrc/gather.cuh
@@ -18,7 +18,19 @@
   void* xd; int ldd;
   long long B;
   int* err_flag;
+  int fold;
+  int Rp;
 };
+
+__device__ __forceinline__ uint4 onehot8(int v, long long r) {
+  const long long j = r - 8ll * v;
+  uint4 w;
+  w.x = (j == 0 ? 0x3f80u : 0u) | (j == 1 ? 0x3f800000u : 0u);
+  w.y = (j == 2 ? 0x3f80u : 0u) | (j == 3 ? 0x3f800000u : 0u);
+  w.z = (j == 4 ? 0x3f80u : 0u) | (j == 5 ? 0x3f800000u : 0u);
+  w.w = (j == 6 ? 0x3f80u : 0u) | (j == 7 ? 0x3f800000u : 0u);
+  return w;
+}
 
 template <typename T>
 __device__ __forceinline__ void store4(T* dst, float4 v);
@@ -50,10 +62,12 @@
   const int E4 = p.E >> 2, Z4 = p.Z >> 2;
   T* xg = static_cast<T*>(p.xg);
   T* xd = static_cast<T*>(p.xd);
+  const int rw = p.fold ? 0 : p.E;
 
   for (long long b = warp_global; b < p.B; b += num_warps) {
     const float *hrow, *rrow, *trow = nullptr;
     bool bad = false;
+    long long ri = 0;
     if (p.heads != nullptr) {
       long long i = p.heads[b * p.head_stride];
       if (i < 0) i += p.N;
@@ -63,9 +77,9 @@
       hrow = p.h + b * p.E;
     }
     if (p.rels != nullptr) {
-      long long i = p.rels[b * p.rel_stride];
-      if (i < 0 || i >= p.R) { bad = true; i = 0; }
-      rrow = p.rel_emb + i * p.E;
+      ri = p.rels[b * p.rel_stride];
+      if (ri < 0 || ri >= p.R) { bad = true; ri = 0; }
+      rrow = p.rel_emb + ri * p.E;
     } else {
       rrow = p.r + b * p.E;
     }
@@ -83,22 +97,27 @@
     T* d = xd ? xd + b * p.ldd : nullptr;
     for (int v = lane; v < E4; v += 32) {
       const float4 hv = ld_stream4(hrow + 4 * v);
-      const float4 rv = ld_stream4(rrow + 4 * v);
-      if (g) { store4<T>(g + 4 * v, hv); store4<T>(g + p.E + 4 * v, rv); }
+      const float4 rv = p.fold ? hv : ld_stream4(rrow + 4 * v);
+      if (g) { store4<T>(g + 4 * v, hv); if (!p.fold) store4<T>(g + p.E + 4 * v, rv); }
       if (d) {
         store4<T>(d + 4 * v, hv);
-        store4<T>(d + p.E + 4 * v, rv);
-        store4<T>(d + 2 * p.E + 4 * v, ld_stream4(trow + 4 * v));
-      }
+        if (!p.fold) store4<T>(d + p.E + 4 * v, rv);
+        store4<T>(d + p.E + rw + 4 * v, ld_stream4(trow + 4 * v));
+      }
+    }
+    const int oh = p.fold ? p.Rp : 0;
+    for (int v = lane; v < oh / 8; v += 32) {
+      if (g) *reinterpret_cast<uint4*>(g + p.E + p.Z + 8 * v) = onehot8(v, ri);
+      if (d) *reinterpret_cast<uint4*>(d + 2 * p.E + 8 * v) = onehot8(v, ri);
     }
     if (g) {
       const float* zrow = p.z + b * p.Z;
-      for (int v = lane; v < Z4; v += 32) store4<T>(g + 2 * p.E + 4 * v, ld_stream4(zrow + 4 * v));
-      for (int v = (2 * p.E + p.Z) / 4 + lane; v < p.ldg / 4; v += 32)
+      for (int v = lane; v < Z4; v += 32) store4<T>(g + p.E + rw + 4 * v, ld_stream4(zrow + 4 * v));
+      for (int v = (p.E + rw + p.Z + oh) / 4 + lane; v < p.ldg / 4; v += 32)
         store4<T>(g + 4 * v, make_float4(0.f, 0.f, 0.f, 0.f));
     }
     if (d) {
-      for (int v = (3 * p.E) / 4 + lane; v < p.ldd / 4; v += 32)
+      for (int v = (2 * p.E + rw + oh) / 4 + lane; v < p.ldd / 4; v += 32)
         store4<T>(d + 4 * v, make_float4(0.f, 0.f, 0.f, 0.f));
     }
   }
@@ -113,6 +132,7 @@
   const long long warp_global = (static_cast<long long>(blockIdx.x) * blockDim.x + threadIdx.x) >> 5;
   const long long num_warps = (static_cast<long long>(gridDim.x) * blockDim.x) >> 5;
   const int E = sp.g.E, Z = sp.g.Z, E4 = E >> 2, Z4 = Z >> 2;
+  const int rw = sp.g.fold ? 0 : E;
   const long long N = sp.g.N;
   __nv_bfloat16* const xg = static_cast<__nv_bfloat16*>(sp.g.xg);
   __nv_bfloat16* const xd = static_cast<__nv_bfloat16*>(sp.g.xd);
@@ -132,26 +152,31 @@
     __nv_bfloat16* d = xd ? xd + b * sp.g.ldd : nullptr;
     for (int v = lane; v < E4; v += 32) {
       const float4 hv = ld_stream4(hrow + 4 * v);
-      const float4 rv = ld_stream4(rrow + 4 * v);
+      const float4 rv = sp.g.fold ? hv : ld_stream4(rrow + 4 * v);
       const float4 tv = ld_stream4(trow + 4 * v);
       if (g) {
         store4<__nv_bfloat16>(g + 4 * v, hv);
-        store4<__nv_bfloat16>(g + E + 4 * v, rv);
+        if (!sp.g.fold) store4<__nv_bfloat16>(g + E + 4 * v, rv);
       }
       if (d) {
         store4<__nv_bfloat16>(d + 4 * v, hv);
-        store4<__nv_bfloat16>(d + E + 4 * v, rv);
-        store4<__nv_bfloat16>(d + 2 * E + 4 * v, tv);
+        if (!sp.g.fold) store4<__nv_bfloat16>(d + E + 4 * v, rv);
+        store4<__nv_bfloat16>(d + E + rw + 4 * v, tv);
       }
       if (sp.xt) store4<float>(sp.xt + b * E + 4 * v, tv);
     }
+    const int oh = sp.g.fold ? sp.g.Rp : 0;
+    for (int v = lane; v < oh / 8; v += 32) {
+      if (g) *reinterpret_cast<uint4*>(g + E + Z + 8 * v) = onehot8(v, ri);
+      if (d) *reinterpret_cast<uint4*>(d + 2 * E + 8 * v) = onehot8(v, ri);
+    }
     if (g) {
-      for (int v = lane; v < Z4; v += 32) store4<__nv_bfloat16>(g + 2 * E + 4 * v, ld_stream4(sp.g.z + b * Z + 4 * v));
-      for (int v = (2 * E + Z) / 4 + lane; v < sp.g.ldg / 4; v += 32)
+      for (int v = lane; v < Z4; v += 32) store4<__nv_bfloat16>(g + E + rw + 4 * v, ld_stream4(sp.g.z + b * Z + 4 * v));
+      for (int v = (E + rw + Z + oh) / 4 + lane; v < sp.g.ldg / 4; v += 32)
         store4<__nv_bfloat16>(g + 4 * v, make_float4(0.f, 0.f, 0.f, 0.f));
     }
     if (d)
-      for (int v = (3 * E) / 4 + lane; v < sp.g.ldd / 4; v += 32)
+      for (int v = (2 * E + rw + oh) / 4 + lane; v < sp.g.ldd / 4; v += 32)
         store4<__nv_bfloat16>(d + 4 * v, make_float4(0.f, 0.f, 0.f, 0.f));
   }
 }
@@ -166,6 +191,33 @@
   }
 }
 
+__global__ void fold_weight_kernel(const float* __restrict__ w, int n, int k, int E, const float* __restrict__ rel, int R,
+                                   __nv_bfloat16* __restrict__ out, int np, int kp) {
+  const int X = k - 2 * E;
+  const long long total = static_cast<long long>(np) * kp;
+  for (long long i = static_cast<long long>(blockIdx.x) * blockDim.x + threadIdx.x; i < total;
+       i += static_cast<long long>(gridDim.x) * blockDim.x) {
+    const int row = static_cast<int>(i / kp), col = static_cast<int>(i % kp);
+    float v = 0.f;
+    if (row < n) {
+      const float* wr = w + static_cast<long long>(row) * k;
+      if (col < E) {
+        v = wr[col];
+      } else if (col < E + X) {
+        v = wr[E + col];
+      } else if (col < E + X + R) {
+        const float* rr = rel + static_cast<long long>(col - E - X) * E;
+        double acc = 0.0;
+        for (int j = 0; j < E; ++j)
+          acc += static_cast<double>(__bfloat162float(__float2bfloat16_rn(wr[E + j]))) *
+                 static_cast<double>(__bfloat162float(__float2bfloat16_rn(rr[j])));
+        v = static_cast<float>(acc);
+      }
+    }
+    out[i] = __float2bfloat16_rn(v);
+  }
+}
+
 __global__ void pad_f32_kernel(const float* __restrict__ src, float* __restrict__ dst, int n, int n_p) {
   for (int i = blockIdx.x * blockDim.x + threadIdx.x; i < n_p; i += gridDim.x * blockDim.x)
     dst[i] = i < n ? src[i] : 0.f;
diff --git a/pro-b-gan_b200/csrc/pass2_kernel.cuh b/pro-b-gan_b200/csrc/pass2_kernel.cuh
--- a/pro-b-gan_b200/csrc/pass2_kernel.cuh
+++ b/pro-b-gan_b200/csrc/pass2_kernel.cuh
@@ -226,6 +226,7 @@
   __nv_bfloat16* xd = static_cast<__nv_bfloat16*>(g.xd);
   const float* src = nullptr;
   bool bad = false;
+  long long rid = 0;
   if (lane < 12) {
     const long long row = r0 + lane / 3;
     const int which = lane % 3;
@@ -234,8 +235,11 @@
         if (g.heads) { long long i = g.heads[row * g.head_stride]; if (i < 0) i += g.N; if (i < 0 || i >= g.N) { bad = true; i = 0; } src = g.node_emb + i * g.E; }
         else src = g.h + row * g.E;
       } else if (which == 1) {
-        if (g.rels) { long long i = g.rels[row * g.rel_stride]; if (i < 0 || i >= g.R) { bad = true; i = 0; } src = g.rel_emb + i * g.E; }
-        else src = g.r + row * g.E;
+        if (g.rels) {
+          long long i = g.rels[row * g.rel_stride]; if (i < 0 || i >= g.R) { bad = true; i = 0; }
+          if (g.fold) rid = i;
+          else src = g.rel_emb + i * g.E;
+        } else src = g.r + row * g.E;
       } else if (g.tails) {
         long long i = g.tails[row * g.tail_stride]; if (i < 0) i += g.N; if (i < 0 || i >= g.N) { bad = true; i = 0; } src = g.node_emb + i * g.E;
       } else if (xd != nullptr) {
@@ -246,8 +250,13 @@
   if (bad) atomicOr(g.err_flag, 1);
   const unsigned long long sp = reinterpret_cast<unsigned long long>(src);
   const int Z4 = g.Z >> 2;
-  const int wg = 2 * g.E + g.Z, wd = 3 * g.E;
+  const int rw = g.fold ? 0 : g.E;
+  const int oh = g.fold ? g.Rp : 0;
+  const int wg = g.E + rw + g.Z + oh, wd = 2 * g.E + rw + oh;
   float4 hv[4], rv[4], tv[4], zv[4];
+  long long rr[4];
+#pragma unroll
+  for (int j = 0; j < 4; ++j) rr[j] = __shfl_sync(0xffffffffu, rid, j * 3 + 1);
 #pragma unroll
   for (int j = 0; j < 4; ++j) {
     const float* ph = reinterpret_cast<const float*>(__shfl_sync(0xffffffffu, sp, j * 3 + 0));
@@ -257,7 +266,7 @@
     hv[j] = rv[j] = tv[j] = zv[j] = make_float4(0.f, 0.f, 0.f, 0.f);
     if (row < g.B) {
       hv[j] = ld_stream4(ph + 4 * lane);
-      rv[j] = ld_stream4(pr + 4 * lane);
+      if (!g.fold) rv[j] = ld_stream4(pr + 4 * lane);
       if (xd != nullptr) tv[j] = ld_stream4(pt + 4 * lane);
       if (xg != nullptr && lane < Z4) zv[j] = ld_stream4(g.z + row * g.Z + 4 * lane);
     }
@@ -269,8 +278,9 @@
     for (int j = 0; j < 4; ++j) {
       __nv_bfloat16* o = reinterpret_cast<__nv_bfloat16*>(st) + j * wg;
       store4<__nv_bfloat16>(o + 4 * lane, hv[j]);
-      store4<__nv_bfloat16>(o + g.E + 4 * lane, rv[j]);
-      if (lane < Z4) store4<__nv_bfloat16>(o + 2 * g.E + 4 * lane, zv[j]);
+      if (!g.fold) store4<__nv_bfloat16>(o + g.E + 4 * lane, rv[j]);
+      if (lane < Z4) store4<__nv_bfloat16>(o + g.E + rw + 4 * lane, zv[j]);
+      if (lane < oh / 8) *reinterpret_cast<uint4*>(o + g.E + g.Z + 8 * lane) = onehot8(lane, rr[j]);
     }
     fence_proxy_async_smem();
     __syncwarp();
@@ -287,8 +297,9 @@
     for (int j = 0; j < 4; ++j) {
       __nv_bfloat16* o = reinterpret_cast<__nv_bfloat16*>(st) + j * wd;
       store4<__nv_bfloat16>(o + 4 * lane, hv[j]);
-      store4<__nv_bfloat16>(o + g.E + 4 * lane, rv[j]);
-      store4<__nv_bfloat16>(o + 2 * g.E + 4 * lane, tv[j]);
+      if (!g.fold) store4<__nv_bfloat16>(o + g.E + 4 * lane, rv[j]);
+      store4<__nv_bfloat16>(o + g.E + rw + 4 * lane, tv[j]);
+      if (lane < oh / 8) *reinterpret_cast<uint4*>(o + 2 * g.E + 8 * lane) = onehot8(lane, rr[j]);
     }
     fence_proxy_async_smem();
     __syncwarp();
diff --git a/pro-b-gan_b200/csrc/pass_common.cuh b/pro-b-gan_b200/csrc/pass_common.cuh
--- a/pro-b-gan_b200/csrc/pass_common.cuh
+++ b/pro-b-gan_b200/csrc/pass_common.cuh
@@ -80,6 +80,7 @@
   __nv_bfloat16* xd = static_cast<__nv_bfloat16*>(g.xd);
   const float* src = nullptr;
   bool bad = false;
+  long long rid = 0;
   if (lane < 12) {
     const long long row = r0 + lane / 3;
     const int which = lane % 3;
@@ -88,8 +89,11 @@
         if (g.heads) { long long i = g.heads[row * g.head_stride]; if (i < 0) i += g.N; if (i < 0 || i >= g.N) { bad = true; i = 0; } src = g.node_emb + i * g.E; }
         else src = g.h + row * g.E;
       } else if (which == 1) {
-        if (g.rels) { long long i = g.rels[row * g.rel_stride]; if (i < 0 || i >= g.R) { bad = true; i = 0; } src = g.rel_emb + i * g.E; }
-        else src = g.r + row * g.E;
+        if (g.rels) {
+          long long i = g.rels[row * g.rel_stride]; if (i < 0 || i >= g.R) { bad = true; i = 0; }
+          if (g.fold) rid = i;
+          else src = g.rel_emb + i * g.E;
+        } else src = g.r + row * g.E;
       } else if (g.tails) {
         long long i = g.tails[row * g.tail_stride]; if (i < 0) i += g.N; if (i < 0 || i >= g.N) { bad = true; i = 0; } src = g.node_emb + i * g.E;
       } else if (xd != nullptr) {
@@ -100,6 +104,17 @@
   if (bad) atomicOr(g.err_flag, 1);
   const unsigned long long sp = reinterpret_cast<unsigned long long>(src);
   const int E4 = g.E >> 2, Z4 = g.Z >> 2;
+  const int rw = g.fold ? 0 : g.E;
+  const int oh = g.fold ? g.Rp : 0;
+  for (int j = 0; j < 4; ++j) {
+    const long long r = __shfl_sync(0xffffffffu, rid, j * 3 + 1);
+    const long long row = r0 + j;
+    if (row >= g.B) continue;
+    for (int v = lane; v < oh / 8; v += 32) {
+      if (xg != nullptr) *reinterpret_cast<uint4*>(xg + row * g.ldg + g.E + g.Z + 8 * v) = onehot8(v, r);
+      if (xd != nullptr) *reinterpret_cast<uint4*>(xd + row * g.ldd + 2 * g.E + 8 * v) = onehot8(v, r);
+    }
+  }
   if (MODE == 1 || (MODE == 0 && E4 == 32 && Z4 <= 32)) {
     float4 hv[4], rv[4], tv[4], zv[4];
 #pragma unroll
@@ -111,7 +126,7 @@
       hv[j] = rv[j] = tv[j] = zv[j] = make_float4(0.f, 0.f, 0.f, 0.f);
       if (row < g.B) {
         hv[j] = ld_stream4(ph + 4 * lane);
-        rv[j] = ld_stream4(pr + 4 * lane);
+        if (!g.fold) rv[j] = ld_stream4(pr + 4 * lane);
         if (xd != nullptr) tv[j] = ld_stream4(pt + 4 * lane);
         if (xg != nullptr && lane < Z4) zv[j] = ld_stream4(g.z + row * g.Z + 4 * lane);
       }
@@ -123,17 +138,17 @@
       if (xg != nullptr) {
         __nv_bfloat16* o = xg + row * g.ldg;
         store4<__nv_bfloat16>(o + 4 * lane, hv[j]);
-        store4<__nv_bfloat16>(o + g.E + 4 * lane, rv[j]);
-        if (lane < Z4) store4<__nv_bfloat16>(o + 2 * g.E + 4 * lane, zv[j]);
-        for (int v = (2 * g.E + g.Z) / 4 + lane; v < g.ldg / 4; v += 32)
+        if (!g.fold) store4<__nv_bfloat16>(o + g.E + 4 * lane, rv[j]);
+        if (lane < Z4) store4<__nv_bfloat16>(o + g.E + rw + 4 * lane, zv[j]);
+        for (int v = (g.E + rw + g.Z + oh) / 4 + lane; v < g.ldg / 4; v += 32)
           store4<__nv_bfloat16>(o + 4 * v, make_float4(0.f, 0.f, 0.f, 0.f));
       }
       if (xd != nullptr) {
         __nv_bfloat16* o = xd + row * g.ldd;
         store4<__nv_bfloat16>(o + 4 * lane, hv[j]);
-        store4<__nv_bfloat16>(o + g.E + 4 * lane, rv[j]);
-        store4<__nv_bfloat16>(o + 2 * g.E + 4 * lane, tv[j]);
-        for (int v = (3 * g.E) / 4 + lane; v < g.ldd / 4; v += 32)
+        if (!g.fold) store4<__nv_bfloat16>(o + g.E + 4 * lane, rv[j]);
+        store4<__nv_bfloat16>(o + g.E + rw + 4 * lane, tv[j]);
+        for (int v = (2 * g.E + rw + oh) / 4 + lane; v < g.ldd / 4; v += 32)
           store4<__nv_bfloat16>(o + 4 * v, make_float4(0.f, 0.f, 0.f, 0.f));
       }
     }
@@ -147,21 +162,23 @@
       __nv_bfloat16* og = xg ? xg + row * g.ldg : nullptr;
       __nv_bfloat16* od = xd ? xd + row * g.ldd : nullptr;
       for (int v = lane; v < E4; v += 32) {
-        const float4 h4 = ld_stream4(ph + 4 * v), r4 = ld_stream4(pr + 4 * v);
-        if (og) { store4<__nv_bfloat16>(og + 4 * v, h4); store4<__nv_bfloat16>(og + g.E + 4 * v, r4); }
-        if (od) {
-          store4<__nv_bfloat16>(od + 4 * v, h4);
-          store4<__nv_bfloat16>(od + g.E + 4 * v, r4);
-          store4<__nv_bfloat16>(od + 2 * g.E + 4 * v, ld_stream4(pt + 4 * v));
+        const float4 h4 = ld_stream4(ph + 4 * v);
+        if (og) store4<__nv_bfloat16>(og + 4 * v, h4);
+        if (od) store4<__nv_bfloat16>(od + 4 * v, h4);
+        if (!g.fold) {
+          const float4 r4 = ld_stream4(pr + 4 * v);
+          if (og) store4<__nv_bfloat16>(og + g.E + 4 * v, r4);
+          if (od) store4<__nv_bfloat16>(od + g.E + 4 * v, r4);
         }
+        if (od) store4<__nv_bfloat16>(od + g.E + rw + 4 * v, ld_stream4(pt + 4 * v));
       }
       if (og) {
-        for (int v = lane; v < Z4; v += 32) store4<__nv_bfloat16>(og + 2 * g.E + 4 * v, ld_stream4(g.z + row * g.Z + 4 * v));
-        for (int v = (2 * g.E + g.Z) / 4 + lane; v < g.ldg / 4; v += 32)
+        for (int v = lane; v < Z4; v += 32) store4<__nv_bfloat16>(og + g.E + rw + 4 * v, ld_stream4(g.z + row * g.Z + 4 * v));
+        for (int v = (g.E + rw + g.Z + oh) / 4 + lane; v < g.ldg / 4; v += 32)
           store4<__nv_bfloat16>(og + 4 * v, make_float4(0.f, 0.f, 0.f, 0.f));
       }
       if (od)
-        for (int v = (3 * g.E) / 4 + lane; v < g.ldd / 4; v += 32)
+        for (int v = (2 * g.E + rw + oh) / 4 + lane; v < g.ldd / 4; v += 32)
           store4<__nv_bfloat16>(od + 4 * v, make_float4(0.f, 0.f, 0.f, 0.f));
     }
   }
diff --git a/pro-b-gan_b200/csrc/pbg.cu b/pro-b-gan_b200/csrc/pbg.cu
--- a/pro-b-gan_b200/csrc/pbg.cu
+++ b/pro-b-gan_b200/csrc/pbg.cu
@@ -49,6 +49,7 @@
   long long rows = 0;
   void *xg0 = nullptr, *xd0 = nullptr, *bufA = nullptr, *bufB = nullptr, *bufD = nullptr;
   CUtensorMap tm_xg0, tm_xd0, tm_bufA_g, tm_bufA_d, tm_bufB_g, tm_bufD_d;
+  CUtensorMap tm_xg0f, tm_xd0f;
   CUtensorMap tmo_bufA, tmo_bufB, tmo_bufD;
   int mb_cap = 0;
   int* ready = nullptr;
@@ -74,9 +75,10 @@
   void *xg0 = nullptr, *xd0 = nullptr;
   float* xt = nullptr;
   float* z = nullptr;
-  CUtensorMap tm_xg0, tm_xd0;
+  CUtensorMap tm_xg0, tm_xd0, tm_xg0f, tm_xd0f;
   long long B = -1;
   bool has_g = false, has_d = false;
+  bool fold = false;
   bool has_xt = false;
   const float* node_emb = nullptr; long long N = 0; const long long* tails = nullptr;
 };
@@ -96,6 +98,10 @@
   bool g_loaded = false, d_loaded = false;
   int kg0 = 0, kg0p = 0, kd0 = 0, kd0p = 0, hgp = 0, hdp = 0, hd2 = 0, hmax = 0;
   Linear g[3], d[2];
+  int kg0f = 0, kd0f = 0, fold_rp = 0;
+  Linear g0x, d0x;
+  bool fold_on = false;
+  const float* fold_rel = nullptr; long long fold_R = 0;
   float* d_w3 = nullptr;
   float* d_w3_pad = nullptr;
   float d_b3 = 0.f;
@@ -263,6 +269,10 @@
     PBG_CUDA(c, cudaMemset(w.sched, 0, sizeof(PassSched)));
     PBG_TRY(make_tmap(c, &w.tm_xg0, w.xg0, cap, c->kg0p, kBlockM));
     PBG_TRY(make_tmap(c, &w.tm_xd0, w.xd0, cap, c->kd0p, kBlockM));
+    if (c->fold_rp > 0) {
+      PBG_TRY(make_tmap(c, &w.tm_xg0f, w.xg0, cap, c->kg0f, kBlockM));
+      PBG_TRY(make_tmap(c, &w.tm_xd0f, w.xd0, cap, c->kd0f, kBlockM));
+    }
     PBG_TRY(make_tmap(c, &w.tm_bufA_g, w.bufA, cap, c->hgp, kBlockM));
     PBG_TRY(make_tmap(c, &w.tm_bufA_d, w.bufA, cap, c->hdp, kBlockM));
     PBG_TRY(make_tmap(c, &w.tm_bufB_g, w.bufB, cap, c->hgp, kBlockM));
@@ -290,6 +300,10 @@
   PBG_CUDA(c, cudaMalloc(&st.z, sizeof(float) * cap * c->dims.noise_dim));
   PBG_TRY(make_tmap(c, &st.tm_xg0, st.xg0, cap, c->kg0p, kBlockM));
   PBG_TRY(make_tmap(c, &st.tm_xd0, st.xd0, cap, c->kd0p, kBlockM));
+  if (c->fold_rp > 0) {
+    PBG_TRY(make_tmap(c, &st.tm_xg0f, st.xg0, cap, c->kg0f, kBlockM));
+    PBG_TRY(make_tmap(c, &st.tm_xd0f, st.xd0, cap, c->kd0f, kBlockM));
+  }
   st.cap = cap;
   return PBG_OK;
 }
@@ -366,8 +380,13 @@
   void* gen_out = nullptr; int out_dtype = PBG_DT_F32;
   float *gen_scores = nullptr, *logits = nullptr, *probs = nullptr;
   bool run_g = false, run_d = false;
+  bool may_fold = false;
   long long B = 0; int prec = PBG_PREC_BF16; cudaStream_t stream = nullptr;
 };
+
+bool folds(const pbg_ctx* c, const float* rel_emb, long long R) {
+  return c->fold_on && rel_emb == c->fold_rel && R == c->fold_R;
+}
 
 int run_chunk(pbg_ctx* c, const Pass& a, long long off, long long rows) {
   const int E = c->dims.embed_dim, Z = c->dims.noise_dim;
@@ -386,8 +405,10 @@
     PBG_TRY(launch_draw(c, c->lat_seed, 0, c->lat_st, off + rows == a.B, a.B, off, rows, c->lat_z, s));
     gp.z = c->lat_z;
   }
-  gp.xg = a.run_g ? w.xg0 : nullptr; gp.ldg = bf ? c->kg0p : c->kg0;
-  gp.xd = a.run_d ? w.xd0 : nullptr; gp.ldd = bf ? c->kd0p : c->kd0;
+  gp.fold = bf && a.may_fold && a.rels && folds(c, a.rel_emb, a.R);
+  gp.Rp = c->fold_rp;
+  gp.xg = a.run_g ? w.xg0 : nullptr; gp.ldg = bf ? (gp.fold ? c->kg0f : c->kg0p) : c->kg0;
+  gp.xd = a.run_d ? w.xd0 : nullptr; gp.ldd = bf ? (gp.fold ? c->kd0f : c->kd0p) : c->kd0;
   gp.B = rows; gp.err_flag = c->err_flag;
   const int gather_blocks = (int)std::min<long long>((rows + 7) / 8, (long long)c->num_sms * 8);
   if (!bf && (c->n_mirror > 0 || c->mc_gen || c->mc_cos || c->mc_logits || c->mc_probs))
@@ -475,9 +496,11 @@
   const int grid = pass_grid(c) & ~1;
   Pass2Params p;
   memset(&p, 0, sizeof p);
-  const Linear* lin[5] = {&c->g[0], &c->d[0], &c->g[1], &c->d[1], &c->g[2]};
-  const CUtensorMap* amap[5] = {slot ? &slot->tm_xg0 : &w.tm_xg0, slot ? &slot->tm_xd0 : &w.tm_xd0, &w.tm_bufA_g, &w.tm_bufD_d,
-                                &w.tm_bufB_g};
+  const bool fold = slot ? slot->fold : gp.fold != 0;
+  const Linear* lin[5] = {fold ? &c->g0x : &c->g[0], fold ? &c->d0x : &c->d[0], &c->g[1], &c->d[1], &c->g[2]};
+  const CUtensorMap* amap[5] = {slot ? (fold ? &slot->tm_xg0f : &slot->tm_xg0) : (fold ? &w.tm_xg0f : &w.tm_xg0),
+                                slot ? (fold ? &slot->tm_xd0f : &slot->tm_xd0) : (fold ? &w.tm_xd0f : &w.tm_xd0),
+                                &w.tm_bufA_g, &w.tm_bufD_d, &w.tm_bufB_g};
   const CUtensorMap* omap[5] = {&w.tmo_bufA, &w.tmo_bufD, &w.tmo_bufB, nullptr, nullptr};
   const bool on[5] = {a.run_g, a.run_d, a.run_g, a.run_d, a.run_g};
   const int nrb = static_cast<int>((rows + kP2Rows - 1) / kP2Rows);
@@ -545,7 +568,7 @@
   } else if (gather_ahead && slot) {
     p.dead_xg = a.run_g ? slot->xg0 : nullptr; p.dead_xd = a.run_d ? slot->xd0 : nullptr;
   }
-  p.dead_ldg = c->kg0p; p.dead_ldd = c->kd0p;
+  p.dead_ldg = fold ? c->kg0f : c->kg0p; p.dead_ldd = fold ? c->kd0f : c->kd0p;
   p.nrb = nrb; p.rb_cap = w.mb_cap; p.M = static_cast<int>(rows); p.slope = c->dims.leaky_slope;
   p.sched = w.sched; p.ready = w.ready; p.fin = w.fin;
   p.gen_out = gen_out; p.out_f32 = a.out_dtype == PBG_DT_F32; p.n_valid = c->dims.embed_dim; p.ld_gen = c->dims.embed_dim;
@@ -582,8 +605,9 @@
     p.mc_probs = (c->mc_probs && a.probs) ? c->mc_probs + off : nullptr;
   }
   static const bool pdl = [] { const char* e = getenv("PBG_PDL"); return !e || atoi(e) != 0; }();
-  const bool fastg = c->dims.embed_dim == 128 && c->dims.noise_dim % 4 == 0 && c->dims.noise_dim <= 128 &&
-                     c->kg0p == c->kg0 && c->kd0p == c->kd0;
+  const int E = c->dims.embed_dim, Z = c->dims.noise_dim;
+  const bool fastg = E == 128 && Z % 4 == 0 && Z <= 128 &&
+                     (gp.fold ? c->kg0f == E + Z + c->fold_rp && c->kd0f == 2 * E + c->fold_rp : c->kg0p == c->kg0 && c->kd0p == c->kd0);
   const Pass2Kernel kern = kPass2[(p.trace ? 4 : 0) | (fastg ? 2 : 0) | (biass ? 1 : 0)];
   cudaError_t le;
   { LaunchScope ls(c, PBG_K_PASS, a.stream);
@@ -671,6 +695,49 @@
     if (E <= 128) topk_prepare_kernel<8, 1><<<c->num_sms * 8, 256, 0, s>>>(table, N, n_pad, E, t.tn, t.inv_t);
     else topk_prepare_kernel<2, 4><<<c->num_sms * 8, 256, 0, s>>>(table, N, n_pad, E, t.tn, t.inv_t); }
   PBG_CUDA(c, cudaGetLastError());
+  return PBG_OK;
+}
+
+int pbg_prepare_relations(pbg_ctx* c, const float* rel_emb, int64_t R, void* stream) {
+  if (!c) return PBG_ERR_INVALID;
+  if (!rel_emb || R <= 0) return fail(c, PBG_ERR_INVALID, "prepare_relations: null or empty relation table");
+  if (!c->g_loaded && !c->d_loaded) return fail(c, PBG_ERR_NOT_LOADED, "prepare_relations: no model weights loaded");
+  PBG_CUDA(c, cudaSetDevice(c->dims.device));
+  cudaStream_t s = (cudaStream_t)stream;
+  PBG_TRY(begin_growth(c, s, "the folded first layers"));
+  const int E = c->dims.embed_dim, Z = c->dims.noise_dim;
+  const int rp = round_up(static_cast<int>(std::min<int64_t>(R, 1 << 20)), kBlockK);
+  if (rel_emb != c->fold_rel || R != c->fold_R)
+    for (StageSlot& st : c->stage) if (st.fold) st.B = -1;
+  c->fold_on = false; c->fold_rel = nullptr; c->fold_R = 0;
+  if (rp >= E) return PBG_OK;
+  c->fold_rp = rp;
+  c->kg0f = round_up(E + Z + rp, kBlockK); c->kd0f = round_up(2 * E + rp, kBlockK);
+  auto build = [&](Linear& x, const Linear& l, int kp) -> int {
+    free_linear(x);
+    x.n = l.n; x.k = kp; x.np = l.np; x.kp = kp;
+    PBG_CUDA(c, cudaMalloc(&x.w_bf16, sizeof(__nv_bfloat16) * (size_t)x.np * x.kp));
+    PBG_CUDA(c, cudaMalloc(&x.b_pad, sizeof(float) * x.np));
+    PBG_CUDA(c, cudaMemcpyAsync(x.b_pad, l.b_pad, sizeof(float) * x.np, cudaMemcpyDeviceToDevice, s));
+    fold_weight_kernel<<<c->num_sms * 4, 256, 0, s>>>(l.w_f32, l.n, l.k, E, rel_emb, static_cast<int>(R), x.w_bf16, x.np, x.kp);
+    PBG_CUDA(c, cudaGetLastError());
+    PBG_TRY(make_tmap(c, &x.tmap_w128, x.w_bf16, x.np, x.kp, 128));
+    return make_tmap(c, &x.tmap_w64, x.w_bf16, x.np, x.kp, 64);
+  };
+  if (c->g_loaded) PBG_TRY(build(c->g0x, c->g[0], c->kg0f));
+  if (c->d_loaded) PBG_TRY(build(c->d0x, c->d[0], c->kd0f));
+  Workspace& w = c->ws_bf16;
+  if (w.rows > 0) {
+    PBG_TRY(make_tmap(c, &w.tm_xg0f, w.xg0, w.rows, c->kg0f, kBlockM));
+    PBG_TRY(make_tmap(c, &w.tm_xd0f, w.xd0, w.rows, c->kd0f, kBlockM));
+  }
+  for (StageSlot& st : c->stage)
+    if (st.cap > 0) {
+      PBG_TRY(make_tmap(c, &st.tm_xg0f, st.xg0, st.cap, c->kg0f, kBlockM));
+      PBG_TRY(make_tmap(c, &st.tm_xd0f, st.xd0, st.cap, c->kd0f, kBlockM));
+    }
+  PBG_CUDA(c, cudaStreamSynchronize(s));
+  c->fold_rel = rel_emb; c->fold_R = R; c->fold_on = true;
   return PBG_OK;
 }
 
@@ -935,6 +1002,7 @@
   cudaDeviceSynchronize();
   for (auto& l : c->g) free_linear(l);
   for (auto& l : c->d) free_linear(l);
+  free_linear(c->g0x); free_linear(c->d0x);
   cudaFree(c->d_w3); cudaFree(c->d_w3_pad);
   free_ws(c->ws_bf16); free_ws(c->ws_f32);
   free_stage(c->stage[0]); free_stage(c->stage[1]);
@@ -958,6 +1026,7 @@
   if (n_floats != want) return fail(c, PBG_ERR_INVALID, "generator blob has %zu floats, expected %zu", n_floats, want);
   PBG_CUDA(c, cudaSetDevice(c->dims.device));
   c->g_loaded = false;
+  c->fold_on = false;
   const float* w1 = p;            const float* b1 = w1 + H * K0;
   const float* w2 = b1 + H;       const float* b2 = w2 + H * H;
   const float* w3 = b2 + H;       const float* b3 = w3 + E * H;
@@ -975,6 +1044,7 @@
   if (n_floats != want) return fail(c, PBG_ERR_INVALID, "discriminator blob has %zu floats, expected %zu", n_floats, want);
   PBG_CUDA(c, cudaSetDevice(c->dims.device));
   c->d_loaded = false;
+  c->fold_on = false;
   const float* w1 = p;            const float* b1 = w1 + H * K0;
   const float* w2 = b1 + H;       const float* b2 = w2 + H2 * H;
   const float* w3 = b2 + H2;      const float* b3 = w3 + H2;
@@ -1036,7 +1106,7 @@
                        float* logits, float* probs, int64_t B, int precision, void* stream) {
   if (!c) return PBG_ERR_INVALID;
   if (B > 0 && (!node_emb || !rel_emb || !triplets)) return fail(c, PBG_ERR_INVALID, "null tensor");
-  Pass a; a.node_emb = node_emb; a.N = N; a.rel_emb = rel_emb; a.R = R;
+  Pass a; a.node_emb = node_emb; a.N = N; a.rel_emb = rel_emb; a.R = R; a.may_fold = true;
   const long long* t = (const long long*)triplets;
   a.heads = t; a.rels = t + 1; a.tails = t + 2; a.hs = a.rs = a.ts = 3;
   a.z = z; a.gen_out = gen_out; a.out_dtype = out_dtype; a.gen_scores = gen_scores;
@@ -1105,8 +1175,10 @@
   gp.node_emb = node_emb; gp.rel_emb = rel_emb; gp.N = N; gp.R = R; gp.E = c->dims.embed_dim; gp.Z = c->dims.noise_dim;
   gp.heads = t; gp.rels = t + 1; gp.tails = t + 2; gp.head_stride = gp.rel_stride = gp.tail_stride = 3;
   gp.z = z;
-  gp.xg = gen ? st.xg0 : nullptr; gp.ldg = c->kg0p;
-  gp.xd = disc ? st.xd0 : nullptr; gp.ldd = c->kd0p;
+  gp.fold = folds(c, rel_emb, R);
+  gp.Rp = c->fold_rp;
+  gp.xg = gen ? st.xg0 : nullptr; gp.ldg = gp.fold ? c->kg0f : c->kg0p;
+  gp.xd = disc ? st.xd0 : nullptr; gp.ldd = gp.fold ? c->kd0f : c->kd0p;
   gp.B = B; gp.err_flag = c->err_flag;
   return gp;
 }
@@ -1151,7 +1223,7 @@
   { LaunchScope ls(c, PBG_K_GATHER, s);
     stage_rows_kernel<<<blocks, 128, 0, s>>>(sp); }
   PBG_CUDA(c, cudaGetLastError());
-  st.B = B; st.has_g = want_gen != 0; st.has_d = want_disc != 0; st.has_xt = want_gen != 0;
+  st.B = B; st.has_g = want_gen != 0; st.has_d = want_disc != 0; st.has_xt = want_gen != 0; st.fold = sp.g.fold != 0;
   st.node_emb = node_emb; st.N = N; st.tails = t + 2;
   return PBG_OK;
 }
@@ -1191,7 +1263,7 @@
   const GatherParams gp = slot_gather(c, nx, node_emb, N, rel_emb, R, t, next_z, next_B, a.run_g, a.run_d);
   PBG_TRY(launch_pass2(c, c->ws_bf16, a, gp, 0, a.B, gen_out, gen_scores, true, &st, true));
   st.B = -1;
-  nx.B = next_B; nx.has_g = a.run_g; nx.has_d = a.run_d; nx.has_xt = false;
+  nx.B = next_B; nx.has_g = a.run_g; nx.has_d = a.run_d; nx.has_xt = false; nx.fold = gp.fold != 0;
   nx.node_emb = node_emb; nx.N = N; nx.tails = t + 2;
   return PBG_OK;
 }
diff --git a/pro-b-gan_b200/pbg/cabi.py b/pro-b-gan_b200/pbg/cabi.py
--- a/pro-b-gan_b200/pbg/cabi.py
+++ b/pro-b-gan_b200/pbg/cabi.py
@@ -18,6 +18,7 @@
     "pbg_set_launch_width", "pbg_set_result_mirrors", "pbg_topk_prepare", "pbg_topk", "pbg_parse_index_rows", "pbg_format_f32_json", "pbg_format_i64_json",
     "pbg_reserve", "pbg_stage_triplets", "pbg_score_staged", "pbg_set_result_multicast", "pbg_topk_last_flagged", "pbg_score_triplets_host_packed", "pbg_score_staged_stage_next", "pbg_set_workspace_discard", "pbg_last_pass_sm_clock",
     "pbg_draw_latents", "pbg_set_latent_stream", "pbg_get_latent_stream", "pbg_score_triplets_host_ids",
+    "pbg_prepare_relations",
 )
 
 
@@ -72,6 +73,7 @@
         "pbg_last_pass_sm_clock": (C.c_int, [vp, vp, C.POINTER(C.c_double)]),
         "pbg_set_result_mirrors": (C.c_int, [vp, i32, vp, vp, vp, vp]),
         "pbg_topk_prepare": (C.c_int, [vp, vp, i64, vp]),
+        "pbg_prepare_relations": (C.c_int, [vp, vp, i64, vp]),
         "pbg_topk": (C.c_int, [vp, vp, i64, i32, vp, vp, vp]),
         "pbg_parse_index_rows": (i64, [C.c_char_p, sz, i32, vp, sz]),
         "pbg_format_f32_json": (i64, [vp, sz, i32, i32, i32, vp, sz]),
diff --git a/pro-b-gan_b200/pbg/engine.py b/pro-b-gan_b200/pbg/engine.py
--- a/pro-b-gan_b200/pbg/engine.py
+++ b/pro-b-gan_b200/pbg/engine.py
@@ -133,12 +133,37 @@
     def load_generator(self, layers) -> None:
         blob = torch.cat([t.reshape(-1).float().cpu() for wb in layers for t in wb]).contiguous()
         cabi.check(self._lib.pbg_load_generator(self._h, C.c_void_p(blob.data_ptr()), blob.numel()), self._h)
+        self._rel_key = None
         self.g_loaded = True
 
     def load_discriminator(self, layers) -> None:
         blob = torch.cat([t.reshape(-1).float().cpu() for wb in layers for t in wb]).contiguous()
         cabi.check(self._lib.pbg_load_discriminator(self._h, C.c_void_p(blob.data_ptr()), blob.numel()), self._h)
+        self._rel_key = None
         self.d_loaded = True
+
+    def prepare_relations(self, rel_w: torch.Tensor) -> None:
+        rel_w = self._f32(rel_w, self.E, "rel_emb.weight")
+        key = (rel_w.data_ptr(), tuple(rel_w.shape), rel_w._version)
+        with torch.cuda.device(self.device):
+            cabi.check(self._lib.pbg_prepare_relations(self._h, _ptr(rel_w), rel_w.shape[0], self._stream()), self._h)
+        self._rel_key, self._rel_table = key, rel_w
+
+    def _fold(self, rel_w: torch.Tensor) -> None:
+        if not (self.g_loaded or self.d_loaded):
+            return
+        key = (rel_w.data_ptr(), tuple(rel_w.shape), rel_w._version)
+        if getattr(self, "_rel_key", None) == key:
+            return
+        unfolded = self.__dict__.setdefault("_rel_unfolded", set())
+        if torch.cuda.is_current_stream_capturing():
+            if getattr(self, "_rel_key", None) is not None and self._rel_key[:2] == key[:2]:
+                raise RuntimeError("rel_emb.weight changed in place since it was folded into the first layers: run a call "
+                                   "(or prepare_relations) before capturing")
+            unfolded.add(key[:2])
+            return
+        if key[:2] not in unfolded:
+            self.prepare_relations(rel_w)
 
     def _stream(self):
         return C.c_void_p(torch.cuda.current_stream(self.device).cuda_stream)
@@ -273,6 +298,8 @@
         run_g = want_gen_out or want_gen_scores
         if run_g:
             z = self._latents(z)
+        if precision_code(precision) == cabi.PREC_BF16:
+            self._fold(rel_w)
         res = {}
         out = out or {}
 
@@ -317,6 +344,7 @@
         trip = trip.contiguous()
         if want_gen:
             z = self._latents(z)
+        self._fold(rel_w)
         B = trip.shape[0]
         with torch.cuda.device(self.device):
             cabi.check(self._lib.pbg_stage_triplets(
@@ -362,6 +390,7 @@
                 run_g = want_gen_out or want_gen_scores
                 if run_g:
                     n_z = self._latents(n_z)
+                self._fold(n_rel)
                 cabi.check(self._lib.pbg_score_staged_stage_next(
                     self._h, int(slot), _ptr(gen_out), dt, _ptr(scores), _ptr(logits), _ptr(probs), _ptr(n_emb), n_emb.shape[0],
                     _ptr(n_rel), n_rel.shape[0], _ptr(n_trip), _ptr(n_z if run_g else None), n_trip.shape[0], self._stream()),
@@ -388,6 +417,8 @@
         if triplets_host.dtype != torch.int64 or triplets_host.dim() != 2 or triplets_host.shape[1] != 3:
             raise ValueError("triplets_host must be int64 [B, 3]")
         B = triplets_host.shape[0]
+        if precision_code(precision) == cabi.PREC_BF16:
+            self._fold(rel_w)
         with torch.cuda.device(self.device):
             cabi.check(self._lib.pbg_score_triplets_host(
                 self._h, _ptr(node_emb), node_emb.shape[0], _ptr(rel_w), rel_w.shape[0], _ptr(triplets_host),
@@ -402,6 +433,8 @@
             raise ValueError(f"in_block_host must hold {B * (24 + 4 * self.Z)} contiguous bytes")
         if out_block_host.dtype != torch.float32 or out_block_host.numel() != 3 * B or not out_block_host.is_contiguous():
             raise ValueError(f"out_block_host must be a contiguous fp32 tensor of {3 * B} elements")
+        if precision_code(precision) == cabi.PREC_BF16:
+            self._fold(rel_w)
         with torch.cuda.device(self.device):
             cabi.check(self._lib.pbg_score_triplets_host_packed(
                 self._h, _ptr(node_emb), node_emb.shape[0], _ptr(rel_w), rel_w.shape[0], _ptr(in_block_host),
@@ -419,6 +452,8 @@
             raise ValueError(f"out_block_host must be a contiguous fp32 tensor of {3 * B} elements")
         if not self._latent_on:
             raise ValueError("score_triplets_host_ids draws the latents on the device: call set_latent_stream first")
+        if precision_code(precision) == cabi.PREC_BF16:
+            self._fold(rel_w)
         with torch.cuda.device(self.device):
             cabi.check(self._lib.pbg_score_triplets_host_ids(
                 self._h, _ptr(node_emb), node_emb.shape[0], _ptr(rel_w), rel_w.shape[0], _ptr(triplets_host),
diff --git a/pro-b-gan_b200/pbg/inference.py b/pro-b-gan_b200/pbg/inference.py
--- a/pro-b-gan_b200/pbg/inference.py
+++ b/pro-b-gan_b200/pbg/inference.py
@@ -48,6 +48,7 @@
         self.generator.precision = self.discriminator.precision = precision
         t2 = time.perf_counter()
         self.engine = m.make_fused_engine(self.generator, self.discriminator)
+        self.engine.prepare_relations(self.rel_weight)
         self.latents = m.latent_source(latents)
         if self.latents == "cuda":
             self.engine.set_latent_stream(True, m.LATENT_SEED, 0)
```

After: 178.1 million, median of 6. About the same (+0.0%).
